# avik-pal/RegNeuralDE.jl

Hardware: AMD Instinct MI355X
Metric: training-step samples/sec + mean NFE, MNIST Neural ODE bs=512 (higher is better)
Workload: dtype f32; 1 GPU; MNIST NODE regularized (error_est), Tsit5 reltol=abstol=1.4e-8, batch 512 per GPU, 1xMI355X per rank; step = loss fwd + reverse pass through the solver + InvDecay/Momentum update; the weights train during the timed steps (mean_nfe drifts with --steps: value_fixed_weights of --full is the stationary companion); global_batch=512, parallelism=single

## Files before the change

### include/rnde.h

```cpp
#ifndef RNDE_H
#define RNDE_H
#include <stddef.h>
#include <stdint.h>

#ifdef __cplusplus
extern "C" {
#endif

#define RNDE_MAX_LAYERS 8

typedef enum {
    RNDE_OK = 0,
    RNDE_ERR_BAD_ARG = 1,
    RNDE_ERR_MAX_ATTEMPTS = 2,
    RNDE_ERR_DT_UNDERFLOW = 3,
    RNDE_ERR_NONFINITE = 4,
    RNDE_ERR_HIP = 5,
    RNDE_ERR_NO_TAPE = 6,
    RNDE_ERR_NO_DEVICE = 7
} rnde_status;

typedef enum { RNDE_ACT_IDENTITY = 0, RNDE_ACT_TANH = 1, RNDE_ACT_RELU = 2, RNDE_ACT_SIGMOID = 3, RNDE_ACT_SOFTPLUS = 4, RNDE_ACT_ELU = 5 } rnde_act;
typedef enum { RNDE_PRE_NONE = 0, RNDE_PRE_TANH = 1, RNDE_PRE_CUBE = 2 } rnde_pre_act;
typedef enum { RNDE_SOLVER_TSIT5 = 0, RNDE_SOLVER_DP5 = 1, RNDE_SOLVER_DOP853 = 2 } rnde_solver;
// ... 17 lines not shown
    int32_t max_attempts;
    int32_t device;
    int32_t col_tile;
    int32_t persist;
    int32_t wgrad_side_pct;
    int32_t stage_generic;
} rnde_node_config;

typedef struct rnde_node rnde_node;
typedef struct rnde_comm rnde_comm;

const char* rnde_version(void);
const char* rnde_last_error(const rnde_node* h);
int32_t     rnde_param_count(const rnde_node_config* cfg);

rnde_status rnde_node_create(const rnde_node_config* cfg, rnde_node** out);
void        rnde_node_destroy(rnde_node* h);

rnde_status rnde_node_forward(rnde_node* h, const float* x_dev, const float* p_dev, int32_t B,
                              float t0, float t1, float* u_out_dev, int64_t* nfe_out,
                              float* saveval_host, int32_t* n_saveval_out, int32_t keep_tape,
                              void* stream);

rnde_status rnde_node_forward_saveat(rnde_node* h, const float* x_dev, const float* p_dev, int32_t B,
                                     float t0, float t1, const float* saveat_host, int32_t n_saveat,
                                     float* u_saved_dev, int64_t* nfe_out, float* saveval_host,
                                     int32_t* n_saveval_out, int32_t keep_tape, void* stream);

rnde_status rnde_node_forward_everystep(rnde_node* h, const float* x_dev, const float* p_dev, int32_t B, float t0, float t1,
                                        int32_t save_start, float* sol_out_dev, int32_t capacity, float* t_host_out, int32_t* n_out,
                                        int64_t* nfe_out, float* saveval_host, int32_t* n_saveval_out, int32_t keep_tape, void* stream);

rnde_status rnde_node_forward_replay(rnde_node* h, const float* x_dev, const float* p_dev, int32_t B,
                                     float t0, float t1, const float* steps_host, int32_t n_steps,
                                     float* u_out_dev, int64_t* nfe_out, float* saveval_host,
                                     int32_t* n_saveval_out, int32_t keep_tape, void* stream);

rnde_status rnde_node_backward(rnde_node* h, const float* u_bar_dev, const float* saveval_bar_host,
                               float* x_bar_dev, float* p_bar_dev, float* tspan_bar_host,
                               void* stream);

rnde_status rnde_node_backward_async(rnde_node* h, const float* u_bar_dev, const float* saveval_bar_host,
                                     float* x_bar_dev, float* p_bar_dev, float* tspan_bar_dev, void* stream);

rnde_status rnde_node_release_tape(rnde_node* h);

rnde_status rnde_node_forward_host(rnde_node* h, const float* x, const float* p, int32_t B, float t0,
                                   float t1, float* u_out, int64_t* nfe_out, float* saveval,
                                   int32_t* n_saveval_out, int32_t keep_tape);
rnde_status rnde_node_backward_host(rnde_node* h, const float* u_bar, const float* saveval_bar,
                                    float* x_bar, float* p_bar, float* tspan_bar);

rnde_status rnde_node_steps(rnde_node* h, float* steps_host, int32_t capacity, int32_t* n_attempts_out);

rnde_status rnde_debug_feval(rnde_node* h, const float* u_dev, const float* p_dev, int32_t B, float t,
                             float* out_dev, void* stream);
rnde_status rnde_debug_attempt(rnde_node* h, const float* uprev_dev, const float* k1_dev,
                               const float* p_dev, int32_t B, float t, float dt, float* k_out_dev,
                               float* unew_out_dev, float* eest_out, void* stream);
rnde_status rnde_bench_attempt(rnde_node* h, const float* x_dev, const float* p_dev, int32_t B,
                               int32_t iters, float* mean_us_out, void* stream);
rnde_status rnde_bench_attempt_taped(rnde_node* h, const float* x_dev, const float* p_dev, int32_t B,
                                     int32_t iters, float* mean_us_out, void* stream);
rnde_status rnde_bench_attempt_cold_tape(rnde_node* h, const float* x_dev, const float* p_dev, int32_t B, int32_t iters,
                                         int32_t records, float* mean_us_out, void* stream);
rnde_status rnde_node_set_timing(rnde_node* h, int32_t on);
rnde_status rnde_node_timing(rnde_node* h, float* fwd_attempts_ms, float* rev_sweep_ms, float* rev_rest_ms);
int32_t     rnde_node_last_attempts(const rnde_node* h);
int32_t     rnde_node_fallback_count(const rnde_node* h);
int32_t     rnde_node_launches_per_attempt(const rnde_node* h);
int32_t     rnde_node_one_launch_solves(const rnde_node* h);
#define RNDE_MATRIX_F32 0
#define RNDE_MATRIX_BF16X3 1
rnde_status rnde_node_set_matrix_mode(rnde_node* h, int32_t mode);
int32_t     rnde_node_matrix_mode(const rnde_node* h);

typedef struct rnde_tapes rnde_tapes;
rnde_status rnde_tapes_create(const rnde_node_config* cfg, int32_t max_tapes, rnde_tapes** out);
void        rnde_tapes_destroy(rnde_tapes* t);
const char* rnde_tapes_last_error(const rnde_tapes* t);
int32_t     rnde_tapes_in_use(const rnde_tapes* t);
rnde_node*  rnde_tapes_node(rnde_tapes* t, int32_t tape_id);
rnde_status rnde_tapes_forward(rnde_tapes* t, const float* x_dev, const float* p_dev, int32_t B, float t0, float t1, float* u_out_dev,
                               int64_t* nfe_out, float* saveval_host, int32_t* n_saveval_out, int32_t keep_tape, void* stream,
                               int32_t* tape_id_out);
rnde_status rnde_tapes_backward(rnde_tapes* t, int32_t tape_id, const float* u_bar_dev, const float* saveval_bar_host, float* x_bar_dev,
                                float* p_bar_dev, float* tspan_bar_host, void* stream);
rnde_status rnde_tapes_release(rnde_tapes* t, int32_t tape_id);

rnde_status rnde_classifier_head(rnde_node* h, const float* u_dev, const float* p3_dev, const float* y_dev,
                                 int32_t B, int32_t n_classes, float* logits_out_dev, float* u_bar_dev,
                                 float* p3_bar_dev, float* ce_out_dev, void* stream);

rnde_status rnde_node_classifier_grad(rnde_node* h, const float* x_dev, const float* p2_dev, const float* p3_dev,
                                      const float* y_dev, int32_t B, int32_t n_classes, float t0, float t1, float lambda,
                                      float* p2_bar_dev, float* p3_bar_dev, float* x_bar_dev, float* ce_out_dev,
                                      float* reg_out_host, int64_t* nfe_out, rnde_comm* comm, void* stream);

rnde_status rnde_momentum_step(float* p_dev, const float* g_dev, float* v_dev, int64_t len, int64_t n, float gamma,
                               float eta, float rho, void* stream);

rnde_status rnde_momentum_step_scaled(float* p_dev, const float* g_dev, float* v_dev, int64_t len, int64_t n, float gamma,
                                      float eta, float rho, float gscale, void* stream);
rnde_status rnde_adam_step(float* p_dev, const float* g_dev, float* m_dev, float* v_dev, int64_t len, int64_t t, float eta, float beta1,
                           float beta2, float eps, float gscale, void* stream);
rnde_status rnde_adabelief_step(float* p_dev, const float* g_dev, float* m_dev, float* s_dev, int64_t len, float eta, float beta1, float beta2,
                                float eps, float gscale, void* stream);

#define RNDE_COMM_ID_BYTES 128
rnde_status rnde_comm_unique_id(uint8_t id_out[RNDE_COMM_ID_BYTES]);
rnde_status rnde_comm_create(const uint8_t id[RNDE_COMM_ID_BYTES], int32_t rank, int32_t world, int32_t device, rnde_comm** out);
void        rnde_comm_destroy(rnde_comm* c);
int32_t     rnde_comm_world(const rnde_comm* c);
const char* rnde_comm_last_error(const rnde_comm* c);
const char* rnde_comm_library(void);
rnde_status rnde_comm_allreduce(rnde_comm* c, float* buf_dev, int64_t n, int32_t mean, void* stream);
rnde_status rnde_comm_create_local_group(int32_t world, int32_t device, rnde_comm** out);
rnde_status rnde_comm_health(rnde_comm* c);
#define RNDE_COMM_WINDOW_BYTES 64
typedef struct rnde_comm_window rnde_comm_window;
rnde_status rnde_comm_window_create(int32_t device, rnde_comm_window** win_out, uint8_t handle_out[RNDE_COMM_WINDOW_BYTES]);
void        rnde_comm_window_destroy(rnde_comm_window* w);
rnde_status rnde_comm_create_peers(rnde_comm_window* win, const uint8_t* handles, int32_t rank, int32_t world, rnde_comm** out);
const char* rnde_comm_path(const rnde_comm* c);

rnde_status rnde_node_set_coupling(rnde_node* h, rnde_comm* c, int32_t global_batch);

typedef enum { RNDE_SDE_SOSRI = 0, RNDE_SDE_SRIW1 = 1, RNDE_SDE_SOSRI2 = 2 } rnde_sde_solver;

typedef struct {
    int32_t drift_layers;
    int32_t drift_dims[RNDE_MAX_LAYERS + 1];
    int32_t drift_act[RNDE_MAX_LAYERS];
    int32_t diff_layers;
    int32_t diff_dims[RNDE_MAX_LAYERS + 1];
    int32_t diff_act[RNDE_MAX_LAYERS];
    int32_t max_batch;
    int32_t solver;
    float   reltol, abstol;
    int32_t regularize;
    int32_t cb_save_start;
    int32_t max_attempts;
    int32_t device;
    float   beta1, beta2, gamma, qmin, qmax, qoldinit, delta;
    int32_t generic;
    float   stability_size;
} rnde_nsde_config;

typedef struct rnde_nsde rnde_nsde;

int32_t     rnde_nsde_param_count(const rnde_nsde_config* cfg, int32_t* len_drift_out);
rnde_status rnde_nsde_create(const rnde_nsde_config* cfg, rnde_nsde** out);
void        rnde_nsde_destroy(rnde_nsde* h);
const char* rnde_nsde_last_error(const rnde_nsde* h);

rnde_status rnde_nsde_forward(rnde_nsde* h, const float* x_dev, const float* p_dev, int32_t B, float t0, float t1,
// ... 95 lines not shown
```

### regneuralde.jl_amd/_lib.py

```python
import ctypes as C
import os

from . import build as _build

MAX_LAYERS = 8
OK, BAD_ARG, MAX_ATTEMPTS, DT_UNDERFLOW, NONFINITE, HIP_ERR, NO_TAPE, NO_DEVICE = range(8)
REG = {"none": 0, False: 0, None: 0, "error_est": 1, True: 1, "stiff_est": 2, "error_stiff_est": 3}


class NodeConfig(C.Structure):
    _fields_ = [("n_layers", C.c_int32), ("dims", C.c_int32 * (MAX_LAYERS + 1)), ("act", C.c_int32 * MAX_LAYERS),
                ("time_dep", C.c_int32), ("pre_act", C.c_int32), ("max_batch", C.c_int32), ("solver", C.c_int32),
                ("reltol", C.c_float), ("abstol", C.c_float), ("regularize", C.c_int32),
                ("cb_save_start", C.c_int32), ("track_ctrl", C.c_int32), ("track_initdt", C.c_int32),
                ("max_attempts", C.c_int32), ("device", C.c_int32), ("col_tile", C.c_int32),
                ("persist", C.c_int32), ("wgrad_side_pct", C.c_int32), ("stage_generic", C.c_int32)]


class NsdeConfig(C.Structure):
    _fields_ = [("drift_layers", C.c_int32), ("drift_dims", C.c_int32 * (MAX_LAYERS + 1)), ("drift_act", C.c_int32 * MAX_LAYERS),
                ("diff_layers", C.c_int32), ("diff_dims", C.c_int32 * (MAX_LAYERS + 1)), ("diff_act", C.c_int32 * MAX_LAYERS),
                ("max_batch", C.c_int32), ("solver", C.c_int32), ("reltol", C.c_float), ("abstol", C.c_float),
                ("regularize", C.c_int32), ("cb_save_start", C.c_int32), ("max_attempts", C.c_int32), ("device", C.c_int32),
                ("beta1", C.c_float), ("beta2", C.c_float), ("gamma", C.c_float), ("qmin", C.c_float), ("qmax", C.c_float),
# ... 2 lines not shown

class FfjordConfig(C.Structure):
    _fields_ = [("in_dims", C.c_int32), ("hidden", C.c_int32), ("dynamics", C.c_int32), ("time_dep", C.c_int32), ("regularize", C.c_int32),
                ("kinetic_reg", C.c_int32), ("max_batch", C.c_int32), ("solver", C.c_int32), ("reltol", C.c_float), ("abstol", C.c_float),
                ("cb_save_start", C.c_int32), ("max_attempts", C.c_int32), ("device", C.c_int32)]


class LatentConfig(C.Structure):
    _fields_ = [("max_batch", C.c_int32), ("max_T", C.c_int32), ("device", C.c_int32)]


ODE_SOLVER = {"Tsit5": 0, "AutoTsit5": 0, "DP5": 1, "DOP853": 2}
SDE_SOLVER = {"SOSRI": 0, "SRIW1": 1, "SOSRI2": 2, "AutoSOSRI2": 2}


class RndeError(RuntimeError):
    def __init__(self, status, msg):
        super().__init__(f"rnde status {status}: {msg}")
        self.status = status


_lib = None


def lib():
    global _lib
    if _lib is not None:
        return _lib
    path = _build.LIB
    if not os.path.exists(path):
        raise ImportError(f"{path} is missing: build it with `python -c 'import __graft_entry__ as g; g.build()'` "
                          "(hipcc --offload-arch=gfx950). There is no CPU fallback for the integration path.")
    L = C.CDLL(path)
    vp, f, i32, i64p, fp, i32p = C.c_void_p, C.c_float, C.c_int32, C.POINTER(C.c_int64), C.POINTER(C.c_float), C.POINTER(C.c_int32)
    L.rnde_version.restype = C.c_char_p
    L.rnde_last_error.restype = C.c_char_p
    L.rnde_last_error.argtypes = [vp]
    L.rnde_param_count.restype = i32
    L.rnde_param_count.argtypes = [C.POINTER(NodeConfig)]
    L.rnde_node_create.argtypes = [C.POINTER(NodeConfig), C.POINTER(vp)]
    L.rnde_node_destroy.argtypes = [vp]
    L.rnde_node_destroy.restype = None
    L.rnde_node_forward.argtypes = [vp, vp, vp, i32, f, f, vp, i64p, fp, i32p, i32, vp]
    L.rnde_node_forward_saveat.argtypes = [vp, vp, vp, i32, f, f, fp, i32, vp, i64p, fp, i32p, i32, vp]
    L.rnde_node_forward_everystep.argtypes = [vp, vp, vp, i32, f, f, i32, vp, i32, fp, i32p, i64p, fp, i32p, i32, vp]
    L.rnde_node_forward_replay.argtypes = [vp, vp, vp, i32, f, f, fp, i32, vp, i64p, fp, i32p, i32, vp]
    L.rnde_node_backward.argtypes = [vp, vp, fp, vp, vp, fp, vp]
    L.rnde_node_backward_async.restype = C.c_int32
    L.rnde_node_backward_async.argtypes = [vp, vp, fp, vp, vp, vp, vp]
    L.rnde_node_release_tape.argtypes = [vp]
    L.rnde_node_forward_host.argtypes = [vp, fp, fp, i32, f, f, fp, i64p, fp, i32p, i32]
    L.rnde_node_backward_host.argtypes = [vp, fp, fp, fp, fp, fp]
    L.rnde_node_steps.argtypes = [vp, fp, i32, i32p]
    L.rnde_debug_feval.argtypes = [vp, vp, vp, i32, f, vp, vp]
    L.rnde_debug_attempt.argtypes = [vp, vp, vp, vp, i32, f, f, vp, vp, fp, vp]
    L.rnde_bench_attempt.argtypes = [vp, vp, vp, i32, i32, fp, vp]
    L.rnde_bench_attempt_taped.argtypes = [vp, vp, vp, i32, i32, fp, vp]
    L.rnde_bench_attempt_cold_tape.argtypes = [vp, vp, vp, i32, i32, i32, fp, vp]
    L.rnde_node_set_timing.argtypes = [vp, i32]
    L.rnde_node_timing.argtypes = [vp, fp, fp, fp]
    L.rnde_node_fallback_count.restype = C.c_int32
    L.rnde_node_fallback_count.argtypes = [vp]
    L.rnde_node_last_attempts.restype = C.c_int32
    L.rnde_node_last_attempts.argtypes = [vp]
    L.rnde_node_launches_per_attempt.restype = C.c_int32
    L.rnde_node_launches_per_attempt.argtypes = [vp]
    L.rnde_node_one_launch_solves.restype = C.c_int32
    L.rnde_node_one_launch_solves.argtypes = [vp]
    L.rnde_node_set_matrix_mode.restype = C.c_int32
    L.rnde_node_set_matrix_mode.argtypes = [vp, i32]
    L.rnde_node_matrix_mode.restype = C.c_int32
    L.rnde_node_matrix_mode.argtypes = [vp]
    L.rnde_classifier_head.argtypes = [vp, vp, vp, vp, i32, i32, vp, vp, vp, vp, vp]
    L.rnde_node_classifier_grad.argtypes = [vp, vp, vp, vp, vp, i32, i32, f, f, f, vp, vp, vp, vp, fp, C.POINTER(C.c_int64), vp, vp]
    L.rnde_momentum_step.argtypes = [vp, vp, vp, C.c_int64, C.c_int64, f, f, f, vp]
    u64 = C.c_uint64
    L.rnde_momentum_step_scaled.argtypes = [vp, vp, vp, C.c_int64, C.c_int64, f, f, f, f, vp]
    L.rnde_adam_step.argtypes = [vp, vp, vp, vp, C.c_int64, C.c_int64, C.c_float, C.c_float, C.c_float, C.c_float, C.c_float, vp]
    L.rnde_adabelief_step.argtypes = [vp, vp, vp, vp, C.c_int64, f, f, f, f, f, vp]
    L.rnde_moment_loss.argtypes = [vp, vp, vp, i32, i32, i32, vp, vp, vp]
    L.rnde_comm_unique_id.argtypes = [C.c_char_p]
    L.rnde_comm_create.argtypes = [C.c_char_p, i32, i32, i32, C.POINTER(vp)]
    L.rnde_comm_destroy.argtypes = [vp]
    L.rnde_comm_destroy.restype = None
    L.rnde_comm_world.argtypes = [vp]
    L.rnde_comm_world.restype = i32
    L.rnde_comm_last_error.argtypes = [vp]
    L.rnde_comm_last_error.restype = C.c_char_p
    L.rnde_comm_library.argtypes = []
    L.rnde_comm_library.restype = C.c_char_p
    L.rnde_comm_allreduce.argtypes = [vp, vp, C.c_int64, i32, vp]
    L.rnde_comm_create_local_group.argtypes = [i32, i32, C.POINTER(vp)]
    L.rnde_node_set_coupling.argtypes = [vp, vp, i32]
    L.rnde_comm_health.argtypes = [vp]
    L.rnde_comm_window_create.argtypes = [i32, C.POINTER(vp), C.c_char_p]
    L.rnde_comm_window_destroy.argtypes = [vp]
    L.rnde_comm_window_destroy.restype = None
    L.rnde_comm_create_peers.argtypes = [vp, C.c_char_p, i32, i32, C.POINTER(vp)]
    L.rnde_comm_path.argtypes = [vp]
    L.rnde_comm_path.restype = C.c_char_p
    L.rnde_tapes_create.argtypes = [C.POINTER(NodeConfig), i32, C.POINTER(vp)]
    L.rnde_tapes_destroy.argtypes = [vp]
    L.rnde_tapes_destroy.restype = None
    L.rnde_tapes_last_error.argtypes = [vp]
    L.rnde_tapes_last_error.restype = C.c_char_p
    L.rnde_tapes_in_use.argtypes = [vp]
    L.rnde_tapes_node.argtypes = [vp, i32]
    L.rnde_tapes_node.restype = vp
    L.rnde_tapes_forward.argtypes = [vp, vp, vp, i32, C.c_float, C.c_float, vp, C.POINTER(C.c_int64), fp, C.POINTER(i32), i32, vp, C.POINTER(i32)]
    L.rnde_tapes_backward.argtypes = [vp, i32, vp, fp, vp, vp, fp, vp]
    L.rnde_tapes_release.argtypes = [vp, i32]
    L.rnde_nsde_param_count.restype = i32
    L.rnde_nsde_param_count.argtypes = [C.POINTER(NsdeConfig), i32p]
    L.rnde_nsde_create.argtypes = [C.POINTER(NsdeConfig), C.POINTER(vp)]
    L.rnde_nsde_destroy.argtypes = [vp]
    L.rnde_nsde_destroy.restype = None
    L.rnde_nsde_last_error.restype = C.c_char_p
    L.rnde_nsde_last_error.argtypes = [vp]
    L.rnde_nsde_forward.argtypes = [vp, vp, vp, i32, f, f, vp, i32, u64, vp, i64p, i64p, fp, i32p, i32, vp]
    L.rnde_nsde_forward_saveat.argtypes = [vp, vp, vp, i32, f, f, vp, i32, u64, fp, i32, vp, i64p, i64p, fp, i32p, i32, vp]
    L.rnde_nsde_forward_everystep.argtypes = [vp, vp, vp, i32, f, f, vp, i32, u64, i32, vp, i32, fp, i32p, i64p, i64p, fp, i32p, i32, vp]
    L.rnde_nsde_forward_replay.argtypes = [vp, vp, vp, i32, f, f, vp, i32, fp, i32, vp, i64p, i64p, fp, i32p, i32, vp]
    L.rnde_nsde_backward.argtypes = [vp, vp, fp, vp, vp, vp]
    L.rnde_nsde_backward_async.argtypes = [vp, vp, fp, vp, vp, vp]
    L.rnde_nsde_classifier_head.argtypes = [vp, vp, vp, vp, i32, i32, vp, vp, vp, vp, vp]
    L.rnde_nsde_classifier_grad.argtypes = [vp, vp, vp, vp, vp, i32, i32, f, f, vp, i32, C.c_uint64, f, vp, vp, vp, vp, fp, C.POINTER(C.c_int64), C.POINTER(C.c_int64), vp]
    L.rnde_nsde_steps.argtypes = [vp, fp, i32, i32p, i32p]
    L.rnde_nsde_debug_attempt.argtypes = [vp, vp, vp, i32, f, vp, vp, vp, vp, fp, vp]
    L.rnde_nsde_set_pre_act.argtypes = [vp, i32, i32]
    L.rnde_nsde_moment_grad.argtypes = [vp, vp, vp, i32, f, f, vp, i32, u64, fp, i32, vp, vp, f, vp, vp, vp, fp, i64p, i64p, vp]
    L.rnde_nsde_timing.argtypes = [vp, fp, fp, i32p, i32p]
    L.rnde_normal_fill.argtypes = [vp, C.c_int64, u64, u64, vp]
    L.rnde_latent_create.argtypes = [C.POINTER(LatentConfig), C.POINTER(vp)]
    L.rnde_latent_destroy.argtypes = [vp]
    L.rnde_latent_destroy.restype = None
    L.rnde_latent_last_error.argtypes = [vp]
    L.rnde_latent_last_error.restype = C.c_char_p
    L.rnde_latent_param_counts.argtypes = [i32p, i32p, i32p]
    L.rnde_latent_param_counts.restype = None
    L.rnde_latent_encode.argtypes = [vp, vp, vp, vp, vp, i32, i32, vp, vp, vp, vp]
    L.rnde_latent_decode_loss.argtypes = [vp, vp, vp, vp, i32, i32, vp, vp, vp, vp]
    L.rnde_latent_encode_backward.argtypes = [vp, vp, f, vp, vp, vp, vp, vp, vp]
    L.rnde_adamax_step.argtypes = [vp, vp, vp, vp, C.c_int64, C.c_int64, f, f, f, f, f, f, vp]
    L.rnde_ffjord_param_count.restype = i32
    L.rnde_ffjord_param_count.argtypes = [C.POINTER(FfjordConfig)]
    L.rnde_ffjord_create.argtypes = [C.POINTER(FfjordConfig), C.POINTER(vp)]
    L.rnde_ffjord_destroy.argtypes = [vp]
    L.rnde_ffjord_destroy.restype = None
    L.rnde_ffjord_last_error.argtypes = [vp]
    L.rnde_ffjord_last_error.restype = C.c_char_p
    L.rnde_ffjord_forward.argtypes = [vp, vp, vp, vp, i32, f, f, u64, vp, vp, i64p, fp, i32p, i32, vp]
    L.rnde_ffjord_forward_replay.argtypes = [vp, vp, vp, vp, i32, f, f, u64, fp, i32, vp, vp, i64p, fp, i32p, i32, vp]
    L.rnde_ffjord_steps.argtypes = [vp, fp, i32, i32p]
    L.rnde_ffjord_backward.argtypes = [vp, vp, fp, vp, vp, vp]
    L.rnde_ffjord_sample.argtypes = [vp, vp, vp, i32, f, f, u64, vp, vp]
    L.rnde_ffjord_debug_feval.argtypes = [vp, vp, vp, vp, i32, f, i32, vp, vp]
    L.rnde_ffjord_timing.argtypes = [vp, fp, fp, i32p, i32p]
    L.rnde_ffjord_create_tiled.argtypes = [C.POINTER(FfjordConfig), C.POINTER(vp)]
    L.rnde_ffjord_engine.restype = i32
    L.rnde_ffjord_engine.argtypes = [vp]
    _lib = L
    return L


EXPORTS = ["rnde_version", "rnde_last_error", "rnde_param_count", "rnde_node_create", "rnde_node_destroy",
           "rnde_node_forward", "rnde_node_forward_saveat", "rnde_node_forward_everystep", "rnde_node_forward_replay", "rnde_node_backward", "rnde_node_backward_async", "rnde_node_release_tape", "rnde_node_forward_host",
           "rnde_node_backward_host", "rnde_node_steps", "rnde_debug_feval", "rnde_debug_attempt",
           "rnde_bench_attempt", "rnde_bench_attempt_taped", "rnde_bench_attempt_cold_tape", "rnde_node_set_timing", "rnde_node_timing", "rnde_node_last_attempts", "rnde_node_fallback_count",
           "rnde_node_launches_per_attempt", "rnde_node_one_launch_solves", "rnde_node_set_matrix_mode", "rnde_node_matrix_mode", "rnde_classifier_head", "rnde_node_classifier_grad", "rnde_momentum_step", "rnde_momentum_step_scaled", "rnde_adam_step",
           "rnde_comm_unique_id", "rnde_comm_create", "rnde_comm_destroy", "rnde_comm_world", "rnde_comm_last_error", "rnde_comm_library", "rnde_comm_allreduce", "rnde_comm_create_local_group", "rnde_comm_health", "rnde_comm_window_create", "rnde_comm_window_destroy", "rnde_comm_create_peers", "rnde_comm_path", "rnde_node_set_coupling", "rnde_tapes_create", "rnde_tapes_destroy", "rnde_tapes_last_error", "rnde_tapes_in_use", "rnde_tapes_node", "rnde_tapes_forward", "rnde_tapes_backward", "rnde_tapes_release",
           "rnde_nsde_param_count", "rnde_nsde_create", "rnde_nsde_destroy", "rnde_nsde_last_error", "rnde_nsde_forward",
           "rnde_nsde_forward_saveat", "rnde_nsde_forward_everystep", "rnde_nsde_forward_replay", "rnde_nsde_backward", "rnde_nsde_backward_async", "rnde_nsde_classifier_head", "rnde_nsde_classifier_grad", "rnde_nsde_steps", "rnde_nsde_debug_attempt", "rnde_nsde_set_pre_act", "rnde_nsde_moment_grad", "rnde_moment_loss", "rnde_adabelief_step", "rnde_nsde_timing", "rnde_normal_fill", "rnde_latent_create", "rnde_latent_destroy", "rnde_latent_last_error", "rnde_latent_param_counts", "rnde_latent_encode",
           "rnde_latent_decode_loss", "rnde_latent_encode_backward", "rnde_adamax_step",
           "rnde_ffjord_param_count", "rnde_ffjord_create", "rnde_ffjord_destroy", "rnde_ffjord_last_error", "rnde_ffjord_forward",
           "rnde_ffjord_forward_replay", "rnde_ffjord_steps", "rnde_ffjord_backward", "rnde_ffjord_sample", "rnde_ffjord_debug_feval",
           "rnde_ffjord_timing", "rnde_ffjord_create_tiled", "rnde_ffjord_engine"]


def check(h, status):
    if status != OK:
        msg = lib().rnde_last_error(h).decode() if h else lib().rnde_last_error(None).decode()
        raise RndeError(status, msg)


def check_latent(h, status):
    if status != OK:
        raise RndeError(status, lib().rnde_latent_last_error(h if h else None).decode())


def check_ffjord(h, status):
    if status != OK:
        raise RndeError(status, lib().rnde_ffjord_last_error(h if h else None).decode())


def check_nsde(h, status):
    if status != OK:
        raise RndeError(status, lib().rnde_nsde_last_error(h if h else None).decode())
```

### regneuralde.jl_amd/classifier.py

```python
import math
import os

import torch

from .layers import Dense
from .node import TrackedNeuralODE


class ClassifierNODE:

    def __init__(self, node: TrackedNeuralODE, post: Dense, device="cuda"):
        self.node = node
        self.post_shape = (post.n_in, post.n_out)
        self.p1 = torch.zeros(0, device=device)
        self.p2 = node.p.to(device).clone().requires_grad_(True)
        self.p3 = torch.cat([post.W.reshape(-1), post.b]).to(device).clone().requires_grad_(True)

    def trainable(self):
        return (self.p1, self.p2, self.p3)

    def __call__(self, x, p1=None, p2=None, p3=None, **node_kwargs):
        p2 = self.p2 if p2 is None else p2
        p3 = self.p3 if p3 is None else p3
        x = x.reshape(x.shape[0], -1)
# ... 55 lines not shown
    n = nsv.value
    reg = 0.0
    svb = None
    if regularize and n > 0 and node.regularize:
        if agg_max:
            vals = list(sv[:n])
            k = max(range(n), key=lambda i: vals[i])
            reg = lam * vals[k]
            svb = (C.c_float * n)(*[lam if i == k else 0.0 for i in range(n)])
        else:
            reg = lam * sum(sv[:n]) / n
            svb = (C.c_float * n)(*([lam / n] * n))
    xbar = torch.empty_like(x2)
    n2 = p2bar.numel()
    if not sync:
        _lib.check(h.ptr, L.rnde_node_backward_async(h.ptr, ubar.data_ptr(), svb, xbar.data_ptr(), p2bar.data_ptr(), None, stream))
        if reducer is not None:
            reducer.allreduce_range_(0, n2 + p3bar.numel())
        model.p2.grad, model.p3.grad = p2bar, p3bar
        node.last_nfe = int(nfe.value)
        model._keep = (ubar, xbar, u)
        return ce + reg, ce, reg, int(nfe.value)
    _lib.check(h.ptr, L.rnde_node_backward(h.ptr, ubar.data_ptr(), svb, xbar.data_ptr(), p2bar.data_ptr(), None, stream))
    if reducer is not None:
        reducer.allreduce_range_(0, n2 + p3bar.numel())
    model.p2.grad, model.p3.grad = p2bar, p3bar
    node.last_nfe = int(nfe.value)
    ce_f = float(ce.item())
    return ce_f + reg, ce_f, reg, int(nfe.value)


def logitcrossentropy(pred, y_onehot):
    return -(y_onehot * torch.log_softmax(pred, dim=1)).sum(dim=1).mean()


def loss_function(x, y, model, p1=None, p2=None, p3=None, lam=1.0e2, regularize=True, agg=torch.mean, func="error_est",
                  tspan=None):
    pred, nfe, sv = model(x, p1, p2, p3, func=func, tspan=tspan)
    ce = logitcrossentropy(pred, y)
    reg = lam * agg(sv.saveval) if regularize else torch.zeros((), device=pred.device)
    return ce + reg, ce.detach(), reg.detach(), nfe


class FluxOptimiser:

    def __init__(self, params, gamma=1.0e-5, eta=0.1, rho=0.9):
        self.params = [p for p in params if p.numel() > 0]
        self.gamma, self.eta, self.rho = gamma, eta, rho
        self.n = [1 for _ in self.params]
        self.v = [torch.zeros_like(p) for p in self.params]

    @torch.no_grad()
    def step(self, grads=None, grad_scale=1.0):
        for i, p in enumerate(self.params):
            g = p.grad if grads is None else grads[i]
            if g is None:
                continue
            if p.is_cuda:
                import ctypes as C
                from . import _lib
                g = g.contiguous()
                st = _lib.lib().rnde_momentum_step_scaled(p.data_ptr(), g.data_ptr(), self.v[i].data_ptr(), p.numel(), self.n[i],
                                                          self.gamma, self.eta, self.rho, float(grad_scale),
                                                          C.c_void_p(torch.cuda.current_stream(p.device).cuda_stream))
                _lib.check(None, st)
                self.n[i] += 1
                p.grad = None
                continue
            g = g * (grad_scale / (1.0 + self.gamma * self.n[i]))
            self.n[i] += 1
            self.v[i].mul_(self.rho).sub_(g, alpha=self.eta)
            p.add_(self.v[i])
            p.grad = None


class FluxADAM:

    def __init__(self, params, eta=0.001, beta=(0.9, 0.999), eps=1.0e-8, gamma=0.0, weight_decay=0.0):
        self.params = [p for p in params if p.numel() > 0]
        self.eta, self.beta, self.eps, self.gamma, self.weight_decay = eta, beta, eps, gamma, weight_decay
        self.n = [1 for _ in self.params]
        self.t = 0
        self.m = [torch.zeros_like(p) for p in self.params]
        self.v = [torch.zeros_like(p) for p in self.params]

    @torch.no_grad()
    def step(self, grad_scale=1.0):
        import ctypes as C
        from . import _lib
        self.t += 1
        for i, p in enumerate(self.params):
            g = p.grad
            if g is None:
                continue
            if not p.is_cuda:
                raise RuntimeError("FluxADAM runs on the device only")
            g = g.contiguous()
            gs = float(grad_scale) / (1.0 + self.gamma * self.n[i])
            if self.weight_decay:
                g = g.mul(float(grad_scale)).add_(p.data, alpha=float(self.weight_decay)).contiguous()
                gs = 1.0 / (1.0 + self.gamma * self.n[i])
            st = _lib.lib().rnde_adam_step(p.data_ptr(), g.data_ptr(), self.m[i].data_ptr(), self.v[i].data_ptr(), p.numel(), self.t, self.eta,
                                           self.beta[0], self.beta[1], self.eps, gs,
                                           C.c_void_p(torch.cuda.current_stream(p.device).cuda_stream))
            _lib.check(None, st)
            self.n[i] += 1
# ... 55 lines not shown
```

### regneuralde.jl_amd/csrc/rnde.hip

```cpp
#include "rnde_node.h"

static thread_local std::string g_create_err;
extern "C" const char* rnde_version(void) { return "rnde 0.1.0 (gfx950)"; }
extern "C" const char* rnde_last_error(const rnde_node* h) { return h ? h->err.c_str() : g_create_err.c_str(); }

extern "C" int32_t rnde_param_count(const rnde_node_config* c) {
    int n = 0;
    for (int l = 0; l < c->n_layers; ++l) n += (c->dims[l] + (c->time_dep ? 1 : 0)) * c->dims[l + 1] + c->dims[l + 1];
    return n;
}

StepParams make_params(rnde_node* h, const float* x, int B, float t0, float t1, int tape) {
    StepParams P{};
    P.x = x;
    P.f0 = h->f0; P.h0 = h->h0; P.u1 = h->u1; P.f1 = h->f1; P.h1 = h->h1;
    P.arena = h->arena; P.rec_stride = h->rec_stride;
    P.ctl = h->ctl; P.ctl_final = h->ctl_final; P.meta = h->meta; P.initrec = h->initrec;
    P.errpart = h->errpart; P.initpart = h->initpart; P.dbg_out = nullptr;
    P.D = h->D; P.H = h->H; P.B = B; P.Bn = h->couple ? h->couple_batch : B;
    P.Bpad = ((B + 15) / 16) * 16;
    P.nwg = h->engine == 2 ? h->sR * (P.Bpad / 16) : (h->engine == 3 ? (h->mw ? P.Bpad / 16 : (P.Bpad / 16 + kCW - 1) / kCW) : P.Bpad / h->BT);
    P.reltol = h->cfg.reltol; P.abstol = h->cfg.abstol; P.t0 = t0; P.t1 = t1;
    P.tape = tape; P.max_attempts = h->cfg.max_attempts;
    P.forced = 0; P.forced_t = 0; P.forced_dt = 0;
// ... 300 lines not shown
    if (hipGetDeviceCount(&ndev) != hipSuccess || ndev <= c->device) { g_create_err = "no HIP device"; return RNDE_ERR_NO_DEVICE; }
    if ((c->solver != RNDE_SOLVER_TSIT5 && c->solver != RNDE_SOLVER_DP5 && c->solver != RNDE_SOLVER_DOP853) || c->n_layers < 1 || c->n_layers > RNDE_MAX_LAYERS || c->dims[0] != c->dims[c->n_layers]) {
        g_create_err = "unsupported configuration: Tsit5 (or DP5) over a Dense chain with dims[0] == dims[n_layers]"; return RNDE_ERR_BAD_ARG;
    }
    if (c->pre_act != RNDE_PRE_NONE && c->pre_act != RNDE_PRE_TANH && c->pre_act != RNDE_PRE_CUBE) {
        g_create_err = "pre_act: RNDE_PRE_NONE, RNDE_PRE_TANH or RNDE_PRE_CUBE"; return RNDE_ERR_BAD_ARG;
    }
    if (!rnde_check_acts(c->n_layers, c->act, "act", g_create_err)) return RNDE_ERR_BAD_ARG;
    const bool mnist_form = c->n_layers == 2 && c->time_dep && !c->pre_act && c->act[0] == RNDE_ACT_TANH;
    if (mnist_form && c->col_tile != 64 && c->col_tile != 65 && c->act[1] != RNDE_ACT_IDENTITY && c->act[1] != RNDE_ACT_TANH) {
        g_create_err = std::string("act[1] = ") + rnde_act_name(c->act[1]) + ": the stage engine (two time-dependent layers, act[0] = tanh, no pre_act, col_tile 0 / 16) "
                       "serves identity or tanh in its second layer; a chain of width <= 64 runs any served activation on the chain engine (col_tile 64 / 65)";
        return RNDE_ERR_BAD_ARG;
    }
    if ((c->solver == RNDE_SOLVER_DP5 || c->solver == RNDE_SOLVER_DOP853) && ((mnist_form && c->col_tile != 65) || c->col_tile == 64 || c->regularize >= RNDE_REG_STIFF)) {
        g_create_err = "DP5 / DOP853 run on the tableau-as-data kernels of the chain engine (col_tile 0 for Dense chains of width <= 64, or 65), callbacks none / EEst*dt";
        return RNDE_ERR_BAD_ARG;
    }
    if (c->col_tile == 64 || c->col_tile == 65 || !mnist_form) return chain_create(c, out);
    if (c->regularize < RNDE_REG_NONE || c->regularize > RNDE_REG_STIFF_DT) { g_create_err = "regularize: unknown value"; return RNDE_ERR_BAD_ARG; }
    rnde_node* h = new rnde_node();
    h->cfg = *c;
    h->D = c->dims[0]; h->H = c->dims[1]; h->P = rnde_param_count(c); h->act2 = c->act[1];
    h->BT = 8;
    if (c->col_tile != 0 && c->col_tile != 16) {
        g_create_err = "col_tile must be 0 (auto) or 16 (stage engine) for the two-layer TDChain form; 64 / 65 select the chain engine.  (The round-1 column-owner "
                       "engine, col_tile 4 / 8, was retired in round 4: 126 us per attempted step against 24; its sources are kept under tools/experiments/column_owner/.)";
        delete h; return RNDE_ERR_BAD_ARG;
    }
    if (h->H + 2 > 128 || h->D < 1 || h->H < 1 || (h->D + 15) / 16 > 64 || c->max_batch < 1 || c->max_attempts < 1) {
        g_create_err = "shape outside the kernel limits (H <= 126, D <= 1024)"; delete h; return RNDE_ERR_BAD_ARG;
    }
    h->Bpad_max = ((c->max_batch + 15) / 16) * 16;
    h->sMT = (h->D + 15) / 16; h->sHT = (h->H + 1 + 15) / 16; h->sK2b = (h->H + 2 + 15) / 16; h->sKHb = (h->H + 15) / 16;
    { int best = 1, bw = 1 << 30;
      for (int wt = std::min(8, h->sMT); wt >= std::max(1, std::min(4, h->sMT)); --wt) { int R = (h->sMT + wt - 1) / wt; int waste = R * wt - h->sMT; if (waste < bw) { bw = waste; best = wt; } }
      if (const char* e = getenv("RNDE_STAGE_WT")) { const int v = atoi(e); if (v >= 1 && v <= 8) best = std::min(v, h->sMT); }
      h->sWT = best; h->sR = (h->sMT + best - 1) / best; }
    h->engine = 2;
    h->nwg_max = std::max(h->Bpad_max / h->BT, h->sR * (h->Bpad_max / 16));
    h->stage_lds = sizeof(float) * ((size_t)16 * (16 * std::max(h->sK2b, h->sHT) + 4) + (size_t)16 * (16 * std::max(h->sWT, h->sKHb) + 4) + 64);
    if (hipSetDevice(c->device) != hipSuccess) { g_create_err = "hipSetDevice failed"; delete h; return RNDE_ERR_HIP; }
    const size_t A = (size_t)h->D * h->Bpad_max, HB = (size_t)h->H * h->Bpad_max;
    RecLayout L{(long long)A, (long long)HB};
    h->rec_stride = L.total();
    auto dm = [&](void** p, size_t bytes) { return hipMalloc(p, bytes) == hipSuccess; };
    bool ok = true;
    ok &= dm((void**)&h->f0, A * 4) && dm((void**)&h->u1, A * 4) && dm((void**)&h->f1, A * 4) && dm((void**)&h->xcopy, A * 4);
    ok &= dm((void**)&h->h0, HB * 4) && dm((void**)&h->h1, HB * 4);
    ok &= dm((void**)&h->pcopy, (size_t)h->P * 4);
    ok &= dm((void**)&h->spwB, (size_t)h->sMT * h->sK2b * 64 * 16) && dm((void**)&h->spwD, (size_t)h->sHT * h->sMT * 64 * 16);
    ok &= dm((void**)&h->spwBt, (size_t)h->sMT * h->sKHb * 64 * 16) && dm((void**)&h->spwDt, (size_t)h->sHT * h->sMT * 64 * 16);
    ok &= dm((void**)&h->slab2, (size_t)2 * (h->Bpad_max / 16) * h->sR * h->sHT * 64 * 16);
    const size_t tslab_bytes = (size_t)3 * (h->Bpad_max / 16) * h->sR * h->sHT * 64 * 16;
    h->tslab_bytes = tslab_bytes;
    ok &= dm((void**)&h->tslab, tslab_bytes);
    static_assert(sizeof(StepState) <= 512 && sizeof(InitRec) <= 504, "mailbox layout");
    h->mbox_meta_off = (1024 + (size_t)h->nwg_max * 4 + 255) / 256 * 256;
    const size_t mbox_bytes = h->mbox_meta_off + (size_t)(c->max_attempts + 1) * sizeof(StepMeta);
    ok &= dm((void**)&h->mbox, mbox_bytes) && hipHostMalloc((void**)&h->h_mbox, mbox_bytes) == hipSuccess;
    if (ok) {
        hipMemset(h->mbox, 0, mbox_bytes);
        h->ctl_final = (StepState*)h->mbox; h->initrec = (InitRec*)(h->mbox + 512);
        h->pabort = (unsigned*)(h->mbox + 1016); h->pxcc = (unsigned*)(h->mbox + 1024); h->meta = (StepMeta*)(h->mbox + h->mbox_meta_off);
        h->h_ctl = (StepState*)h->h_mbox; h->h_init = (InitRec*)(h->h_mbox + 512);
        h->h_pchk = (unsigned*)(h->h_mbox + 1016); h->h_meta = (StepMeta*)(h->h_mbox + h->mbox_meta_off);
    }
    ok &= dm((void**)&h->ctl, 2 * sizeof(StepState));
    ok &= dm((void**)&h->errpart, (size_t)(6 * h->nwg_max + 256 + 16) * 4) && dm((void**)&h->initpart, (size_t)(3 * h->nwg_max + 256) * 4);
    h->arena_recs = 2;
    ok &= dm((void**)&h->arena, (size_t)h->arena_recs * h->rec_stride * 4);
    ok &= hipHostMalloc((void**)&h->h_scal, 64 * sizeof(float)) == hipSuccess;
    if (!ok) { g_create_err = "device allocation failed"; rnde_node_destroy(h); return RNDE_ERR_HIP; }
    hipMemset(h->tslab, 0xFF, tslab_bytes); hipMemset(h->pabort, 0, 8); hipMemset(h->pxcc, 0, (size_t)h->nwg_max * 4);
    {
        const char* e = getenv("RNDE_PERSIST");
        const bool off = c->persist < 0 || (e && e[0] == '0');
        h->persist = (h->engine == 2 && h->sR <= 8 && !off) ? 1 : 0;
        if (const char* e2 = getenv("RNDE_PERSIST_SPINS")) h->persist_spins = atoi(e2);
        if (const char* e3 = getenv("RNDE_PERSIST2")) h->persist2 = atoi(e3);
        h->wgrad_side_pct = c->wgrad_side_pct < 0 ? 0 : (c->wgrad_side_pct == 0 ? 30 : std::min(100, c->wgrad_side_pct));
        if (const char* e3 = getenv("RNDE_WGRAD_SIDE")) h->wgrad_side_pct = atoi(e3);
        h->stage_generic = (c->stage_generic != 0 || getenv("RNDE_STAGE_GENERIC") != nullptr) ? 1 : 0;
        if (const char* e6 = getenv("RNDE_STAGE_SOLVE")) h->stage_solve = atoi(e6);
    }
    if (h->persist == 1 && h->stage_solve && c->max_attempts < 8192) {
        const size_t xb = (size_t)(c->max_attempts + 1) * 3 * 256 * 8;
        if (hipMalloc((void**)&h->sxch, xb) != hipSuccess) { g_create_err = "device allocation failed"; rnde_node_destroy(h); return RNDE_ERR_HIP; }
        hipMemset(h->sxch, 0, xb);
    }
    if (h->persist == 1) {
        h->x3 = 1;
        if (const char* e7 = getenv("RNDE_X3")) h->x3 = atoi(e7) != 0;
        if (h->sMT == 49 && h->sHT == 7 && h->sR == 7 && h->sWT == 7 && h->D == 784 && h->H == 100 && !h->stage_generic) {
            const size_t img = (size_t)49 * 4 * 3 * 64 * 16;
            if (hipMalloc(&h->x3B, img) != hipSuccess || hipMalloc(&h->x3D, img) != hipSuccess || hipMalloc(&h->x3Bt, img) != hipSuccess || hipMalloc(&h->x3Dt, img) != hipSuccess) { g_create_err = "device allocation failed"; rnde_node_destroy(h); return RNDE_ERR_HIP; }
        } else h->x3 = 0;
    }
    h->predicted = 12;
    *out = h;
    return RNDE_OK;
}

extern "C" void rnde_node_destroy(rnde_node* h) {
    if (!h) return;
    void* d[] = {h->f0, h->h0, h->u1, h->f1, h->h1, h->arena, h->xcopy, h->pcopy, h->spwB, h->spwD, h->spwBt, h->spwDt, h->slab2,
                 h->ctl, h->ctl_final, h->meta, h->initrec, h->errpart, h->initpart};
// ... 65 lines not shown
    HIPCHK(h, hipMalloc((void**)&h->arena, (size_t)recs * h->rec_stride * 4));
    h->arena_recs = recs;
    return RNDE_OK;
}

static StageParams make_stage_params(rnde_node* h, const StepParams& P, const float* p_dev) {
    StageParams Q{};
    Q.F = P; Q.p = p_dev; Q.pwB = h->spwB; Q.pwD = h->spwD; Q.slab = h->slab2;
    Q.MT = h->sMT; Q.WT = h->sWT; Q.R = h->sR; Q.C = P.Bpad / 16; Q.HT = h->sHT; Q.K2b = h->sK2b; Q.Bpad16 = P.Bpad;
    return Q;
}
template <int ACT2, int MODE>
static hipError_t launch_stage_t(rnde_node* h, const StageParams& Q, int n, int s, hipStream_t st) {
    hipLaunchKernelGGL((rnde_stage_kernel<ACT2, MODE>), dim3(Q.R * Q.C), dim3(64 * Q.WT), h->stage_lds, st, Q, n, s);
    return hipGetLastError();
}
template <int MODE>
static hipError_t launch_stage(rnde_node* h, const StageParams& Q, int n, int s, hipStream_t st) {
    return h->act2 ? launch_stage_t<1, MODE>(h, Q, n, s, st) : launch_stage_t<0, MODE>(h, Q, n, s, st);
}
hipError_t stage_pack(rnde_node* h, const float* p, f32x4* dst, int which, int MTrows, int Kb, hipStream_t st) {
    const long long total = (long long)MTrows * Kb * 64;
    const int grid = (int)std::min<long long>((total + 255) / 256, 1024);
    hipLaunchKernelGGL(rnde_stage_pack_kernel, dim3(grid), dim3(256), 0, st, p, dst, which, h->D, h->H, MTrows, Kb);
    return hipGetLastError();
}
static rnde_status x3_pack(rnde_node* h, const float* p_dev, bool with_rev, hipStream_t s) {
    h->x3_fwd = false;
    if (!(h->x3 && h->x3B && h->x3D && h->persist == 1 && !h->stage_generic)) return RNDE_OK;
    HIPCHK(h, rnde_launch_x3_pack(p_dev, h->x3B, h->x3D, with_rev ? h->x3Bt : nullptr, with_rev ? h->x3Dt : nullptr, h->D, h->H, h->sMT, h->sWT, h->sR, h->sHT, s));
    h->x3_fwd = true;
    h->x3_packed = with_rev;
    return RNDE_OK;
}
static rnde_status stage_pack_weights(rnde_node* h, const float* p_dev, hipStream_t s) {
    HIPCHK(h, stage_pack(h, p_dev, h->spwB, 0, h->sMT, h->sK2b, s));
    HIPCHK(h, stage_pack(h, p_dev, h->spwD, 1, h->sHT, h->sMT, s));
    return x3_pack(h, p_dev, false, s);
}
rnde_status stage_pack_all(rnde_node* h, const float* p_dev, hipStream_t s, const float* x_src, long long x_floats) {
    PackJobs J{};
    int n = 0;
    auto add = [&](void* dst, long long total, int kind, int which, int kdim, const float* src = nullptr) { J.j[n++] = PackJob{dst, src, total, kind, which, kdim, 0}; };
    add(h->spwB, (long long)h->sMT * h->sK2b * 64, 0, 0, h->sK2b);
    add(h->spwD, (long long)h->sHT * h->sMT * 64, 0, 1, h->sMT);
    add(h->spwBt, (long long)h->sMT * h->sKHb * 64, 0, 2, h->sKHb);
    add(h->spwDt, (long long)h->sHT * h->sMT * 64, 0, 3, h->sMT);
    auto add_copy = [&](float* dst, const float* src, long long floats) {
        const bool v4 = floats % 4 == 0 && ((uintptr_t)dst % 16 == 0) && ((uintptr_t)(src ? src : p_dev) % 16 == 0);
        add(dst, v4 ? floats / 4 : floats, v4 ? 3 : 2, 0, 0, src);
    };
    add_copy(h->pcopy, nullptr, (long long)h->P);
    if (x_src) add_copy(h->xcopy, x_src, x_floats);
    long long most = 0;
    for (int i = 0; i < n; ++i) most = std::max(most, J.j[i].total);
    const int grid = (int)std::min<long long>((most + 255) / 256, 256);
    hipLaunchKernelGGL(rnde_pack_all_kernel, dim3(grid, n), dim3(256), 0, s, p_dev, J, h->D, h->H);
    HIPCHK(h, hipGetLastError());
    h->rev_packed = true;
    return x3_pack(h, p_dev, true, s);
}
hipError_t slab_prepare(rnde_node* h, int Bpad, hipStream_t s) {
    if (h->tslab_Bpad == Bpad) return hipSuccess;
    h->tslab_Bpad = Bpad;
    return hipMemsetAsync(h->tslab, 0xFF, h->tslab_bytes, s);
}
static bool stage_two_tile(const rnde_node* h, const StageParams& Q) {
    const bool fix = Q.WT == 7 && Q.HT == 7 && Q.K2b == 7 && Q.MT == 49 && Q.R == 7 && h->D == 784 && h->H == 100 && !h->stage_generic;
    return h->persist == 1 && fix && Q.C % 2 == 0 && h->persist2 != 0 && (Q.C >= kPersist2MinTiles || h->persist2 >= 1);
}
static bool stage_epart_reduce(const rnde_node* h, const StageParams& Q) {
    return stage_two_tile(h, Q) && Q.F.nwg >= 896 && !getenv("RNDE_NO_EPART_REDUCE");
}
static hipError_t stage_attempt(rnde_node* h, const StageParams& Q, int n, hipStream_t s) {
    if (h->persist == 1) {
        PersistSync Y{h->tslab, h->pabort, h->pxcc, h->persist_spins};
        if (hipError_t e = slab_prepare(h, Q.Bpad16, s); e != hipSuccess) return e;
        const dim3 grid(8 * Q.R * ((Q.C + 7) / 8));
        const bool fix = Q.WT == 7 && Q.HT == 7 && Q.K2b == 7 && Q.MT == 49 && Q.R == 7 && h->D == 784 && h->H == 100 && !h->stage_generic;
        static const bool x3_over_mt = !(getenv("RNDE_X3_MT") && atoi(getenv("RNDE_X3_MT")) == 0);
        if (stage_two_tile(h, Q)) {
            const dim3 grid2(8 * Q.R * ((Q.C / 2 + 7) / 8));
            if (h->x3_fwd && x3_over_mt) {
                const size_t xlds2 = sizeof(float) * ((size_t)2 * 2 * kX3ImageFloats + 32 * 3);
                if (h->act2) hipLaunchKernelGGL((rnde_stage_attempt_mt_kernel<1, 2, 1>), grid2, dim3(64 * 7), xlds2, s, Q, n, Y, (const void*)h->x3B, (const void*)h->x3D);
                else hipLaunchKernelGGL((rnde_stage_attempt_mt_kernel<0, 2, 1>), grid2, dim3(64 * 7), xlds2, s, Q, n, Y, (const void*)h->x3B, (const void*)h->x3D);
                return hipGetLastError();
            }
            const size_t lds2 = sizeof(float) * (2 * 2 * 16 * (16 * 7 + 4) + 32 * 3);
            if (h->act2) hipLaunchKernelGGL((rnde_stage_attempt_mt_kernel<1, 2>), grid2, dim3(64 * 7), lds2, s, Q, n, Y, (const void*)nullptr, (const void*)nullptr);
            else hipLaunchKernelGGL((rnde_stage_attempt_mt_kernel<0, 2>), grid2, dim3(64 * 7), lds2, s, Q, n, Y, (const void*)nullptr, (const void*)nullptr);
            return hipGetLastError();
        }
        if (fix && h->x3_fwd) {
            const size_t xlds = sizeof(float) * ((size_t)2 * kX3ImageFloats + 64);
            if (h->act2) hipLaunchKernelGGL((rnde_stage_attempt_kernel<1, 1, 1>), grid, dim3(64 * 7), xlds, s, Q, n, Y, (const void*)h->x3B, (const void*)h->x3D);
            else hipLaunchKernelGGL((rnde_stage_attempt_kernel<0, 1, 1>), grid, dim3(64 * 7), xlds, s, Q, n, Y, (const void*)h->x3B, (const void*)h->x3D);
        } else if (fix) {
            if (h->act2) hipLaunchKernelGGL((rnde_stage_attempt_kernel<1, 1>), grid, dim3(64 * Q.WT), h->stage_lds, s, Q, n, Y, (const void*)nullptr, (const void*)nullptr);
            else hipLaunchKernelGGL((rnde_stage_attempt_kernel<0, 1>), grid, dim3(64 * Q.WT), h->stage_lds, s, Q, n, Y, (const void*)nullptr, (const void*)nullptr);
        } else if (h->act2) hipLaunchKernelGGL((rnde_stage_attempt_kernel<1, 0>), grid, dim3(64 * Q.WT), h->stage_lds, s, Q, n, Y, (const void*)nullptr, (const void*)nullptr);
        else hipLaunchKernelGGL((rnde_stage_attempt_kernel<0, 0>), grid, dim3(64 * Q.WT), h->stage_lds, s, Q, n, Y, (const void*)nullptr, (const void*)nullptr);
        return hipGetLastError();
    }
    hipError_t e = launch_stage<SM_START>(h, Q, n, 0, s);
    for (int st = 1; st <= 5 && e == hipSuccess; ++st) e = launch_stage<SM_STAGE>(h, Q, n, st, s);
    if (e == hipSuccess) e = launch_stage<SM_LAST>(h, Q, n, 6, s);
    return e;
}

bool bsweep_failed(rnde_node* h, hipStream_t s) {
    if (!h->pending_bsweep) return false;
    h->pending_bsweep = false;
    bool bad = h->h_mw_bchk[0] != 0;
    const int nt = h->bsweep_nt;
    for (int i = 1; i < nt && !h->bsweep_global && !bad; ++i) bad = h->h_mw_bchk[2 + i] != h->h_mw_bchk[2];
    if (!bad) return false;
    fprintf(stderr, "[rnde] chain engine: one-launch reverse sweep abandoned (%s); one launch per reversed attempt for the next %d solves\n",
// ... 95 lines not shown
        h->err = "coupled controller: equal shards only (B * world must equal the global batch given to rnde_node_set_coupling)";
        return RNDE_ERR_BAD_ARG;
    }
    HIPCHK(h, hipSetDevice(h->cfg.device));
    h->have_tape = false; h->rev_packed = false; h->x3_packed = false; h->x3_fwd = false;
    const float* x_caller = nullptr;
    if (keep_tape) {
        rnde_status st = ensure_arena(h, h->cfg.max_attempts);
        if (st != RNDE_OK) return st;
        if (B % h->BT) HIPCHK(h, hipMemsetAsync(h->xcopy, 0, (size_t)h->D * (((B + h->BT - 1) / h->BT) * h->BT) * 4, s));
        if (h->engine != 2) {
            HIPCHK(h, hipMemcpyAsync(h->xcopy, x_dev, (size_t)h->D * B * 4, hipMemcpyDeviceToDevice, s));
            HIPCHK(h, hipMemcpyAsync(h->pcopy, p_dev, (size_t)h->P * 4, hipMemcpyDeviceToDevice, s));
        } else x_caller = x_dev;
        x_dev = h->xcopy;
    }
    StepParams P = make_params(h, x_dev, B, t0, t1, keep_tape ? 1 : 0);
    P.sv_t = n_saveat > 0 ? h->sv_t_dev : nullptr; P.nsave = n_saveat; P.sv_out = sv_out_dev;
    if (h->n_replay > 0) {
        if ((size_t)h->n_replay > h->replay_cap) {
            if (h->replay_dev) hipFree(h->replay_dev);
            h->replay_dev = nullptr; h->replay_cap = 0;
            HIPCHK(h, hipMalloc((void**)&h->replay_dev, (size_t)h->n_replay * 8));
            h->replay_cap = h->n_replay;
        }
        HIPCHK(h, hipMemcpyAsync(h->replay_dev, h->replay_host, (size_t)h->n_replay * 8, hipMemcpyHostToDevice, s));
        P.replay = h->replay_dev; P.n_replay = h->n_replay;
    }
    h->B = B; h->Bpad = P.Bpad; h->nwg = P.nwg; h->t0 = t0; h->t1 = t1;
    rnde_status st = RNDE_OK;
    if (h->engine == 2 && keep_tape) st = stage_pack_all(h, p_dev, s, x_caller, (long long)h->D * B);
    else if (h->engine == 3) st = chain_pack(h, keep_tape ? h->pcopy : p_dev, s);
    if (st != RNDE_OK) return st;
    StageParams SQ{};
    ChainParams CQ{};
    MwParams MQ{};
    if (h->engine == 3) {
        CQ = make_chain_params(h, P);
        if (h->mw) {
            if (keep_tape) { st = ensure_mw_slab(h, 2 + (long long)(h->rk_S - 1) * std::max(4, h->predicted), P.Bpad, s); if (st != RNDE_OK) return st; }
            MQ = make_mw_params(h, P);
            HIPCHK(h, launch_mw<MW_INIT_A>(h, MQ, 0, s));
            if ((st = couple_sum(h, P.initpart, 2LL * P.nwg, s)) != RNDE_OK) return st;
            HIPCHK(h, launch_mw<MW_INIT_B>(h, MQ, 0, s));
            if ((st = couple_sum(h, P.initpart + 2LL * P.nwg, P.nwg, s)) != RNDE_OK) return st;
        } else {
            HIPCHK(h, launch_chain<CM_INIT_A>(h, CQ, 0, nullptr, s));
            HIPCHK(h, launch_chain<CM_INIT_B>(h, CQ, 0, nullptr, s));
        }
    } else if (h->engine == 2) {
        if (!keep_tape) { st = stage_pack_weights(h, p_dev, s); if (st != RNDE_OK) return st; }
        SQ = make_stage_params(h, P, keep_tape ? h->pcopy : p_dev);
        if (stage_epart_reduce(h, SQ)) SQ.F.esum = (const double*)(h->errpart + 6 * (size_t)h->nwg_max + 256);
        HIPCHK(h, launch_stage<SM_I1>(h, SQ, 0, 0, s));
        HIPCHK(h, launch_stage<SM_I2>(h, SQ, 0, 0, s));
        if ((st = couple_sum(h, P.initpart, 2LL * P.nwg, s)) != RNDE_OK) return st;
        HIPCHK(h, launch_stage<SM_I3>(h, SQ, 0, 0, s));
        HIPCHK(h, launch_stage<SM_I4>(h, SQ, 0, 0, s));
        if ((st = couple_sum(h, P.initpart + 2LL * P.nwg, P.nwg, s)) != RNDE_OK) return st;
    }
    int launched = 0;
    int chunk = h->couple ? 16 : std::max(4, h->predicted);
    const int cap = h->cfg.max_attempts;
    h->tev_fwd = false;
    if (h->timing) HIPCHK(h, hipEventRecord(h->tev[0], s));
    bool solved = false;
    if (h->engine == 3 && h->mw && h->mw_solve > 0 && !h->couple && P.Bpad / 16 <= kMwMeetMax) {
        const int n_limit = keep_tape ? std::min(cap, std::max(48, 2 * h->predicted)) : cap;
        if (keep_tape) { st = ensure_mw_slab(h, 2 + (long long)(h->rk_S - 1) * n_limit, P.Bpad, s); if (st != RNDE_OK) return st; MQ.slab = h->mw_slab; }
        MQ.n_limit = n_limit;
        if (++h->mw_epoch >= 500000u) { h->mw_epoch = 1; HIPCHK(h, hipMemsetAsync(h->mw_xch, 0, (size_t)(cap + 4) * 3 * kMwMeetMax * 8, s)); }
        const int nt = P.Bpad / 16;
        MQ.u_out = u_out_dev; MQ.xch = h->mw_xch; MQ.xcc = h->mw_xcc; MQ.abort_word = h->mw_abort; MQ.epoch = h->mw_epoch; MQ.xch_global = nt > 32 ? 1 : 0; MQ.xcd_slot = h->mw_slot;
        HIPCHK(h, launch_mw<MW_SOLVE>(h, MQ, 0, s));
        if (h->timing) { HIPCHK(h, hipEventRecord(h->tev[1], s)); h->tev_fwd = true; }
        HIPCHK(h, hipMemcpyAsync(h->h_ctl, h->ctl_final, sizeof(StepState), hipMemcpyDeviceToHost, s));
        HIPCHK(h, hipMemcpyAsync(h->h_meta, h->meta, (size_t)cap * sizeof(StepMeta), hipMemcpyDeviceToHost, s));
        HIPCHK(h, hipMemcpyAsync(h->h_init, h->initrec, sizeof(InitRec), hipMemcpyDeviceToHost, s));
        HIPCHK(h, hipMemcpyAsync(h->h_mw_chk, h->mw_abort, 4, hipMemcpyDeviceToHost, s));
        HIPCHK(h, hipMemcpyAsync(h->h_mw_chk + 2, h->mw_xcc, (size_t)nt * 4, hipMemcpyDeviceToHost, s));
        if (h->after_solve) {
            HIPCHK(h, hipEventRecord(h->ev_host, s));
            const rnde_status hs = h->after_solve(s);
            if (hs != RNDE_OK) return hs;
            HIPCHK(h, hipEventSynchronize(h->ev_host));
        } else HIPCHK(h, hipStreamSynchronize(s));
        if (bsweep_failed(h, s)) { h->err = "the one-launch reverse sweep of the previous asynchronous backward call was abandoned: the gradients of that step are invalid (one launch per reversed attempt now in use)"; return RNDE_ERR_HIP; }
        bool bad = h->h_mw_chk[0] != 0;
        for (int i = 1; i < nt && !MQ.xch_global && !bad; ++i) bad = h->h_mw_chk[2 + i] != h->h_mw_chk[2];
        if (bad) {
            fprintf(stderr, "[rnde] chain engine: one-launch solve abandoned (%s); one launch per attempted step for the next %d solves\n",
                    h->h_mw_chk[0] ? "a meeting timed out" : "workgroups pinned by block index landed on different XCDs", h->mw_retry_after);
            h->mw_solve = -1; h->mw_clean = 0; ++h->persist_fallbacks;
            hipMemsetAsync(h->mw_abort, 0, 8, s);
            return RNDE_INTERNAL_RETRY;
        }
        if (!h->h_ctl->done && h->h_ctl->n_att >= n_limit && n_limit < cap) { h->predicted = cap; return RNDE_INTERNAL_RETRY; }
        h->pending_bwd = false;
        ++h->one_launch_solves;
        solved = true;
    }
    if (h->engine == 2 && h->persist == 1 && h->stage_solve && h->sxch && SQ.C <= 32 && n_saveat == 0 && h->n_replay == 0 && !h->couple &&
        SQ.WT == 7 && SQ.HT == 7 && SQ.K2b == 7 && SQ.MT == 49 && SQ.R == 7 && h->D == 784 && h->H == 100 && !h->stage_generic) {
        PersistSync Y{h->tslab, h->pabort, h->pxcc, h->persist_spins};
        HIPCHK(h, slab_prepare(h, SQ.Bpad16, s));
        if (++h->s_epoch >= 500000u) { h->s_epoch = 1; HIPCHK(h, hipMemsetAsync(h->sxch, 0, (size_t)(cap + 1) * 3 * 256 * 8, s)); }
        const int x3 = h->x3_fwd ? 1 : 0;
        SolveSync Z{h->sxch, h->s_epoch, cap, h->x3B, h->x3D};
#ifdef RNDE_DIAG
        StageParams SD = SQ;
        if (getenv("RNDE_DIAG_SOLVE")) {
// ... 171 lines not shown
    }
    h->n_saveval = nsv;
    if (n_saveval_out) *n_saveval_out = nsv;
    switch (h->h_ctl->status) {
        case 0: break;
        case 2: h->err = "max_attempts reached"; return RNDE_ERR_MAX_ATTEMPTS;
        case 3: h->err = "dt underflow"; return RNDE_ERR_DT_UNDERFLOW;
        default: h->err = "non-finite error estimate or dt"; return RNDE_ERR_NONFINITE;
    }
    h->have_tape = keep_tape != 0;
    return RNDE_OK;
}

extern "C" rnde_status rnde_node_forward_everystep(rnde_node* h, const float* x_dev, const float* p_dev, int32_t B, float t0, float t1, int32_t save_start,
                                                   float* sol_out_dev, int32_t capacity, float* t_host_out, int32_t* n_out, int64_t* nfe_out,
                                                   float* saveval_host, int32_t* n_saveval_out, int32_t keep_tape, void* stream) {
    if (!h || !n_out || !sol_out_dev || capacity < 1) return RNDE_ERR_BAD_ARG;
    rnde_status st = forward_impl(h, x_dev, p_dev, B, t0, t1, nullptr, nullptr, 0, nullptr, nullptr, nullptr, nullptr, 0, stream);
    if (st != RNDE_OK) return st;
    std::vector<float> times;
    if (save_start) times.push_back(t0);
    for (int i = 0; i < h->n_att; ++i) {
        const StepMeta& m = h->h_meta[i];
        if (m.flags & F_ACCEPT) { float tn = m.t + m.dt; if (tn > t1) tn = t1; times.push_back(tn); }
    }
    *n_out = (int32_t)times.size();
    if ((int)times.size() > capacity) { h->err = "rnde_node_forward_everystep: more accepted steps than the output has room for"; return RNDE_ERR_BAD_ARG; }
    if (t_host_out) memcpy(t_host_out, times.data(), times.size() * sizeof(float));
    st = forward_impl(h, x_dev, p_dev, B, t0, t1, nullptr, times.data(), (int32_t)times.size(), sol_out_dev, nfe_out, saveval_host, n_saveval_out, keep_tape, stream);
    if (st != RNDE_OK) return st;
    size_t k = save_start ? 1 : 0;
    for (int i = 0; i < h->n_att; ++i) {
        const StepMeta& m = h->h_meta[i];
        if (!(m.flags & F_ACCEPT)) continue;
        float tn = m.t + m.dt; if (tn > t1) tn = t1;
        if (k >= times.size() || times[k] != tn) { h->err = "rnde_node_forward_everystep: the saving solve did not retrace the steps of the first one"; return RNDE_ERR_HIP; }
        ++k;
    }
    if (k != times.size()) { h->err = "rnde_node_forward_everystep: the saving solve took fewer accepted steps than the first one"; return RNDE_ERR_HIP; }
    return RNDE_OK;
}

extern "C" rnde_status rnde_node_steps(rnde_node* h, float* steps_host, int32_t capacity, int32_t* n_out) {
    if (!h) return RNDE_ERR_BAD_ARG;
    const int n = std::min(capacity, h->n_att);
    for (int i = 0; i < n; ++i) {
        steps_host[4 * i + 0] = h->h_meta[i].t; steps_host[4 * i + 1] = h->h_meta[i].dt;
        steps_host[4 * i + 2] = h->h_meta[i].eest; steps_host[4 * i + 3] = (h->h_meta[i].flags & F_ACCEPT) ? 1.f : 0.f;
    }
    if (n_out) *n_out = h->n_att;
    return RNDE_OK;
}

extern "C" rnde_status rnde_node_set_timing(rnde_node* h, int32_t on) {
    if (!h) return RNDE_ERR_BAD_ARG;
    if (on && !h->tev[0]) for (auto& e : h->tev) HIPCHK(h, hipEventCreate(&e));
    h->timing = on ? 1 : 0; h->tev_fwd = h->tev_bwd = false;
    return RNDE_OK;
}
extern "C" rnde_status rnde_node_timing(rnde_node* h, float* fwd_attempts_ms, float* rev_sweep_ms, float* rev_rest_ms) {
    if (!h || !h->timing) return RNDE_ERR_BAD_ARG;
    float a = -1.f, b = -1.f, c = -1.f;
    if (h->tev_fwd) { HIPCHK(h, hipEventSynchronize(h->tev[1])); HIPCHK(h, hipEventElapsedTime(&a, h->tev[0], h->tev[1])); }
    if (h->tev_bwd) {
        HIPCHK(h, hipEventSynchronize(h->tev[4]));
        HIPCHK(h, hipEventElapsedTime(&b, h->tev[2], h->tev[3])); HIPCHK(h, hipEventElapsedTime(&c, h->tev[3], h->tev[4]));
    }
    if (fwd_attempts_ms) *fwd_attempts_ms = a;
    if (rev_sweep_ms) *rev_sweep_ms = b;
    if (rev_rest_ms) *rev_rest_ms = c;
    return RNDE_OK;
}
extern "C" int32_t rnde_node_last_attempts(const rnde_node* h) { return h ? h->n_att : 0; }
extern "C" int32_t rnde_node_fallback_count(const rnde_node* h) { return h ? h->persist_fallbacks : 0; }

extern "C" int32_t rnde_node_one_launch_solves(const rnde_node* h) { return h ? h->one_launch_solves : 0; }
extern "C" rnde_status rnde_node_set_matrix_mode(rnde_node* h, int32_t mode) {
    if (!h) return RNDE_ERR_BAD_ARG;
    if (mode != RNDE_MATRIX_F32 && mode != RNDE_MATRIX_BF16X3) { h->err = "matrix mode: 0 (fp32-input MFMA) or 1 (bf16x3 on the matrix cores)"; return RNDE_ERR_BAD_ARG; }
    h->x3 = (mode == RNDE_MATRIX_BF16X3 && h->x3B && h->x3D) ? 1 : 0;
    return RNDE_OK;
}
extern "C" int32_t rnde_node_matrix_mode(const rnde_node* h) { return (h && h->x3 && h->x3B && h->x3D) ? RNDE_MATRIX_BF16X3 : RNDE_MATRIX_F32; }
extern "C" int32_t rnde_node_launches_per_attempt(const rnde_node* h) {
    if (!h) return 0;
    return (h->engine == 2 && h->persist != 1) ? 7 : 1;
}

extern "C" rnde_status rnde_node_release_tape(rnde_node* h) {
    if (!h) return RNDE_ERR_BAD_ARG;
    h->have_tape = false;
    return RNDE_OK;
}

extern "C" rnde_status rnde_node_forward_host(rnde_node* h, const float* x, const float* p, int32_t B, float t0, float t1,
                                              float* u_out, int64_t* nfe_out, float* saveval, int32_t* n_saveval_out,
                                              int32_t keep_tape) {
    if (!h) return RNDE_ERR_BAD_ARG;
    float *xd = nullptr, *pd = nullptr, *ud = nullptr;
    const size_t nb = (size_t)h->D * B * 4;
    HIPCHK(h, hipMalloc((void**)&xd, nb)); HIPCHK(h, hipMalloc((void**)&ud, nb)); HIPCHK(h, hipMalloc((void**)&pd, (size_t)h->P * 4));
    HIPCHK(h, hipMemcpy(xd, x, nb, hipMemcpyHostToDevice)); HIPCHK(h, hipMemcpy(pd, p, (size_t)h->P * 4, hipMemcpyHostToDevice));
    rnde_status st = rnde_node_forward(h, xd, pd, B, t0, t1, ud, nfe_out, saveval, n_saveval_out, keep_tape, nullptr);
    if (st == RNDE_OK || st == RNDE_ERR_MAX_ATTEMPTS) hipMemcpy(u_out, ud, nb, hipMemcpyDeviceToHost);
    hipFree(xd); hipFree(pd); hipFree(ud);
    return st;
// ... 180 lines not shown
```

### regneuralde.jl_amd/csrc/rnde_binit_stage.h

```cpp
#pragma once
#include "rnde_bstage.h"

namespace rnde {

template <int ACT2, int STEP>
__global__ __launch_bounds__(64 * kSMaxW) void rnde_binit_stage_kernel(const BStageParams Q) {
#pragma clang fp contract(off)
    const BwdParams& Bq = Q.B;
    const StepParams& P = Bq.F;
    extern __shared__ __attribute__((aligned(16))) float smem[];
    const int KZ = 16 * Q.KHb + 4, KG = 16 * Q.WT + 4;
    float* ZL = smem;
    float* GL = ZL + kSCB * KZ;
    float* RED = GL + kSCB * KG;
    const int tid = threadIdx.x, lane = tid & 63;
    const int w = __builtin_amdgcn_readfirstlane(tid >> 6);
    const int rb = blockIdx.x / Q.C, ct = blockIdx.x - rb * Q.C;
    const int wg = blockIdx.x;
    const int col = lane & 15, gcol = ct * kSCB + col;
    const bool colok = gcol < P.B;
    const bool vec = (P.D & 3) == 0;
    const bool writer = (blockIdx.x == 0 && tid == 0);
    const int T = rb * Q.WT + w;
    const int r0 = 16 * T + 4 * (lane >> 4);
    const bool tile_ok = T < Q.MT;
    const long long A = (long long)P.D * P.Bpad, HB = (long long)P.H * P.Bpad;
    const size_t co = (size_t)gcol * P.D;
    const double N = (double)P.D * (double)P.Bn;
    const InitRec ir = *P.initrec;
    const float dt0 = ir.dt0;
    constexpr bool kD = (STEP == 0 || STEP == 2);
    constexpr int kPhase = STEP < 2 ? 1 : 2;
    constexpr int par = STEP < 2 ? 0 : 1;

    float dot = 0.f, tau = 0.f;
    if constexpr (kD) {
        f32x4 wD[kSMaxW];
#pragma unroll
        for (int kb = 0; kb < kSMaxW; ++kb)
            if (kb < Q.WT && w < Q.HT && rb * Q.WT + kb < Q.MT) wD[kb] = Q.pwDt[((size_t)w * Q.MT + rb * Q.WT + kb) * 64 + lane];
        f32x4 xv = {0.f, 0.f, 0.f, 0.f}, f0v = xv, f1v = xv, ub1 = xv, Uv = xv, K1v = xv;
        if (tile_ok) {
            xv = ld4(P.x + co, r0, P.D, colok, P.xvec != 0);
            f0v = ld4(P.f0 + co, r0, P.D, true, vec);
            f1v = ld4(P.f1 + co, r0, P.D, true, vec);
            if constexpr (kPhase == 2) {
                ub1 = ld4(Bq.UB1 + co, r0, P.D, true, vec);
                Uv = ld4(Bq.U + co, r0, P.D, true, vec);
                K1v = ld4(Bq.K1 + co, r0, P.D, true, vec);
            }
        }
        f32x4 v = {0.f, 0.f, 0.f, 0.f};
        if constexpr (kPhase == 1) {
            double tb, dtpb, qoldb, t1b, t0b;
            finish_attempt_scalars(Bq, 0, lane, tb, dtpb, qoldb, t1b, t0b);
            const double dtb = Bq.track_initdt ? dtpb : 0.0;
            double dt0b = 0, d1b = 0, d2b = 0;
            if (ir.sel == 2) { t1b += dtb; t0b -= dtb; }
            else if (ir.sel == 0) dt0b += 100.0 * dtb;
            else if (!ir.dt1_const) {
                const double mm = ir.max_is_d2 ? (double)ir.d2 : (double)ir.d1;
                const double mb = dtb * (-0.2) * (double)ir.dt1 / mm;
                if (ir.max_is_d2) d2b += mb; else d1b += mb;
            } else if (dt0 * 1e-3f > 1e-6f) dt0b += 1e-3 * dtb;
            const double n2 = (double)ir.d2 * (double)dt0, n2b = d2b / (double)dt0;
            dt0b += -d2b * (double)ir.d2 / (double)dt0;
            const double coef_w = n2 > 0 ? n2b / (N * n2) : 0.0;
            if (writer) { IBState b; b.tb = tb; b.t1b = t1b; b.t0b = t0b; b.dt0b = dt0b; b.d1b = d1b; b.d2b = d2b; b.coef_w = coef_w; b.pad = 0; Bq.ibstate[0] = b; }
            const float cw = (float)coef_w;
            if (tile_ok) {
#pragma unroll
                for (int i = 0; i < 4; ++i) {
                    const float sk = P.abstol + fabsf(xv[i]) * P.reltol;
                    const float wv = (f1v[i] - f0v[i]) / sk;
                    const float f1b = (colok && r0 + i < P.D ? cw * wv : 0.f) / sk;
                    v[i] = ACT2 ? f1b * (1.f - f1v[i] * f1v[i]) : f1b;
                }
                st4(Bq.zi2 + A + co, r0, P.D, true, vec, v);
            }
        } else {
            const IBState ib = Bq.ibstate[0];
            double dot1 = 0, tau1 = 0;
            for (int i = lane; i < P.nwg; i += 64) { dot1 += (double)Bq.ipart[4 * i]; tau1 += (double)Bq.ipart[4 * i + 1]; }
            dot1 = wave_sum_d(dot1); tau1 = wave_sum_d(tau1);
            double dt0b = ib.dt0b + tau1 + dot1, t0b = ib.t0b + tau1, t1b = ib.t1b, d1b = ib.d1b, d0b = 0;
            if (ir.dt0_clamped) { t1b += dt0b; t0b -= dt0b; }
            else if (!ir.dt0_const) { d0b = dt0b / (100.0 * (double)ir.d1); d1b += -dt0b * (double)dt0 / (double)ir.d1; }
            const float cv = ir.d1 > 0.f ? (float)(d1b / (N * (double)ir.d1)) : 0.f;
            const float cz = ir.d0 > 0.f ? (float)(d0b / (N * (double)ir.d0)) : 0.f;
            const float cw = (float)ib.coef_w;
            if (writer) { IBState b = ib; b.t1b = t1b; b.t0b = t0b; Bq.ibstate[1] = b; }
            if (tile_ok) {
                f32x4 u0b = {0.f, 0.f, 0.f, 0.f};
#pragma unroll
                for (int i = 0; i < 4; ++i) {
                    const bool ok = colok && r0 + i < P.D;
                    const float sk = P.abstol + fabsf(xv[i]) * P.reltol;
                    const float wv = (f1v[i] - f0v[i]) / sk, vv = f0v[i] / sk, z = xv[i] / sk;
                    const float wb = ok ? cw * wv : 0.f, vb = ok ? cv * vv : 0.f, zb = ok ? cz * z : 0.f;
                    const float skb = -(wb * wv + vb * vv + zb * z) / sk;
                    const float f0b = K1v[i] + dt0 * ub1[i] + (vb - wb) / sk;
                    u0b[i] = Uv[i] + ub1[i] + zb / sk + skb * P.reltol * sgnf(xv[i]);
                    if (Bq.sv_ubar0 && ok) u0b[i] += Bq.sv_ubar0[((size_t)gcol * Bq.sv_T) * P.D + r0 + i];
                    v[i] = ACT2 ? f0b * (1.f - f0v[i] * f0v[i]) : f0b;
                }
                st4(Bq.zi2 + co, r0, P.D, true, vec, v);
                st_tile(Bq.xbar + co, r0, P.D, colok, false, u0b);
            }
        }
#pragma unroll
        for (int i = 0; i < 4; ++i) GL[col * KG + kperm(16 * w + 4 * (lane >> 4) + i)] = tile_ok ? v[i] : 0.f;
        __syncthreads();
        f32x4* sl = (f32x4*)Q.slab + ((((size_t)par * Q.C + ct) * Q.R + rb) * Q.HT) * 64;
        const float* gbp = GL + col * KG + 4 * (lane >> 4);
        f32x4 bg[kSMaxW];
#pragma unroll
        for (int kb = 0; kb < kSMaxW; ++kb) if (kb < Q.WT) bg[kb] = *(const f32x4*)(gbp + 16 * kb);
        if (w < Q.HT) {
            f32x4 acc0 = {0.f, 0.f, 0.f, 0.f}, acc1 = {0.f, 0.f, 0.f, 0.f};
#pragma unroll
            for (int kb = 0; kb < kSMaxW; ++kb) {
                if (kb < Q.WT && rb * Q.WT + kb < Q.MT) {
                    acc0 = mfma16(wD[kb][0], bg[kb][0], acc0);
                    acc1 = mfma16(wD[kb][1], bg[kb][1], acc1);
                    acc0 = mfma16(wD[kb][2], bg[kb][2], acc0);
                    acc1 = mfma16(wD[kb][3], bg[kb][3], acc1);
                }
            }
            sl[(size_t)w * 64 + lane] = acc0 + acc1;
        }
        for (int ht = w + Q.WT; ht < Q.HT; ht += Q.WT) {
            f32x4 acc0 = {0.f, 0.f, 0.f, 0.f}, acc1 = {0.f, 0.f, 0.f, 0.f};
#pragma unroll
            for (int kb = 0; kb < kSMaxW; ++kb) {
                if (kb < Q.WT && rb * Q.WT + kb < Q.MT) {
                    const f32x4 a = Q.pwDt[((size_t)ht * Q.MT + rb * Q.WT + kb) * 64 + lane];
                    acc0 = mfma16(a[0], bg[kb][0], acc0);
                    acc1 = mfma16(a[1], bg[kb][1], acc1);
                    acc0 = mfma16(a[2], bg[kb][2], acc0);
                    acc1 = mfma16(a[3], bg[kb][3], acc1);
                }
            }
            sl[(size_t)ht * 64 + lane] = acc0 + acc1;
        }
        return;
    } else {
        f32x4 wB[kSMaxHT];
#pragma unroll
        for (int kb = 0; kb < kSMaxHT; ++kb)
            if (kb < Q.KHb && tile_ok) wB[kb] = Q.pwBt[((size_t)T * Q.KHb + kb) * 64 + lane];
        const float* hsrc = kPhase == 1 ? P.h1 : P.h0;
        float* z1dst = kPhase == 1 ? Bq.zi1 + HB : Bq.zi1;
        const float* W1t = Q.p + (size_t)P.H * P.D;
        const f32x4* sl = (const f32x4*)Q.slab + (((size_t)par * Q.C + ct) * Q.R) * Q.HT * 64;
        f32x4 f0v = {0.f, 0.f, 0.f, 0.f};
        if (kPhase == 1 && tile_ok) f0v = ld4(P.f0 + co, r0, P.D, true, vec);
        for (int ht = w; ht < Q.HT; ht += Q.WT) {
            f32x4 z = {0.f, 0.f, 0.f, 0.f};
            for (int r = 0; r < Q.R; ++r) z += sl[((size_t)r * Q.HT + ht) * 64 + lane];
            const int h0 = 16 * ht + 4 * (lane >> 4);
#pragma unroll
            for (int i = 0; i < 4; ++i) {
                const int hr = h0 + i;
                float zv = 0.f;
                if (hr < P.H) {
                    const float hv = hsrc[(size_t)gcol * P.H + hr];
                    zv = z[i] * (1.f - hv * hv);
                    if (rb == 0) { z1dst[(size_t)gcol * P.H + hr] = zv; tau += W1t[hr] * zv; }
                } else if (hr == P.H) {
                    if (rb == 0) tau += z[i];
                }
                if (hr < 16 * Q.KHb) ZL[col * KZ + kperm(hr)] = zv;
            }
        }
        if (Q.KHb > Q.HT) {
            for (int i = tid; i < kSCB * 16 * Q.KHb; i += blockDim.x) {
                const int c = i / (16 * Q.KHb), k = i - c * 16 * Q.KHb;
                if (k >= 16 * Q.HT) ZL[c * KZ + kperm(k)] = 0.f;
            }
        }
        __syncthreads();
        f32x4 gb = {0.f, 0.f, 0.f, 0.f};
        if (tile_ok) {
            f32x4 acc0 = {0.f, 0.f, 0.f, 0.f}, acc1 = {0.f, 0.f, 0.f, 0.f};
            const float* zb = ZL + col * KZ + 4 * (lane >> 4);
            f32x4 bf[kSMaxHT];
#pragma unroll
            for (int kb = 0; kb < kSMaxHT; ++kb) if (kb < Q.KHb) bf[kb] = *(const f32x4*)(zb + 16 * kb);
#pragma unroll
            for (int kb = 0; kb < kSMaxHT; ++kb) {
                if (kb < Q.KHb) {
                    acc0 = mfma16(wB[kb][0], bf[kb][0], acc0);
                    acc1 = mfma16(wB[kb][1], bf[kb][1], acc1);
                    acc0 = mfma16(wB[kb][2], bf[kb][2], acc0);
                    acc1 = mfma16(wB[kb][3], bf[kb][3], acc1);
                }
            }
            gb = acc0 + acc1;
#pragma unroll
            for (int i = 0; i < 4; ++i) if (r0 + i >= P.D) gb[i] = 0.f;
            if constexpr (kPhase == 1) {
                st4(Bq.UB1 + co, r0, P.D, true, vec, gb);
#pragma unroll
                for (int i = 0; i < 4; ++i) dot += gb[i] * f0v[i];
            } else {
                const f32x4 u0b = ld_tile(Bq.xbar + co, r0, P.D, colok, false);
                st_tile(Bq.xbar + co, r0, P.D, colok, false, u0b + gb);
            }
        }
        if (!colok) tau = 0.f;
        dot = wave_sum_f(dot); tau = wave_sum_f(tau);
        __syncthreads();
        if (lane == 0) { RED[w] = dot; RED[8 + w] = tau; }
        __syncthreads();
        if (tid == 0) {
            float sa = 0.f, ta = 0.f;
            for (int i = 0; i < Q.WT; ++i) { sa += RED[i]; ta += RED[8 + i]; }
            if constexpr (kPhase == 1) { float* o = Bq.ipart + (size_t)wg * 4; o[0] = sa; o[1] = ta; o[2] = 0.f; o[3] = 0.f; }
            else { float* o = Bq.ipart + ((size_t)P.nwg + wg) * 4; o[0] = ta; o[1] = 0.f; o[2] = 0.f; o[3] = 0.f; }
        }
    }
}

}
```

### regneuralde.jl_amd/csrc/rnde_head.h

```cpp
#pragma once
#include "rnde_device.h"

namespace rnde {

constexpr int kHeadMaxC = 16;

constexpr int kHeadRowsPerThread = 4;
template <int CC>
__global__ __launch_bounds__(256) void rnde_head_col_kernel(const float* __restrict__ u, const float* __restrict__ p3,
                                                            const float* __restrict__ y, int D, int C, int B,
                                                            float* __restrict__ logits_out, float* __restrict__ ubar,
                                                            float* __restrict__ delta, float* __restrict__ ce_col) {
    constexpr int NC = CC ? CC : kHeadMaxC;
    if (CC) C = CC;
    __shared__ float red[4][kHeadMaxC];
    const int tid = threadIdx.x, lane = tid & 63, w = tid >> 6;
    const int c = blockIdx.x;
    const float* W = p3;
    const float* b = p3 + (size_t)C * D;
    const float* uc = u + (size_t)c * D;
    float wv[kHeadRowsPerThread][NC], uv[kHeadRowsPerThread];
#pragma unroll
    for (int k = 0; k < kHeadRowsPerThread; ++k) {
        const int d = tid + 256 * k;
// ... 48 lines not shown
                                                              int D, int C, int B, float* __restrict__ partial) {
    const int d = blockIdx.x * 256 + threadIdx.x;
    const int ch = blockIdx.y;
    const int per = (B + kHeadChunks - 1) / kHeadChunks;
    const int c0 = ch * per, c1 = min(B, c0 + per);
    if (d >= D) return;
    float acc[kHeadMaxC];
#pragma unroll
    for (int i = 0; i < kHeadMaxC; ++i) acc[i] = 0.f;
    for (int cb = c0; cb < c1; cb += 8) {
        float uv[8];
#pragma unroll
        for (int j = 0; j < 8; ++j) uv[j] = cb + j < c1 ? u[(size_t)(cb + j) * D + d] : 0.f;
#pragma unroll
        for (int j = 0; j < 8; ++j) {
            const int c = cb + j < c1 ? cb + j : c0;
#pragma unroll
            for (int i = 0; i < kHeadMaxC; ++i) if (i < C) acc[i] = fmaf(delta[(size_t)c * C + i], uv[j], acc[i]);
        }
    }
    float* o = partial + (size_t)ch * C * D;
    for (int i = 0; i < C; ++i) o[(size_t)d * C + i] = acc[i];
}
static __global__ __launch_bounds__(256) void rnde_head_reduce_kernel(const float* __restrict__ partial, const float* __restrict__ delta,
                                                               const float* __restrict__ ce_col, int D, int C, int B,
                                                               float* __restrict__ p3bar, float* __restrict__ ce_out) {
    const int i = blockIdx.x * 256 + threadIdx.x;
    if (i < C * D) {
        float v[kHeadChunks];
#pragma unroll
        for (int ch = 0; ch < kHeadChunks; ++ch) v[ch] = partial[(size_t)ch * C * D + i];
        float s = 0.f;
#pragma unroll
        for (int ch = 0; ch < kHeadChunks; ++ch) s += v[ch];
        p3bar[i] = s;
    }
    if (blockIdx.x == gridDim.x - 1) {
        const int lane = threadIdx.x & 63, w = threadIdx.x >> 6;
        for (int k = w; k < C; k += 4) {
            float s = 0.f;
            for (int c = lane; c < B; c += 64) s += delta[(size_t)c * C + k];
            s = wave_sum_f(s);
            if (lane == 0) p3bar[(size_t)C * D + k] = s;
        }
        if (w == 3) {
            float s = 0.f;
            for (int c = lane; c < B; c += 64) s += ce_col[c];
            s = wave_sum_f(s);
            if (lane == 0) *ce_out = s / (float)B;
        }
    }
}

static __global__ __launch_bounds__(256) void rnde_momentum_kernel(float* __restrict__ p, const float* __restrict__ g, float* __restrict__ v,
                                                            long long len, float inv_decay, float eta, float rho) {
    const long long i = (long long)blockIdx.x * 256 + threadIdx.x;
    if (i >= len) return;
    const float gs = g[i] * inv_decay;
    const float vn = rho * v[i] - eta * gs;
    v[i] = vn;
    p[i] = p[i] + vn;
}

static __global__ __launch_bounds__(256) void rnde_adam_kernel(float* __restrict__ p, const float* __restrict__ g, float* __restrict__ m, float* __restrict__ v,
                                                        long long len, float gscale, float eta, float b1, float b2, float bc1, float bc2, float eps) {
    const long long i = (long long)blockIdx.x * 256 + threadIdx.x;
    if (i >= len) return;
    const float gs = g[i] * gscale;
    const float mn = b1 * m[i] + (1.f - b1) * gs;
    const float vn = b2 * v[i] + (1.f - b2) * gs * gs;
    m[i] = mn; v[i] = vn;
    p[i] = p[i] - mn / bc1 / (sqrtf(vn / bc2) + eps) * eta;
}

}
```

### regneuralde.jl_amd/csrc/rnde_node.h

```cpp
#pragma once
#include "../../include/rnde.h"
#include "rnde_fwd.h"
#include "rnde_bwd.h"
#include "rnde_stage.h"
#include "rnde_bstage.h"
#include "rnde_stage_persist2.h"
#include "rnde_bstage_persist.h"
#include "rnde_solve_sync.h"
#include "rnde_binit_stage.h"
#include "rnde_head.h"
#include "rnde_chain.h"
#include "rk_tables.h"
#include "rnde_bchain.h"
#include "rnde_chainmw.h"
#include "rnde_bchainmw.h"

#include <chrono>
#include <algorithm>
#include <atomic>
#include <cmath>
#include <cstdlib>
#include <cstdio>
#include <cstring>
#include <functional>
#include <string>
#include <vector>

static hipError_t rnde_malloc(void** p, size_t bytes) {
    const hipError_t e = (hipMalloc)(p, bytes);
    const bool poison = getenv("RNDE_POISON") != nullptr;
    if (e == hipSuccess && poison && bytes) (void)hipMemset(*p, 0xFF, bytes);
    return e;
}
#define hipMalloc(p, n) rnde_malloc((void**)(p), (n))

extern "C" hipError_t rnde_launch_stage_solve(const void* stage_params, const void* persist_sync, const void* solve_sync, int act2, int x3, hipStream_t s);
extern "C" hipError_t rnde_launch_x3_pack(const float* p, void* x3B, void* x3D, void* x3Bt, void* x3Dt, int D, int H, int MT, int WT, int R, int HT, hipStream_t s);
using namespace rnde;

struct rnde_node {
    rnde_node_config cfg{};
    int D = 0, H = 0, P = 0, BT = 8, act2 = 1;
    int Bpad_max = 0, nwg_max = 0;
    int engine = 1;
    ChainGeo cg{}; float* cfrags = nullptr; int NKD = 0, chain_alt = 0;
    int chain_ga = 0;
    size_t chain_lds_f = 0, chain_lds_b = 0;
    rnde_comm* couple = nullptr; int couple_batch = 0, couple_world = 1;
    int rk_tab = 0; RkTab rk{};
    int mw_slot = 0;
    int mw_clean = 0, mw_retry_after = 8;
    int mw_solve = 1; unsigned long long* mw_xch = nullptr; unsigned* mw_xcc = nullptr; unsigned* mw_abort = nullptr; unsigned* h_mw_chk = nullptr; unsigned mw_epoch = 0;
    int mw_bsweep = 1; int* mw_bargs = nullptr; int* h_mw_bargs = nullptr; unsigned* h_mw_bchk = nullptr; bool pending_bsweep = false; int bsweep_nt = 0; bool bsweep_global = false;
    int rk_S = 7, rk_order = 5;
    int mw_lat = 0;
    int mw = 0; MwGeo mg{}; float* mw_tab = nullptr; float* mw_slab = nullptr; long long mw_slab_evals = 0; size_t mw_lds_f = 0, mw_lds_b = 0;
    float* cslab = nullptr; size_t cslab_floats = 0; float* ev_t = nullptr; float* h_ev_t = nullptr;
    int sMT = 0, sWT = 0, sR = 0, sHT = 0, sK2b = 0, sKHb = 0;
    f32x4 *spwB = nullptr, *spwD = nullptr, *spwBt = nullptr, *spwDt = nullptr;
    float* slab2 = nullptr;
    size_t stage_lds = 0;
    float* head_ws = nullptr; size_t head_ws_floats = 0;
    std::function<rnde_status(hipStream_t)> after_solve; hipEvent_t ev_host = nullptr; bool rev_packed = false;
    float* cg_ws = nullptr; size_t cg_ws_floats = 0; std::vector<float> cg_sv;
    float* sv_t_dev = nullptr; size_t sv_cap = 0; std::vector<float> saveat;
    float* replay_dev = nullptr; size_t replay_cap = 0; const float* replay_host = nullptr; int n_replay = 0;
    int wgrad_side_pct = 30, stage_generic = 0;
    int persist_clean = 0, persist_retry_after = 8, persist_fallbacks = 0;
    int persist2 = -1;
    int persist = 0, persist_spins = kPersistMaxSpins; int tslab_Bpad = -1; size_t tslab_bytes = 0; float* tslab = nullptr; unsigned *pabort = nullptr, *pxcc = nullptr; unsigned* h_pchk = nullptr;
    int stage_solve = 1; unsigned long long* sxch = nullptr; unsigned s_epoch = 0; int one_launch_solves = 0;
    int x3 = 0; void *x3B = nullptr, *x3D = nullptr, *x3Bt = nullptr, *x3Dt = nullptr; bool x3_packed = false, x3_fwd = false;
    hipStream_t wstream = nullptr;
    std::vector<hipEvent_t> wevents;
    float *f0 = nullptr, *h0 = nullptr, *u1 = nullptr, *f1 = nullptr, *h1 = nullptr, *arena = nullptr;
    float* xcopy = nullptr;
    long long arena_recs = 0, rec_stride = 0;
    float* pcopy = nullptr;
    StepState *ctl = nullptr, *ctl_final = nullptr;
    unsigned char *mbox = nullptr, *h_mbox = nullptr; size_t mbox_meta_off = 0;
    StepMeta* meta = nullptr;
    InitRec* initrec = nullptr;
    float *errpart = nullptr, *initpart = nullptr;
    BwdBuffers bw{};
    StepState* h_ctl = nullptr;
    StepMeta* h_meta = nullptr;
    InitRec* h_init = nullptr;
    float* h_scal = nullptr;
    int B = 0, Bpad = 0, nwg = 0, n_att = 0, predicted = 0;
    float t0 = 0, t1 = 0;
    bool have_tape = false;
    bool pending_bwd = false;
    float* diag_buf = nullptr;
    std::vector<int> sv_index;
    int n_saveval = 0;
    int timing = 0; hipEvent_t tev[5] = {nullptr, nullptr, nullptr, nullptr, nullptr}; bool tev_fwd = false, tev_bwd = false;
    std::string err;
};

#define HIPCHK(h, call)                                                                              \
    do {                                                                                             \
        hipError_t e__ = (call);                                                                     \
        if (e__ != hipSuccess) {                                                                     \
            (h)->err = std::string(#call) + ": " + hipGetErrorString(e__);                           \
            return RNDE_ERR_HIP;                                                                     \
        }                                                                                            \
    } while (0)

static const rnde_status RNDE_INTERNAL_RETRY = static_cast<rnde_status>(100);
StepParams make_params(rnde_node* h, const float* x, int B, float t0, float t1, int tape);
MwParams make_mw_params(rnde_node* h, const StepParams& P);
ChainParams make_chain_params(rnde_node* h, const StepParams& P);
rnde_status couple_sum(rnde_node* h, float* partials, long long count, hipStream_t s);
hipError_t stage_pack(rnde_node* h, const float* p, f32x4* dst, int which, int MTrows, int Kb, hipStream_t st);
rnde_status stage_pack_all(rnde_node* h, const float* p_dev, hipStream_t s, const float* x_src = nullptr, long long x_floats = 0);
hipError_t slab_prepare(rnde_node* h, int Bpad, hipStream_t s);
void persist_check_enqueue(rnde_node* h, int grid, hipStream_t s);
bool persist_check_result(rnde_node* h, int C, int R, hipStream_t s);
bool bsweep_failed(rnde_node* h, hipStream_t s);
rnde_status forward_impl(rnde_node* h, const float* x_dev, const float* p_dev, int32_t B, float t0, float t1,
                         float* u_out_dev, const float* saveat_host, int32_t n_saveat, float* sv_out_dev,
                         int64_t* nfe_out, float* saveval_host, int32_t* n_saveval_out, int32_t keep_tape, void* stream);
```

### regneuralde.jl_amd/csrc/rnde_reverse.hip

```cpp
#include "rnde_node.h"
#include "rnde_wgradx.h"

static rnde_status chain_bwd_run(rnde_node* h, const float* u_bar_dev, const float* saveval_bar_host, float* x_bar_dev,
                                 float* p_bar_dev, float* tspan_bar_host, hipStream_t s, bool sync = true, float* tspan_bar_dev = nullptr);
static rnde_status bwd_run(rnde_node* h, const float* u_bar_dev, const float* saveval_bar_host, float* x_bar_dev,
                           float* p_bar_dev, float* tspan_bar_host, hipStream_t s, bool sync = true, float* tspan_bar_dev = nullptr);


extern "C" rnde_status rnde_node_backward_async(rnde_node* h, const float* u_bar_dev, const float* saveval_bar_host, float* x_bar_dev,
                                                float* p_bar_dev, float* tspan_bar_dev, void* stream) {
    if (!h) return RNDE_ERR_BAD_ARG;
    if (!h->have_tape) { h->err = "no recorded forward"; return RNDE_ERR_NO_TAPE; }
    if (h->engine == 3) return chain_bwd_run(h, u_bar_dev, saveval_bar_host, x_bar_dev, p_bar_dev, nullptr, (hipStream_t)stream, false, tspan_bar_dev);
    return bwd_run(h, u_bar_dev, saveval_bar_host, x_bar_dev, p_bar_dev, nullptr, (hipStream_t)stream, false, tspan_bar_dev);
}

extern "C" rnde_status rnde_node_backward(rnde_node* h, const float* u_bar_dev, const float* saveval_bar_host,
                                          float* x_bar_dev, float* p_bar_dev, float* tspan_bar_host, void* stream) {
    if (!h) return RNDE_ERR_BAD_ARG;
    if (!h->have_tape) { h->err = "no recorded forward"; return RNDE_ERR_NO_TAPE; }
    if (h->engine == 3) return chain_bwd_run(h, u_bar_dev, saveval_bar_host, x_bar_dev, p_bar_dev, tspan_bar_host, (hipStream_t)stream);
    return bwd_run(h, u_bar_dev, saveval_bar_host, x_bar_dev, p_bar_dev, tspan_bar_host, (hipStream_t)stream);
}
extern "C" rnde_status rnde_node_backward_host(rnde_node* h, const float* u_bar, const float* saveval_bar, float* x_bar,
// ... 271 lines not shown
            eig_coefs(n, c1, c2);
            const double qo = pow((double)h->h_meta[n].qold_in, (double)kBeta2);
            if (h->persist == 1) {
                PersistSync Y{h->tslab, h->pabort, h->pxcc, h->persist_spins};
                HIPCHK(h, slab_prepare(h, Q.F.Bpad, s));
                const dim3 pgrid(8 * BQ.R * ((BQ.C + 7) / 8));
                const bool fix = BQ.WT == 7 && BQ.HT == 7 && BQ.KHb == 7 && BQ.MT == 49 && BQ.R == 7 && h->D == 784 && h->H == 100 && !h->stage_generic;
                if (fix) {
                    const size_t flds = h->stage_lds + (size_t)(RNDE_BSTAGE_HDMA ? 1 : 0) * 6 * 7 * 2 * 1024;
                    static DeviceOnce attr;
                    if (attr.need()) {
                        HIPCHK(h, hipFuncSetAttribute((const void*)rnde_bstage_attempt_kernel<1, 1>, hipFuncAttributeMaxDynamicSharedMemorySize, 160 * 1024));
                        HIPCHK(h, hipFuncSetAttribute((const void*)rnde_bstage_attempt_kernel<0, 1>, hipFuncAttributeMaxDynamicSharedMemorySize, 160 * 1024));
                        attr.done();
                    }
                    const bool x3 = h->x3_packed && h->x3Bt && h->x3Dt && !getenv("RNDE_X3_REV_OFF");
                    if (x3) {
                        const size_t xlds = sizeof(float) * ((size_t)2 * kX3ImageFloats + 64) + (size_t)(RNDE_BSTAGE_HDMA ? 1 : 0) * 6 * 7 * 2 * 1024;
                        static DeviceOnce attr3;
                        if (attr3.need()) {
#define RNDE_X3_ATTR(A, E) HIPCHK(h, hipFuncSetAttribute((const void*)rnde_bstage_attempt_kernel<A, 1, 1, E>, hipFuncAttributeMaxDynamicSharedMemorySize, 160 * 1024));
                            RNDE_X3_ATTR(1, 0) RNDE_X3_ATTR(1, 1) RNDE_X3_ATTR(1, 2) RNDE_X3_ATTR(1, 3) RNDE_X3_ATTR(0, 0) RNDE_X3_ATTR(0, 1) RNDE_X3_ATTR(0, 2) RNDE_X3_ATTR(0, 3)
#undef RNDE_X3_ATTR
                            attr3.done();
                        }
                        const int ex = (h->saveat.empty() ? 0 : 1) | (h->cfg.regularize >= RNDE_REG_STIFF ? 2 : 0);
#define RNDE_X3_LAUNCH(A, E) hipLaunchKernelGGL((rnde_bstage_attempt_kernel<A, 1, 1, E>), pgrid, blk, xlds, s, BQ, n, h->h_meta[n], c1, c2, sv_lo[n], sv_hi[n], Y, qo, b.h_svb[n])
                        if (h->act2) { if (ex == 0) RNDE_X3_LAUNCH(1, 0); else if (ex == 1) RNDE_X3_LAUNCH(1, 1); else if (ex == 2) RNDE_X3_LAUNCH(1, 2); else RNDE_X3_LAUNCH(1, 3); }
                        else { if (ex == 0) RNDE_X3_LAUNCH(0, 0); else if (ex == 1) RNDE_X3_LAUNCH(0, 1); else if (ex == 2) RNDE_X3_LAUNCH(0, 2); else RNDE_X3_LAUNCH(0, 3); }
#undef RNDE_X3_LAUNCH
                    } else if (h->act2) hipLaunchKernelGGL((rnde_bstage_attempt_kernel<1, 1>), pgrid, blk, flds, s, BQ, n, h->h_meta[n], c1, c2, sv_lo[n], sv_hi[n], Y, qo, b.h_svb[n]);
                    else hipLaunchKernelGGL((rnde_bstage_attempt_kernel<0, 1>), pgrid, blk, flds, s, BQ, n, h->h_meta[n], c1, c2, sv_lo[n], sv_hi[n], Y, qo, b.h_svb[n]);
                } else if (h->act2) hipLaunchKernelGGL((rnde_bstage_attempt_kernel<1, 0>), pgrid, blk, h->stage_lds, s, BQ, n, h->h_meta[n], c1, c2, sv_lo[n], sv_hi[n], Y, qo, b.h_svb[n]);
                else hipLaunchKernelGGL((rnde_bstage_attempt_kernel<0, 0>), pgrid, blk, h->stage_lds, s, BQ, n, h->h_meta[n], c1, c2, sv_lo[n], sv_hi[n], Y, qo, b.h_svb[n]);
                if ((st = couple_sum(h, b.bpart + (size_t)(n & 1) * Q.bpart_n * 4, 4LL * Q.bpart_n, s)) != RNDE_OK) return st;
                if (pre_reduce && n > 0) hipLaunchKernelGGL(rnde_bpart_reduce_kernel, dim3(1), dim3(64), 0, s, Q, n, bsum);
                if (n >= n_att - side_att && (hi_att - n >= group || n == n_att - side_att)) {
                    st = wgrad_group(2 + 6 * n, 2 + 6 * hi_att, true);
                    if (st != RNDE_OK) return st;
                    hi_att = n;
                }
                continue;
            }
            if (h->act2) hipLaunchKernelGGL((rnde_bstage_kernel<1, BM_START>), grid, blk, h->stage_lds, s, BQ, n, 0, h->h_meta[n], c1, c2, sv_lo[n], sv_hi[n], qo);
            else hipLaunchKernelGGL((rnde_bstage_kernel<0, BM_START>), grid, blk, h->stage_lds, s, BQ, n, 0, h->h_meta[n], c1, c2, sv_lo[n], sv_hi[n], qo);
            for (int j = 6; j >= 1; --j) {
                if (h->act2) hipLaunchKernelGGL((rnde_bstage_kernel<1, BM_STAGE>), grid, blk, h->stage_lds, s, BQ, n, j, h->h_meta[n], c1, c2, sv_lo[n], sv_hi[n], qo);
                else hipLaunchKernelGGL((rnde_bstage_kernel<0, BM_STAGE>), grid, blk, h->stage_lds, s, BQ, n, j, h->h_meta[n], c1, c2, sv_lo[n], sv_hi[n], qo);
            }
            if ((st = couple_sum(h, b.bpart + (size_t)(n & 1) * Q.bpart_n * 4, 4LL * Q.bpart_n, s)) != RNDE_OK) return st;
        }
        HIPCHK(h, hipGetLastError());
        {
            if (h->act2) {
                hipLaunchKernelGGL((rnde_binit_stage_kernel<1, 0>), grid, blk, h->stage_lds, s, BQ);
                hipLaunchKernelGGL((rnde_binit_stage_kernel<1, 1>), grid, blk, h->stage_lds, s, BQ);
            } else {
                hipLaunchKernelGGL((rnde_binit_stage_kernel<0, 0>), grid, blk, h->stage_lds, s, BQ);
                hipLaunchKernelGGL((rnde_binit_stage_kernel<0, 1>), grid, blk, h->stage_lds, s, BQ);
            }
            if ((st = couple_sum(h, Q.ipart, 4LL * Q.F.nwg, s)) != RNDE_OK) return st;
            if (h->act2) {
                hipLaunchKernelGGL((rnde_binit_stage_kernel<1, 2>), grid, blk, h->stage_lds, s, BQ);
                hipLaunchKernelGGL((rnde_binit_stage_kernel<1, 3>), grid, blk, h->stage_lds, s, BQ);
            } else {
                hipLaunchKernelGGL((rnde_binit_stage_kernel<0, 2>), grid, blk, h->stage_lds, s, BQ);
                hipLaunchKernelGGL((rnde_binit_stage_kernel<0, 3>), grid, blk, h->stage_lds, s, BQ);
            }
            if ((st = couple_sum(h, Q.ipart + 4LL * Q.F.nwg, 4LL * Q.F.nwg, s)) != RNDE_OK) return st;
            hipLaunchKernelGGL(rnde_bfin_kernel, dim3(1), dim3(64), 0, s, Q);
            HIPCHK(h, hipGetLastError());
        }
    }
    if (h->timing) HIPCHK(h, hipEventRecord(h->tev[3], s));
    st = wgrad_group(0, 2 + 6 * hi_att, false);
    if (st != RNDE_OK) return st;
    if (used_side) {
        hipEvent_t ev = h->wevents[64];
        HIPCHK(h, hipEventRecord(ev, h->wstream));
        HIPCHK(h, hipStreamWaitEvent(s, ev, 0));
    }
    if (cur1 > 16 && cur2 > 16) {
        const long long len1 = (long long)h->H * (h->D + 2), len2 = (long long)h->D * (h->H + 2);
        const size_t seg_r = std::max((size_t)len1, (size_t)len2);
        float* r1 = b.slab_r; float* r2 = b.slab_r + 16 * seg_r;
        const int pg1 = (cur1 + 15) / 16, g1 = (cur1 + pg1 - 1) / pg1, pg2 = (cur2 + 15) / 16, g2 = (cur2 + pg2 - 1) / pg2;
        const int grid = (int)std::min<long long>((std::max(len1, len2) + 255) / 256, 2048);
        ReducePair A{{{slab1, r1, len1, cur1, pg1}, {slab2w, r2, len2, cur2, pg2}}};
        hipLaunchKernelGGL(rnde_wgrad_reduce_pair, dim3(grid, std::max(g1, g2), 2), dim3(256), 0, s, A);
        ReducePair Bp{{{r1, p_bar_dev, len1, g1, g1}, {r2, p_bar_dev + (size_t)h->H * (h->D + 2), len2, g2, g2}}};
        hipLaunchKernelGGL(rnde_wgrad_reduce_pair, dim3(grid, 1, 2), dim3(256), 0, s, Bp);
        HIPCHK(h, hipGetLastError());
    } else {
        st = launch_wgrad_reduce(h, slab1, cur1, h->H, h->D, p_bar_dev, s);
        if (st != RNDE_OK) return st;
        st = launch_wgrad_reduce(h, slab2w, cur2, h->D, h->H, p_bar_dev + (size_t)h->H * (h->D + 2), s);
        if (st != RNDE_OK) return st;
    }
    if (h->timing) { HIPCHK(h, hipEventRecord(h->tev[4], s)); h->tev_bwd = true; }
#ifdef RNDE_DIAG
    if (h->engine == 2 && h->persist == 1 && getenv("RNDE_DIAG_BWD")) {
        unsigned long long hst[64] = {0};
        hipStreamSynchronize(s);
        hipMemcpy(hst, h->diag_buf, sizeof(hst), hipMemcpyDeviceToHost);
        fprintf(stderr, "persistent reverse attempt (workgroup 0 thread 0, cycles): START %lld (entry->weights issued %lld, ->w1t %lld, ->array loads issued %lld, finish_attempt_scalars %lld, scalar chain %lld, vector part %lld), its phase D + put %lld\n", (long long)(hst[1]-hst[0]), (long long)(hst[43]-hst[0]), (long long)(hst[44]-hst[43]), (long long)(hst[40]-hst[44]), (long long)(hst[41]-hst[40]), (long long)(hst[42]-hst[41]), (long long)(hst[1]-hst[42]), (long long)(hst[2]-hst[1]));
        for (int st = 0; st < 6; ++st) { const unsigned long long* q = hst + 3 + 5 * st; const unsigned long long prev = st == 0 ? hst[2] : hst[7 + 5 * (st - 1)];
            fprintf(stderr, "  stage j=%d: poll %lld A %lld B %lld C %lld D+put %lld\n", 6 - st, (long long)(q[0]-prev), (long long)(q[1]-q[0]), (long long)(q[2]-q[1]), (long long)(q[3]-q[2]), st < 5 ? (long long)(q[4]-q[3]) : 0LL); }
        fprintf(stderr, "  total %lld cycles to the end of stage 1, END (reduction of the 21 partial sums) %lld; in START's vector part the wait for the record's k arrays %lld\n",
                (long long)(hst[34]-hst[0]), (long long)(hst[35]-hst[34]), (long long)(hst[45]-hst[42]));
    }
#endif
    if (!sync) {
        if (tspan_bar_dev) HIPCHK(h, hipMemcpyAsync(tspan_bar_dev, b.tspan_out, 8, hipMemcpyDeviceToDevice, s));
        h->have_tape = false;
        h->pending_bwd = (h->engine == 2 && h->persist == 1);
        return RNDE_OK;
    }
    HIPCHK(h, hipMemcpyAsync(h->h_scal, b.tspan_out, 8, hipMemcpyDeviceToHost, s));
    if (h->engine == 2) persist_check_enqueue(h, h->sR * (Q.F.Bpad / 16), s);
    HIPCHK(h, hipStreamSynchronize(s));
// ... 353 lines not shown
    }
    HIPCHK(h, e);
    const int n_units = n_evals * Q.ntiles;
    const int chunks = std::max(1, std::min(96, n_units / 8));
    const int per_chunk = (n_units + chunks - 1) / chunks;
    hipLaunchKernelGGL(rnde_chain_wgrad_kernel, dim3(G.n_layers, chunks), dim3(64 * kCW), 0, s, Q, (const float*)h->ev_t, n_units, per_chunk, b.slab, h->P);
    HIPCHK(h, hipGetLastError());
    {
        const long long len = h->P;
        const int grid = (int)std::min<long long>((len + 255) / 256, 2048);
        if (chunks <= 16) hipLaunchKernelGGL(rnde_wgrad_reduce, dim3(grid, 1), dim3(256), 0, s, (const float*)b.slab, chunks, chunks, len, p_bar_dev);
        else {
            const int per_group = (chunks + 15) / 16, groups = (chunks + per_group - 1) / per_group;
            hipLaunchKernelGGL(rnde_wgrad_reduce, dim3(grid, groups), dim3(256), 0, s, (const float*)b.slab, chunks, per_group, len, b.slab_r);
            hipLaunchKernelGGL(rnde_wgrad_reduce, dim3(grid, 1), dim3(256), 0, s, (const float*)b.slab_r, groups, groups, len, p_bar_dev);
        }
        HIPCHK(h, hipGetLastError());
    }
    h->have_tape = false;
    if (!sync) {
        if (tspan_bar_dev) HIPCHK(h, hipMemcpyAsync(tspan_bar_dev, b.tspan_out, 8, hipMemcpyDeviceToDevice, s));
        return RNDE_OK;
    }
    HIPCHK(h, hipMemcpyAsync(h->h_scal, b.tspan_out, 8, hipMemcpyDeviceToHost, s));
    HIPCHK(h, hipStreamSynchronize(s));
    if (tspan_bar_host) { tspan_bar_host[0] = h->h_scal[0]; tspan_bar_host[1] = h->h_scal[1]; }
    return RNDE_OK;
}

extern "C" rnde_status rnde_adam_step(float* p_dev, const float* g_dev, float* m_dev, float* v_dev, int64_t len, int64_t t, float eta, float beta1,
                                      float beta2, float eps, float gscale, void* stream) {
    if (!p_dev || !g_dev || !m_dev || !v_dev || len < 0 || t < 1) return RNDE_ERR_BAD_ARG;
    if (len == 0) return RNDE_OK;
    const float bc1 = (float)(1.0 - pow((double)beta1, (double)t)), bc2 = (float)(1.0 - pow((double)beta2, (double)t));
    hipLaunchKernelGGL(rnde::rnde_adam_kernel, dim3((unsigned)((len + 255) / 256)), dim3(256), 0, (hipStream_t)stream, p_dev, g_dev, m_dev, v_dev,
                       (long long)len, gscale, eta, beta1, beta2, bc1, bc2, eps);
    return hipGetLastError() == hipSuccess ? RNDE_OK : RNDE_ERR_HIP;
}
extern "C" rnde_status rnde_momentum_step_scaled(float* p_dev, const float* g_dev, float* v_dev, int64_t len, int64_t n, float gamma,
                                                 float eta, float rho, float gscale, void* stream);
extern "C" rnde_status rnde_momentum_step(float* p_dev, const float* g_dev, float* v_dev, int64_t len, int64_t n, float gamma,
                                          float eta, float rho, void* stream) {
    return rnde_momentum_step_scaled(p_dev, g_dev, v_dev, len, n, gamma, eta, rho, 1.0f, stream);
}
extern "C" rnde_status rnde_momentum_step_scaled(float* p_dev, const float* g_dev, float* v_dev, int64_t len, int64_t n, float gamma,
                                                 float eta, float rho, float gscale, void* stream) {
    if (!p_dev || !g_dev || !v_dev || len < 0 || n < 1) return RNDE_ERR_BAD_ARG;
    if (len == 0) return RNDE_OK;
    const float inv_decay = gscale / (1.0f + gamma * (float)n);
    hipLaunchKernelGGL(rnde::rnde_momentum_kernel, dim3((unsigned)((len + 255) / 256)), dim3(256), 0, (hipStream_t)stream, p_dev, g_dev,
                       v_dev, (long long)len, inv_decay, eta, rho);
    return hipGetLastError() == hipSuccess ? RNDE_OK : RNDE_ERR_HIP;
}
```

### regneuralde.jl_amd/csrc/rnde_stage.h

```cpp
#pragma once
#include "rnde_fwd.h"

namespace rnde {

constexpr int kSCB = 16;
constexpr int kSMaxW = 8;
constexpr int kSMaxHT = 8;

struct StageParams {
    StepParams F;
    const float* p;
    const f32x4* pwB;
    const f32x4* pwD;
    float* slab;
    int MT, WT, R, C, HT, K2b;
    int Bpad16;
};

__device__ __forceinline__ int kperm(int k) { return (k & ~15) | ((k & 3) << 2) | ((k >> 2) & 3); }

__device__ __forceinline__ f32x4 mfma16(float a, float b, f32x4 c) {
    return __builtin_amdgcn_mfma_f32_16x16x4f32(a, b, c, 0, 0, 0);
}
__device__ __forceinline__ float add_square_unfused(float acc, float d) {
#pragma clang fp contract(off)
    const float m = d * d;
    return acc + m;
}
__device__ __forceinline__ f32x4 fma4(float s, f32x4 a, f32x4 c) { return __builtin_elementwise_fma((f32x4){s, s, s, s}, a, c); }

__device__ __forceinline__ f32x4 stage_pack_elem(const float* __restrict__ p, int which, int D, int H, int Kb, long long i) {
    const float* W1 = p;
    const float* b1 = W1 + (size_t)H * (D + 1);
    const float* W2 = b1 + H;
    const float* b2 = W2 + (size_t)D * (H + 1);
    const int l = (int)(i & 63);
    const int kb = (int)((i >> 6) % Kb);
    const int T = (int)((i >> 6) / Kb);
    const int m = 16 * T + (l & 15);
    f32x4 v;
#pragma unroll
    for (int q = 0; q < 4; ++q) {
        const int k = 16 * kb + 4 * q + (l >> 4);
        float w = 0.f;
        if (which == 0) { if (m < D) w = k <= H ? W2[(size_t)k * D + m] : (k == H + 1 ? b2[m] : 0.f); }
        else if (which == 1) { if (m < H && k < D) w = W1[(size_t)k * H + m]; }
        else if (which == 2) { if (m < D && k < H) w = W1[(size_t)m * H + k]; }
        else { if (m <= H && k < D) w = W2[(size_t)m * D + k]; }
        v[q] = w;
    }
    return v;
}
static __global__ void rnde_stage_pack_kernel(const float* __restrict__ p, f32x4* __restrict__ dst, int which, int D, int H,
                                       int MTrows, int Kb) {
    const long long total = (long long)MTrows * Kb * 64;
    for (long long i = blockIdx.x * (long long)blockDim.x + threadIdx.x; i < total; i += (long long)gridDim.x * blockDim.x)
        dst[i] = stage_pack_elem(p, which, D, H, Kb, i);
}

struct PackJob { void* dst; const float* src; long long total; int kind, which, kdim, pad; };
struct PackJobs { PackJob j[8]; };
static __global__ void rnde_pack_all_kernel(const float* __restrict__ p, const PackJobs J, int D, int H) {
    const PackJob job = J.j[blockIdx.y];
    for (long long i = blockIdx.x * (long long)blockDim.x + threadIdx.x; i < job.total; i += (long long)gridDim.x * blockDim.x) {
        if (job.kind == 0) ((f32x4*)job.dst)[i] = stage_pack_elem(p, job.which, D, H, job.kdim, i);
        else if (job.kind == 2) ((float*)job.dst)[i] = (job.src ? job.src : p)[i];
        else ((f32x4*)job.dst)[i] = ((const f32x4*)(job.src ? job.src : p))[i];
    }
}

__device__ __forceinline__ void dense_points(const StepParams& P, const RecLayout& L, const float* Rp, float tp, float dtp_, float tnew,
                                             int lo, int hi, size_t co, int gcol, int r0, bool colok, bool vec) {
    const f32x4 up = ld_tile(Rp + L.upc() + co, r0, P.D, true, vec);
    f32x4 k[7];
    k[0] = ld_tile(Rp + L.k1c() + co, r0, P.D, true, vec);
#pragma unroll
    for (int j = 1; j < 7; ++j) k[j] = ld_tile(Rp + L.k(j + 1) + co, r0, P.D, true, vec);
    const f32x4 un = ld_tile(Rp + L.unew() + co, r0, P.D, true, vec);
    for (int idx = lo; idx < hi; ++idx) {
        const float ts = P.sv_t[idx];
        f32x4 o = un;
        if (ts != tnew) {
            float b[7];
            dense_weights((ts - tp) / dtp_, b);
            f32x4 acc = b[0] * k[0];
#pragma unroll
            for (int j = 1; j < 7; ++j) acc += b[j] * k[j];
            o = up + dtp_ * acc;
        }
        st_tile(P.sv_out + ((size_t)gcol * P.nsave + idx) * P.D, r0, P.D, colok, vec && ((P.D & 3) == 0), o);
    }
}

enum { SM_START = 0, SM_STAGE = 1, SM_LAST = 2, SM_I1 = 3, SM_I2 = 4, SM_I3 = 5, SM_I4 = 6, SM_FEVAL1 = 7, SM_FEVAL2 = 8 };

__device__ __forceinline__ f32x4 ld4(const float* colbase, int r0, int D, bool ok, bool vec) { return ld_tile(colbase, r0, D, ok, vec); }
__device__ __forceinline__ void st4(float* colbase, int r0, int D, bool ok, bool vec, f32x4 v) { st_tile(colbase, r0, D, ok, vec, v); }

template <int ACT2, int MODE>
__global__ __launch_bounds__(64 * kSMaxW) void rnde_stage_kernel(const StageParams Q, const int n, const int s) {
    const StepParams& P = Q.F;
    extern __shared__ __attribute__((aligned(16))) float smem[];
    const int KH = 16 * Q.K2b + 4, KG = 16 * Q.WT + 4;
    float* HL = smem;
    float* GL = HL + kSCB * KH;
    float* RED = GL + kSCB * KG;
    const int tid = threadIdx.x, lane = tid & 63;
    const int w = __builtin_amdgcn_readfirstlane(tid >> 6);
    const int rb = blockIdx.x / Q.C, ct = blockIdx.x - rb * Q.C;
    const int col = lane & 15, gcol = ct * kSCB + col;
    const bool colok = gcol < P.B;
    const bool vec = (P.D & 3) == 0;
    const bool writer = (blockIdx.x == 0 && tid == 0);
    const int T = rb * Q.WT + w;
    const int r0 = 16 * T + 4 * (lane >> 4);
    const bool tile_ok = T < Q.MT;
    const RecLayout L{(long long)P.D * P.Bpad, (long long)P.H * P.Bpad};
    constexpr bool kHasA = (MODE == SM_STAGE || MODE == SM_LAST || MODE == SM_I2 || MODE == SM_I4 || MODE == SM_FEVAL2);
    constexpr bool kHasD = (MODE == SM_START || MODE == SM_STAGE || MODE == SM_I1 || MODE == SM_I3 || MODE == SM_FEVAL1);

#ifdef RNDE_DIAG
#define SSTAMP(i) do { if (MODE == SM_STAGE && s == 3 && P.dbg_out && blockIdx.x == 0 && lane == 0) ((unsigned long long*)P.dbg_out)[(w * 8 + (i))] = clock64(); } while (0)
#else
#define SSTAMP(i) do { } while (0)
#endif
    SSTAMP(0);
    StepState S0;
    if constexpr (MODE == SM_STAGE || MODE == SM_LAST) S0 = P.ctl[n & 1];
    f32x4 c_up = {0.f, 0.f, 0.f, 0.f}, c_un = {0.f, 0.f, 0.f, 0.f}, c_k[6];
    bool c_early = false;
    if constexpr (MODE == SM_STAGE || MODE == SM_LAST) {
        if (P.tape && tile_ok) {
            const float* Rn = P.arena + (long long)n * P.rec_stride;
            const size_t co = (size_t)gcol * P.D;
            c_up = ld4(Rn + L.upc() + co, r0, P.D, true, vec);
            c_k[0] = ld4(Rn + L.k1c() + co, r0, P.D, true, vec);
#pragma unroll
            for (int j = 1; j < 6; ++j) if (j < s) c_k[j] = ld4(Rn + L.k(j + 1) + co, r0, P.D, true, vec);
            if constexpr (MODE == SM_LAST) c_un = ld4(Rn + L.unew() + co, r0, P.D, true, vec);
            c_early = true;
        }
    }
    f32x4 wB[kSMaxHT];
    f32x4 wD[kSMaxW];
    if constexpr (kHasA) {
#pragma unroll
        for (int kb = 0; kb < kSMaxHT; ++kb)
            if (kb < Q.K2b && tile_ok) wB[kb] = Q.pwB[((size_t)T * Q.K2b + kb) * 64 + lane];
    }
    if constexpr (kHasD) {
#pragma unroll
        for (int kb = 0; kb < kSMaxW; ++kb)
            if (kb < Q.WT && w < Q.HT && rb * Q.WT + kb < Q.MT) wD[kb] = Q.pwD[((size_t)w * Q.MT + rb * Q.WT + kb) * 64 + lane];
    }

    f32x4 zs = {0.f, 0.f, 0.f, 0.f};
    f32x4 zr[kSMaxW];
    float w1t_own[4] = {0.f, 0.f, 0.f, 0.f}, b1_own[4] = {0.f, 0.f, 0.f, 0.f};
    if constexpr (kHasA) {
#pragma unroll
        for (int i = 0; i < 4; ++i) {
            const int hr = 16 * w + 4 * (lane >> 4) + i;
            if (hr < P.H) { w1t_own[i] = Q.p[(size_t)P.H * P.D + hr]; b1_own[i] = Q.p[(size_t)P.H * (P.D + 1) + hr]; }
        }
        const int par0 = (MODE == SM_STAGE || MODE == SM_LAST) ? (s & 1) : 0;
        const f32x4* sl0 = (const f32x4*)Q.slab + (((size_t)par0 * Q.C + ct) * Q.R) * Q.HT * 64;
        if (w < Q.HT) {
#pragma unroll
            for (int r = 0; r < kSMaxW; ++r) if (r < Q.R) zr[r] = sl0[((size_t)r * Q.HT + w) * 64 + lane];
        }
    }

    float t = P.t0, dt = 0.f;
    int live = -1, rec = 0;
    if constexpr (MODE == SM_START) {
        const StepState S = advance_state(P, n, lane, writer, &P.ctl[n & 1]);
        if (P.nsave > 0) {
            const int lo = (n == 0) ? 0 : P.ctl[(n - 1) & 1].next_save, hi = S.next_save;
            if (hi > lo && tile_ok) {
                if (n == 0) {
                    st_tile(P.sv_out + (size_t)gcol * P.nsave * P.D, r0, P.D, colok, vec,
                            ld_tile(P.x + (size_t)gcol * P.D, r0, P.D, colok, P.xvec != 0));
                } else {
                    const StepState pv = P.ctl[(n - 1) & 1];
                    const float dtp_ = (P.t1 - pv.t < pv.dtp) ? (P.t1 - pv.t) : pv.dtp;
                    const float* Rp = P.arena + (long long)S.live * P.rec_stride;
                    dense_points(P, L, Rp, pv.t, dtp_, S.t, lo, hi, (size_t)gcol * P.D, gcol, r0, colok, vec);
                }
            }
        }
        if (S.done) return;
        t = S.t; dt = (!P.forced && (P.t1 - S.t < S.dtp)) ? (P.t1 - S.t) : S.dtp; live = S.live;
    } else if constexpr (MODE == SM_STAGE || MODE == SM_LAST) {
        const StepState S = S0;
        if (S.done) return;
        t = S.t; dt = (!P.forced && (P.t1 - S.t < S.dtp)) ? (P.t1 - S.t) : S.dtp; live = S.live;
    }
    if constexpr (MODE == SM_START || MODE == SM_STAGE || MODE == SM_LAST) rec = P.tape ? n + P.rec_shift : (live == 0 ? 1 : 0);
    float* R = P.arena + (long long)rec * P.rec_stride;
    const float* upsrc = P.x; const float* k1p = P.f0; bool upok = colok, upvec = P.xvec != 0;
    if (live >= 0) { const float* Rl = P.arena + (long long)live * P.rec_stride; upsrc = Rl + L.unew(); k1p = Rl + L.k(7); upok = true; upvec = vec; }

    if constexpr (kHasA) {
        if (w < Q.HT) {
            const int par0 = (MODE == SM_STAGE || MODE == SM_LAST) ? (s & 1) : 0;
            const f32x4* sl0 = (const f32x4*)Q.slab + (((size_t)par0 * Q.C + ct) * Q.R) * Q.HT * 64;
#pragma unroll
            for (int r = 0; r < kSMaxW; ++r) if (r < Q.R) zs += zr[r];
            for (int r = kSMaxW; r < Q.R; ++r) zs += sl0[((size_t)r * Q.HT + w) * 64 + lane];
        }
    }
    if constexpr (MODE == SM_START || MODE == SM_STAGE || MODE == SM_LAST) {
        if (tile_ok && !c_early) {
            c_up = ld4(upsrc + (size_t)gcol * P.D, r0, P.D, upok, upvec);
            c_k[0] = ld4(k1p + (size_t)gcol * P.D, r0, P.D, true, vec);
            if constexpr (MODE != SM_START) {
#pragma unroll
                for (int j = 1; j < 6; ++j) if (j < s) c_k[j] = ld4(R + L.k(j + 1) + (size_t)gcol * P.D, r0, P.D, true, vec);
            }
            if constexpr (MODE == SM_LAST) c_un = ld4(R + L.unew() + (size_t)gcol * P.D, r0, P.D, true, vec);
        }
    }

    float dt0 = 0.f;
    if constexpr (MODE == SM_I3) {
        const double N = (double)P.D * (double)P.Bn;
        const double s0 = sum_partials(P.initpart, P.nwg, lane), s1 = sum_partials(P.initpart + P.nwg, P.nwg, lane);
        const float d0 = (float)sqrt(s0 / N), d1 = (float)sqrt(s1 / N), dtmax = P.t1 - P.t0;
        int c0 = 0, cl = 0;
        if (d0 < 1e-5f || d1 < 1e-5f) { dt0 = 1e-6f; c0 = 1; } else dt0 = (d0 / d1) / 100.f;
        if (dtmax < dt0) { dt0 = dtmax; cl = 1; }
        if (writer) { P.initrec->d0 = d0; P.initrec->d1 = d1; P.initrec->dt0 = dt0; P.initrec->dt0_const = c0; P.initrec->dt0_clamped = cl; }
    }
    if constexpr (MODE == SM_I4) dt0 = P.initrec->dt0;

    float ts = t;
    float* hdst = nullptr; float* kdst = nullptr;
    if constexpr (MODE == SM_STAGE || MODE == SM_LAST) { ts = fmaf(kTsC[s], dt, t); hdst = R + L.h(s + 1); kdst = R + L.k(s + 1); }
    if constexpr (MODE == SM_I2) { ts = P.t0; hdst = P.h0; kdst = P.f0; }
    if constexpr (MODE == SM_I4) { ts = P.t0 + dt0; hdst = P.h1; kdst = P.f1; }
    if constexpr (MODE == SM_FEVAL2) { ts = P.forced_t; }

    f32x4 kv = {0.f, 0.f, 0.f, 0.f};
    SSTAMP(1);
    if constexpr (kHasA) {

        const float* W1t = Q.p + (size_t)P.H * P.D;
        const float* b1 = Q.p + (size_t)P.H * (P.D + 1);
        const int par = (MODE == SM_STAGE || MODE == SM_LAST) ? (s & 1) : 0;
        const f32x4* sl = (const f32x4*)Q.slab + (((size_t)par * Q.C + ct) * Q.R) * Q.HT * 64;
        for (int ht = w; ht < Q.HT; ht += Q.WT) {
            f32x4 z = zs;
            if (ht != w) {
                z = (f32x4){0.f, 0.f, 0.f, 0.f};
                for (int r = 0; r < Q.R; ++r) z += sl[((size_t)r * Q.HT + ht) * 64 + lane];
            }
            const int h0 = 16 * ht + 4 * (lane >> 4);
            float pre[4];
#pragma unroll
            for (int i = 0; i < 4; ++i) {
                const int hr = h0 + i;
                pre[i] = (hr < P.H) ? fmaf((ht == w) ? w1t_own[i] : W1t[hr], ts, z[i]) + ((ht == w) ? b1_own[i] : b1[hr]) : 0.f;
            }
            const f32x2 t01 = tanh_fast2((f32x2){pre[0], pre[1]}), t23 = tanh_fast2((f32x2){pre[2], pre[3]});
            const float th4[4] = {t01.x, t01.y, t23.x, t23.y};
#pragma unroll
            for (int i = 0; i < 4; ++i) {
                const int hr = h0 + i;
                float v = 0.f;
                if (hr < P.H) {
                    v = th4[i];
                    if (rb == 0 && hdst) hdst[(size_t)gcol * P.H + hr] = v;
                } else if (hr == P.H) v = ts;
                else if (hr == P.H + 1) v = 1.f;
                if (hr < 16 * Q.K2b) HL[col * KH + kperm(hr)] = v;
            }
        }
        if (Q.K2b > Q.HT) {
            for (int i = tid; i < kSCB * 16 * Q.K2b; i += blockDim.x) {
                const int c = i / (16 * Q.K2b), k = i - c * 16 * Q.K2b;
                if (k >= 16 * Q.HT) HL[c * KH + kperm(k)] = (k == P.H) ? ts : (k == P.H + 1 ? 1.f : 0.f);
            }
        }
        SSTAMP(2);
        __syncthreads();
        SSTAMP(3);
        if (tile_ok) {
            f32x4 acc0 = {0.f, 0.f, 0.f, 0.f}, acc1 = {0.f, 0.f, 0.f, 0.f};
            const float* hb = HL + col * KH + 4 * (lane >> 4);
            f32x4 bf[kSMaxHT];
#pragma unroll
            for (int kb = 0; kb < kSMaxHT; ++kb) if (kb < Q.K2b) bf[kb] = *(const f32x4*)(hb + 16 * kb);
#pragma unroll
            for (int kb = 0; kb < kSMaxHT; ++kb) {
                if (kb < Q.K2b) {
                    acc0 = mfma16(wB[kb][0], bf[kb][0], acc0);
                    acc1 = mfma16(wB[kb][1], bf[kb][1], acc1);
                    acc0 = mfma16(wB[kb][2], bf[kb][2], acc0);
                    acc1 = mfma16(wB[kb][3], bf[kb][3], acc1);
                }
            }
            kv = acc0 + acc1;
            if (ACT2) {
                const f32x2 a01 = tanh_fast2((f32x2){kv[0], kv[1]}), a23 = tanh_fast2((f32x2){kv[2], kv[3]});
                kv = (f32x4){a01.x, a01.y, a23.x, a23.y};
            }
#pragma unroll
            for (int i = 0; i < 4; ++i) kv[i] = (r0 + i < P.D) ? kv[i] : 0.f;
        }
    }

    SSTAMP(4);
    f32x4 v = {0.f, 0.f, 0.f, 0.f};
    float part0 = 0.f, part1 = 0.f, part2 = 0.f;
    if (tile_ok) {
        if constexpr (MODE == SM_START) {
            v = fma4(dt, kFwdShift[0][0] * c_k[0], c_up);
            if (P.tape) st4(R + L.g(2) + (size_t)gcol * P.D, r0, P.D, true, vec, v);
            if (P.tape || P.nsave > 0) {
                st4(R + L.upc() + (size_t)gcol * P.D, r0, P.D, true, vec, c_up);
                st4(R + L.k1c() + (size_t)gcol * P.D, r0, P.D, true, vec, c_k[0]);
            }
        } else if constexpr (MODE == SM_STAGE) {
            st4(kdst + (size_t)gcol * P.D, r0, P.D, true, vec, kv);
            f32x4 acc = tsA_rt(s + 1, 0) * c_k[0];
#pragma unroll
            for (int j = 1; j < 6; ++j) if (j < s) acc = fma4(tsA_rt(s + 1, j), c_k[j], acc);
            acc = fma4(tsA_rt(s + 1, s), kv, acc);
            v = fma4(dt, acc, c_up);
            if (s == 5) st4(R + L.unew() + (size_t)gcol * P.D, r0, P.D, true, vec, v);
            else if (P.tape) st4(R + L.g(s + 2) + (size_t)gcol * P.D, r0, P.D, true, vec, v);
        } else if constexpr (MODE == SM_LAST) {
            st4(kdst + (size_t)gcol * P.D, r0, P.D, true, vec, kv);
            const f32x4 up = c_up, un = c_un;
            f32x4 acc = kTsBt[0] * c_k[0];
#pragma unroll
            for (int j = 1; j < 6; ++j) acc = fma4(kTsBt[j], c_k[j], acc);
            acc = fma4(kTsBt[6], kv, acc);
// ... 16 lines not shown
                            const float d1 = kv[i] - c_k[5][i], d2 = un[i] - g6[i];
                            part1 = add_square_unfused(part1, d1); part2 = add_square_unfused(part2, d2);
                        }
                    }
                }
            }
        } else if constexpr (MODE == SM_I1 || MODE == SM_FEVAL1) {
            v = ld4(P.x + (size_t)gcol * P.D, r0, P.D, colok, P.xvec != 0);
        } else if constexpr (MODE == SM_I2) {
            st4(kdst + (size_t)gcol * P.D, r0, P.D, true, vec, kv);
            const f32x4 xv = ld4(P.x + (size_t)gcol * P.D, r0, P.D, colok, P.xvec != 0);
            if (colok) {
#pragma unroll
                for (int i = 0; i < 4; ++i) {
                    if (r0 + i < P.D) {
                        const float sk = P.abstol + fabsf(xv[i]) * P.reltol;
                        const float a = xv[i] / sk, b = kv[i] / sk;
                        part0 += a * a; part1 += b * b;
                    }
                }
            }
        } else if constexpr (MODE == SM_I3) {
            const f32x4 xv = ld4(P.x + (size_t)gcol * P.D, r0, P.D, colok, P.xvec != 0);
            const f32x4 f0 = ld4(P.f0 + (size_t)gcol * P.D, r0, P.D, true, vec);
            v = xv + dt0 * f0;
            st4(P.u1 + (size_t)gcol * P.D, r0, P.D, true, vec, v);
        } else if constexpr (MODE == SM_I4) {
            st4(kdst + (size_t)gcol * P.D, r0, P.D, true, vec, kv);
            const f32x4 xv = ld4(P.x + (size_t)gcol * P.D, r0, P.D, colok, P.xvec != 0);
            const f32x4 f0 = ld4(P.f0 + (size_t)gcol * P.D, r0, P.D, true, vec);
            if (colok) {
#pragma unroll
                for (int i = 0; i < 4; ++i) {
                    if (r0 + i < P.D) {
                        const float sk = P.abstol + fabsf(xv[i]) * P.reltol;
                        const float a = (kv[i] - f0[i]) / sk;
                        part0 += a * a;
                    }
                }
            }
        } else if constexpr (MODE == SM_FEVAL2) {
            st4(P.dbg_out + (size_t)gcol * P.D, r0, P.D, colok, false, kv);
        }
    }

    if constexpr (kHasD) {
#pragma unroll
        for (int i = 0; i < 4; ++i) GL[col * KG + kperm(16 * w + 4 * (lane >> 4) + i)] = (tile_ok && r0 + i < P.D) ? v[i] : 0.f;
        SSTAMP(5);
        __syncthreads();
        SSTAMP(6);
        const int par = (MODE == SM_START) ? 1 : (MODE == SM_STAGE ? ((s + 1) & 1) : 0);
        f32x4* sl = (f32x4*)Q.slab + ((((size_t)par * Q.C + ct) * Q.R + rb) * Q.HT) * 64;
        const float* gbp = GL + col * KG + 4 * (lane >> 4);
        f32x4 bg[kSMaxW];
#pragma unroll
        for (int kb = 0; kb < kSMaxW; ++kb) if (kb < Q.WT) bg[kb] = *(const f32x4*)(gbp + 16 * kb);
        if (w < Q.HT) {
            f32x4 acc0 = {0.f, 0.f, 0.f, 0.f}, acc1 = {0.f, 0.f, 0.f, 0.f};
#pragma unroll
            for (int kb = 0; kb < kSMaxW; ++kb) {
                if (kb < Q.WT && rb * Q.WT + kb < Q.MT) {
                    acc0 = mfma16(wD[kb][0], bg[kb][0], acc0);
                    acc1 = mfma16(wD[kb][1], bg[kb][1], acc1);
                    acc0 = mfma16(wD[kb][2], bg[kb][2], acc0);
                    acc1 = mfma16(wD[kb][3], bg[kb][3], acc1);
                }
            }
            sl[(size_t)w * 64 + lane] = acc0 + acc1;
        }
        for (int ht = w + Q.WT; ht < Q.HT; ht += Q.WT) {
            f32x4 acc0 = {0.f, 0.f, 0.f, 0.f}, acc1 = {0.f, 0.f, 0.f, 0.f};
#pragma unroll
            for (int kb = 0; kb < kSMaxW; ++kb) {
                if (kb < Q.WT && rb * Q.WT + kb < Q.MT) {
                    const f32x4 a = Q.pwD[((size_t)ht * Q.MT + rb * Q.WT + kb) * 64 + lane];
                    acc0 = mfma16(a[0], bg[kb][0], acc0);
                    acc1 = mfma16(a[1], bg[kb][1], acc1);
                    acc0 = mfma16(a[2], bg[kb][2], acc0);
                    acc1 = mfma16(a[3], bg[kb][3], acc1);
                }
            }
            sl[(size_t)ht * 64 + lane] = acc0 + acc1;
        }
        SSTAMP(7);
    }

    if constexpr (MODE == SM_LAST || MODE == SM_I2 || MODE == SM_I4) {
        part0 = wave_sum_f(part0); part1 = wave_sum_f(part1); part2 = wave_sum_f(part2);
        if (lane == 0) { RED[w] = part0; RED[8 + w] = part1; RED[16 + w] = part2; }
        __syncthreads();
        if (tid == 0) {
            float sa = 0.f, sb = 0.f, sc = 0.f;
            for (int i = 0; i < Q.WT; ++i) { sa += RED[i]; sb += RED[8 + i]; sc += RED[16 + i]; }
            if constexpr (MODE == SM_LAST) {
                float* ep = P.errpart + (size_t)(n & 1) * 3 * P.nwg;
                ep[blockIdx.x] = sa; ep[P.nwg + blockIdx.x] = sb; ep[2 * P.nwg + blockIdx.x] = sc;
            }
            else if constexpr (MODE == SM_I2) { P.initpart[blockIdx.x] = sa; P.initpart[P.nwg + blockIdx.x] = sb; }
            else P.initpart[2 * P.nwg + blockIdx.x] = sa;
        }
    }
}

static __global__ __launch_bounds__(256) void rnde_stage_finish_kernel(const StageParams Q, const int n, float* __restrict__ u_out) {
    const StepParams& P = Q.F;
    const int tid = threadIdx.x, lane = tid & 63;
    const bool writer = (blockIdx.x == 0 && tid == 0);
    const StepState S = n < 0 ? *P.ctl_final : advance_state(P, n, lane, writer, P.ctl_final);
    const RecLayout L{(long long)P.D * P.Bpad, (long long)P.H * P.Bpad};
    if (P.nsave > 0 && n > 0) {
        const StepState pv = P.ctl[(n - 1) & 1];
        const int lo = pv.next_save, hi = S.next_save;
        if (hi > lo && !pv.done) {
            const float dtp_ = (P.t1 - pv.t < pv.dtp) ? (P.t1 - pv.t) : pv.dtp;
            const float* Rp = P.arena + (long long)S.live * P.rec_stride;
            const bool vec = (P.D & 3) == 0;
            const int ntile = (P.D + 3) / 4;
            for (long long i = blockIdx.x * 256LL + tid; i < (long long)ntile * P.B; i += (long long)gridDim.x * 256) {
                const int gcol = (int)(i / ntile), r0 = 4 * (int)(i % ntile);
                dense_points(P, L, Rp, pv.t, dtp_, S.t, lo, hi, (size_t)gcol * P.D, gcol, r0, true, vec);
            }
        }
    }
    if (!u_out) return;
    const float* src = S.live < 0 ? P.x : P.arena + (long long)S.live * P.rec_stride + L.unew();
    const long long total = (long long)P.D * P.B;
    if (((total & 3) == 0) && (((reinterpret_cast<size_t>(u_out) | reinterpret_cast<size_t>(src)) & 15) == 0)) {
        for (long long i = blockIdx.x * 256LL + tid; i < total / 4; i += (long long)gridDim.x * 256) ((f32x4*)u_out)[i] = ((const f32x4*)src)[i];
    } else {
        for (long long i = blockIdx.x * 256LL + tid; i < total; i += (long long)gridDim.x * 256) u_out[i] = src[i];
    }
}

}
```

### regneuralde.jl_amd/csrc/rnde_stage_persist.h

```cpp
#pragma once
#include "rnde_stage.h"
#include "rnde_x3.h"

#include <type_traits>

namespace rnde {

struct PersistSync {
    float* tslab;
    unsigned* abort_flag;
    unsigned* xcc;
    int max_spins;
};

constexpr int kPersistMaxSpins = 2000000;
typedef unsigned u32x4 __attribute__((ext_vector_type(4)));

constexpr unsigned kSlabEmpty = 0xFFFFFFFFu;
__device__ __forceinline__ int slab_buf(unsigned ex) { return (int)(ex % 3u); }
__device__ __forceinline__ void slab_put(float* tslab, size_t tile_index, int lane, const f32x4& v) {
    u32x4 b = __builtin_bit_cast(u32x4, v);
#pragma unroll
    for (int i = 0; i < 4; ++i) b[i] = b[i] < 0xFFFFFFFEu ? b[i] : 0xFFFFFFFEu;
    ((u32x4*)tslab + tile_index * 64)[lane] = b;
}
__device__ __forceinline__ void slab_clear(float* tslab, size_t tile_index, int lane) {
    const float e = __builtin_bit_cast(float, kSlabEmpty);
    ((f32x4*)tslab + tile_index * 64)[lane] = (f32x4){e, e, e, e};
}
__device__ __forceinline__ void slab_clears_done() { __builtin_amdgcn_s_waitcnt(0x0F70); }
__device__ __forceinline__ bool slab_poll_sum(const PersistSync& Y, int buf, int C, int R, int HT, int ct, int ht, int lane, f32x4& zs) {
    const float* base = Y.tslab + ((((size_t)buf * C + ct) * R) * HT) * 256;
    __amdgpu_buffer_rsrc_t rs = __builtin_amdgcn_make_buffer_rsrc((void*)base, 0, 0x7fffffff, 0x00020000);
    int spins = 0;
    while (true) {
        __asm__ volatile("" ::: "memory");
        u32x4 e[kSMaxW];
#pragma unroll
        for (int r = 0; r < kSMaxW; ++r)
            if (r < R) e[r] = __builtin_amdgcn_raw_buffer_load_b128(rs, ((r * HT + ht) * 64 + lane) * 16, 0, 16);
        float s0 = 0.f, s1 = 0.f, s2 = 0.f, s3 = 0.f;
#pragma unroll
        for (int r = 0; r < kSMaxW; ++r) {
            if (r < R) {
                const f32x4 f = __builtin_bit_cast(f32x4, e[r]);
                s0 += f[0]; s1 += f[1]; s2 += f[2]; s3 += f[3];
            }
        }
        zs = (f32x4){s0, s1, s2, s3};
        const bool clean = !(__builtin_isunordered(s0, s1) || __builtin_isunordered(s2, s3));
        if (__all(clean)) return true;
        unsigned m = 0u;
#pragma unroll
        for (int r = 0; r < kSMaxW; ++r)
            if (r < R) { const unsigned a = e[r][0] > e[r][1] ? e[r][0] : e[r][1], b = e[r][2] > e[r][3] ? e[r][2] : e[r][3]; const unsigned c = a > b ? a : b; m = m > c ? m : c; }
        const bool ok = m != kSlabEmpty;
        if (__all(ok)) return true;
        if (++spins > Y.max_spins || ((spins & 63) == 0 && __hip_atomic_load(Y.abort_flag, __ATOMIC_RELAXED, __HIP_MEMORY_SCOPE_AGENT))) {
            __hip_atomic_store(Y.abort_flag, 1u, __ATOMIC_RELAXED, __HIP_MEMORY_SCOPE_AGENT);
            zs = (f32x4){0.f, 0.f, 0.f, 0.f};
            return false;
        }
    }
}

#ifdef RNDE_DIAG
#define PSTAMP(i) do { if (P.dbg_out && wg == 0 && tid == 0) ((unsigned long long*)P.dbg_out)[i] = clock64(); } while (0)
#define WSTAMP(st, k) do { if (P.dbg_out && wg == 0 && lane == 0) ((unsigned long long*)P.dbg_out)[64 + (((st) - 1) * 8 + w) * 8 + (k)] = clock64(); } while (0)
#else
#define PSTAMP(i) do { } while (0)
#define WSTAMP(st, k) do { } while (0)
#endif

template <int ACT2, int FIX, int X3 = 0>
__global__ __launch_bounds__(64 * kSMaxW) void rnde_stage_attempt_kernel(const StageParams Q, const int n, const PersistSync Y, const void* x3B = nullptr, const void* x3D = nullptr) {
    static_assert(!X3 || FIX, "the X3 form exists for the headline geometry only");
    const StepParams& P = Q.F;
    const int gWT = FIX ? 7 : Q.WT, gHT = FIX ? 7 : Q.HT, gK2b = FIX ? 7 : Q.K2b, gMT = FIX ? 49 : Q.MT, gR = FIX ? 7 : Q.R;
    const int gD = FIX ? 784 : P.D, gH = FIX ? 100 : P.H;
    extern __shared__ __attribute__((aligned(16))) float smem[];
    const int KH = 16 * gK2b + 4, KG = 16 * gWT + 4;
    float* HL = smem;
    float* GL = HL + (X3 ? kX3ImageFloats : kSCB * KH);
    float* RED = GL + (X3 ? kX3ImageFloats : kSCB * KG);
    unsigned short* HX = (unsigned short*)HL;
    unsigned short* GX = (unsigned short*)GL;
    const int tid = threadIdx.x, lane = tid & 63;
    const int w = __builtin_amdgcn_readfirstlane(tid >> 6);
    if (FIX) __builtin_assume(w >= 0 && w < 7);
    const int rb = (blockIdx.x >> 3) % gR, ct = 8 * ((blockIdx.x >> 3) / gR) + (blockIdx.x & 7);
    if (ct >= Q.C) return;
    const int wg = rb * Q.C + ct;
    const int col = lane & 15, gcol = ct * kSCB + col;
    const bool colok = gcol < P.B;
    const bool vec = (gD & 3) == 0;
    const bool writer = (wg == 0 && tid == 0);
    const int T = rb * gWT + w;
    const int r0 = 16 * T + 4 * (lane >> 4);
    const bool tile_ok = FIX ? true : T < gMT;
    const RecLayout L{(long long)gD * P.Bpad, (long long)gH * P.Bpad};
    if (tid == 0) Y.xcc[wg] = __builtin_amdgcn_s_getreg((3 << 11) | (0 << 6) | 20) & 15;

    PSTAMP(0);
    float pre_part[4] = {0.f, 0.f, 0.f, 0.f};
    f32x4 prev_raw[3] = {{0.f, 0.f, 0.f, 0.f}, {0.f, 0.f, 0.f, 0.f}, {0.f, 0.f, 0.f, 0.f}};
    if (n > 0) {
        const f32x4* cp = (const f32x4*)&P.ctl[(n - 1) & 1];
        prev_raw[0] = cp[0]; prev_raw[1] = cp[1]; prev_raw[2] = cp[2];
        partials_request(P.errpart + (size_t)((n - 1) & 1) * 3 * P.nwg, lane, pre_part);
    }
    const bool spec = P.tape && n > 0 && !P.forced && tile_ok;
    f32x4 sp_up = {0.f, 0.f, 0.f, 0.f}, sp_k = {0.f, 0.f, 0.f, 0.f};
    if (spec) {
        const float* Rs = P.arena + (long long)(n - 1) * P.rec_stride;
        sp_up = ld4(Rs + L.unew() + (size_t)gcol * gD, r0, gD, true, vec);
        sp_k = ld4(Rs + L.k(7) + (size_t)gcol * gD, r0, gD, true, vec);
    }
// ... 349 lines not shown
```

### regneuralde.jl_amd/csrc/rnde_x3.h

```cpp
#pragma once
#include <hip/hip_runtime.h>

namespace rnde {

typedef unsigned x3u4 __attribute__((ext_vector_type(4)));
typedef unsigned x3u2 __attribute__((ext_vector_type(2)));
typedef __bf16 x3bf8 __attribute__((ext_vector_type(8)));
typedef float x3f4 __attribute__((ext_vector_type(4)));

constexpr int kX3K = 136;
constexpr int kX3PlaneShorts = 16 * kX3K;
constexpr int kX3ImageFloats = 3 * kX3PlaneShorts / 2;

__device__ __forceinline__ unsigned x3_cvt2(float a, float b) {
    unsigned r;
    asm("v_cvt_pk_bf16_f32 %0, %1, %2" : "=v"(r) : "v"(a), "v"(b));
    return r;
}
#ifndef RNDE_X3_DOT2
#define RNDE_X3_DOT2 0
#endif
typedef __bf16 x3bf2 __attribute__((ext_vector_type(2)));
typedef float x3f2 __attribute__((ext_vector_type(2)));
__device__ __forceinline__ void x3_split2(float x0, float x1, unsigned& hi, unsigned& mid, unsigned& lo) {
// ... 5 lines not shown
    const x3bf2 bl = __builtin_bit_cast(x3bf2, kl), bh = __builtin_bit_cast(x3bf2, kh);
    const x3bf2 h = __builtin_convertvector((x3f2){x0, x1}, x3bf2);
    const float r0 = __builtin_amdgcn_fdot2_f32_bf16(h, bl, x0, false), r1 = __builtin_amdgcn_fdot2_f32_bf16(h, bh, x1, false);
    const x3bf2 m = __builtin_convertvector((x3f2){r0, r1}, x3bf2);
    const float s0 = __builtin_amdgcn_fdot2_f32_bf16(m, bl, r0, false), s1 = __builtin_amdgcn_fdot2_f32_bf16(m, bh, r1, false);
    hi = __builtin_bit_cast(unsigned, h);
    mid = __builtin_bit_cast(unsigned, m);
    lo = __builtin_bit_cast(unsigned, __builtin_convertvector((x3f2){s0, s1}, x3bf2));
#else
    hi = x3_cvt2(x0, x1);
    const float r0 = x0 - __uint_as_float(hi << 16), r1 = x1 - __uint_as_float(hi & 0xFFFF0000u);
    mid = x3_cvt2(r0, r1);
    const float s0 = r0 - __uint_as_float(mid << 16), s1 = r1 - __uint_as_float(mid & 0xFFFF0000u);
    lo = x3_cvt2(s0, s1);
#endif
}
__device__ __forceinline__ void x3_store4(unsigned short* img, int col, int k0, const x3f4& v) {
    unsigned h01, m01, l01, h23, m23, l23;
    x3_split2(v[0], v[1], h01, m01, l01);
    x3_split2(v[2], v[3], h23, m23, l23);
    unsigned short* p = img + col * kX3K + k0;
    *(x3u2*)p = (x3u2){h01, h23};
    *(x3u2*)(p + kX3PlaneShorts) = (x3u2){m01, m23};
    *(x3u2*)(p + 2 * kX3PlaneShorts) = (x3u2){l01, l23};
}
__device__ __forceinline__ x3u4 x3_frag(const unsigned short* img, int pl, int s, int lane) {
    return *(const x3u4*)(img + pl * kX3PlaneShorts + (lane & 15) * kX3K + 32 * s + 8 * (lane >> 4));
}
__device__ __forceinline__ x3f4 x3_mfma(const x3u4& a, const x3u4& b, const x3f4& c) {
    return __builtin_amdgcn_mfma_f32_16x16x32_bf16(__builtin_bit_cast(x3bf8, a), __builtin_bit_cast(x3bf8, b), c, 0, 0, 0);
}
template <int NS>
__device__ __forceinline__ x3f4 x3_tile(const x3u4 (&wa)[NS][3], const unsigned short* img, int lane) {
    x3f4 aL = {0.f, 0.f, 0.f, 0.f}, aN = {0.f, 0.f, 0.f, 0.f}, aM = {0.f, 0.f, 0.f, 0.f}, aH = {0.f, 0.f, 0.f, 0.f};
    x3u4 bh = x3_frag(img, 0, 0, lane), bm = x3_frag(img, 1, 0, lane), bl = x3_frag(img, 2, 0, lane);
#pragma unroll
    for (int s = 0; s < NS; ++s) {
        x3u4 nh = bh, nm = bm, nl = bl;
        if (s + 1 < NS) { nh = x3_frag(img, 0, s + 1, lane); nm = x3_frag(img, 1, s + 1, lane); nl = x3_frag(img, 2, s + 1, lane); }
        __builtin_amdgcn_sched_barrier(0);
        aL = x3_mfma(wa[s][2], bh, aL);
        aM = x3_mfma(wa[s][1], bh, aM);
        aH = x3_mfma(wa[s][0], bh, aH);
        aN = x3_mfma(wa[s][1], bm, aN);
        aL = x3_mfma(wa[s][0], bl, aL);
        aM = x3_mfma(wa[s][0], bm, aM);
        __builtin_amdgcn_sched_barrier(0);
        bh = nh; bm = nm; bl = nl;
    }
    return ((aL + aN) + aM) + aH;
}

struct X3PackDst { x3u4* d[4]; };
static __global__ void rnde_x3_pack_kernel(const float* __restrict__ p, const X3PackDst dst, int D, int H, int MT, int WT, int R, int HT) {
    const float* W1 = p;
    const float* b1 = W1 + (size_t)H * (D + 1);
    const float* W2 = b1 + H;
    const float* b2 = W2 + (size_t)D * (H + 1);
    const long long nB = (long long)MT * 4 * 64, nD = (long long)HT * R * 4 * 64, per = nB + nD;
    const int nimg = dst.d[2] ? 2 : 1;
    for (long long i = blockIdx.x * (long long)blockDim.x + threadIdx.x; i < nimg * per; i += (long long)gridDim.x * blockDim.x) {
        const int rev = (int)(i / per);
        const long long ii = i - rev * per;
        const bool isD = ii >= nB;
        const long long q = isD ? ii - nB : ii;
        const int l = (int)(q & 63), s = (int)((q >> 6) & 3), tile = (int)(q >> 8);
        float wv[8];
#pragma unroll
        for (int j = 0; j < 8; ++j) {
            const int k = 32 * s + 8 * (l >> 4) + j;
            float w = 0.f;
            if (!isD) {
                const int m = 16 * tile + (l & 15);
                if (m < D) {
                    if (!rev) w = k <= H ? W2[(size_t)k * D + m] : (k == H + 1 ? b2[m] : 0.f);
                    else if (k < H) w = W1[(size_t)m * H + k];
                }
            } else {
                const int wt = tile / R, rb = tile % R;
                const int m = 16 * wt + (l & 15), row = 16 * WT * rb + k;
                if (k < 16 * WT && row < D) {
                    if (!rev) { if (m < H) w = W1[(size_t)row * H + m]; }
                    else if (m <= H) w = W2[(size_t)m * D + row];
                }
            }
            wv[j] = w;
        }
        unsigned hi[4], mid[4], lo[4];
#pragma unroll
        for (int j = 0; j < 4; ++j) x3_split2(wv[2 * j], wv[2 * j + 1], hi[j], mid[j], lo[j]);
        x3u4* o = dst.d[2 * rev + (isD ? 1 : 0)] + ((size_t)(tile * 4 + s) * 3) * 64 + l;
        o[0] = (x3u4){hi[0], hi[1], hi[2], hi[3]};
        o[64] = (x3u4){mid[0], mid[1], mid[2], mid[3]};
        o[128] = (x3u4){lo[0], lo[1], lo[2], lo[3]};
    }
}

}
```

Before: 306,900 samples/s.

## Fuse init-step stage pairs into persistent kernels, fold x3 packing and grouped momentum

Replaces the four separate initial-dt stage launches with two pair kernels. Each pair kernel hands partial sums between stages through a polled slab in global memory, which needs two extra slab regions. The x3 weight packing is folded into the existing pack-all launch. The per-parameter momentum updates are batched into a single grouped launch. All of this is meant to cut kernel launch count and per-step host overhead, at the cost of spin-wait synchronisation, more slab memory and extra poll/clear work.

```diff
diff --git a/include/rnde.h b/include/rnde.h
--- a/include/rnde.h
+++ b/include/rnde.h
@@ -93,6 +93,7 @@
                                     float* x_bar, float* p_bar, float* tspan_bar);
 
 rnde_status rnde_node_steps(rnde_node* h, float* steps_host, int32_t capacity, int32_t* n_attempts_out);
+rnde_status rnde_node_init_step(rnde_node* h, float* dt0_out, float* dt_out);
 
 rnde_status rnde_debug_feval(rnde_node* h, const float* u_dev, const float* p_dev, int32_t B, float t,
                              float* out_dev, void* stream);
@@ -138,11 +139,14 @@
                                       float* p2_bar_dev, float* p3_bar_dev, float* x_bar_dev, float* ce_out_dev,
                                       float* reg_out_host, int64_t* nfe_out, rnde_comm* comm, void* stream);
 
+
 rnde_status rnde_momentum_step(float* p_dev, const float* g_dev, float* v_dev, int64_t len, int64_t n, float gamma,
                                float eta, float rho, void* stream);
 
 rnde_status rnde_momentum_step_scaled(float* p_dev, const float* g_dev, float* v_dev, int64_t len, int64_t n, float gamma,
                                       float eta, float rho, float gscale, void* stream);
+rnde_status rnde_momentum_step_groups(int32_t n_groups, float* const* p_dev, const float* const* g_dev, float* const* v_dev,
+                                      const int64_t* len, const int64_t* n, float gamma, float eta, float rho, float gscale, void* stream);
 rnde_status rnde_adam_step(float* p_dev, const float* g_dev, float* m_dev, float* v_dev, int64_t len, int64_t t, float eta, float beta1,
                            float beta2, float eps, float gscale, void* stream);
 rnde_status rnde_adabelief_step(float* p_dev, const float* g_dev, float* m_dev, float* s_dev, int64_t len, float eta, float beta1, float beta2,
diff --git a/regneuralde.jl_amd/_lib.py b/regneuralde.jl_amd/_lib.py
--- a/regneuralde.jl_amd/_lib.py
+++ b/regneuralde.jl_amd/_lib.py
@@ -78,6 +78,8 @@
     L.rnde_node_forward_host.argtypes = [vp, fp, fp, i32, f, f, fp, i64p, fp, i32p, i32]
     L.rnde_node_backward_host.argtypes = [vp, fp, fp, fp, fp, fp]
     L.rnde_node_steps.argtypes = [vp, fp, i32, i32p]
+    if hasattr(L, "rnde_node_init_step"):
+        L.rnde_node_init_step.argtypes = [vp, fp, fp]
     L.rnde_debug_feval.argtypes = [vp, vp, vp, i32, f, vp, vp]
     L.rnde_debug_attempt.argtypes = [vp, vp, vp, vp, i32, f, f, vp, vp, fp, vp]
     L.rnde_bench_attempt.argtypes = [vp, vp, vp, i32, i32, fp, vp]
@@ -102,6 +104,8 @@
     L.rnde_momentum_step.argtypes = [vp, vp, vp, C.c_int64, C.c_int64, f, f, f, vp]
     u64 = C.c_uint64
     L.rnde_momentum_step_scaled.argtypes = [vp, vp, vp, C.c_int64, C.c_int64, f, f, f, f, vp]
+    if hasattr(L, "rnde_momentum_step_groups"):
+        L.rnde_momentum_step_groups.argtypes = [i32, C.POINTER(vp), C.POINTER(vp), C.POINTER(vp), i64p, i64p, f, f, f, f, vp]
     L.rnde_adam_step.argtypes = [vp, vp, vp, vp, C.c_int64, C.c_int64, C.c_float, C.c_float, C.c_float, C.c_float, C.c_float, vp]
     L.rnde_adabelief_step.argtypes = [vp, vp, vp, vp, C.c_int64, f, f, f, f, f, vp]
     L.rnde_moment_loss.argtypes = [vp, vp, vp, i32, i32, i32, vp, vp, vp]
@@ -191,9 +195,9 @@
 
 EXPORTS = ["rnde_version", "rnde_last_error", "rnde_param_count", "rnde_node_create", "rnde_node_destroy",
            "rnde_node_forward", "rnde_node_forward_saveat", "rnde_node_forward_everystep", "rnde_node_forward_replay", "rnde_node_backward", "rnde_node_backward_async", "rnde_node_release_tape", "rnde_node_forward_host",
-           "rnde_node_backward_host", "rnde_node_steps", "rnde_debug_feval", "rnde_debug_attempt",
+           "rnde_node_backward_host", "rnde_node_steps", "rnde_node_init_step", "rnde_debug_feval", "rnde_debug_attempt",
            "rnde_bench_attempt", "rnde_bench_attempt_taped", "rnde_bench_attempt_cold_tape", "rnde_node_set_timing", "rnde_node_timing", "rnde_node_last_attempts", "rnde_node_fallback_count",
-           "rnde_node_launches_per_attempt", "rnde_node_one_launch_solves", "rnde_node_set_matrix_mode", "rnde_node_matrix_mode", "rnde_classifier_head", "rnde_node_classifier_grad", "rnde_momentum_step", "rnde_momentum_step_scaled", "rnde_adam_step",
+           "rnde_node_launches_per_attempt", "rnde_node_one_launch_solves", "rnde_node_set_matrix_mode", "rnde_node_matrix_mode", "rnde_classifier_head", "rnde_node_classifier_grad", "rnde_momentum_step", "rnde_momentum_step_scaled", "rnde_momentum_step_groups", "rnde_adam_step",
            "rnde_comm_unique_id", "rnde_comm_create", "rnde_comm_destroy", "rnde_comm_world", "rnde_comm_last_error", "rnde_comm_library", "rnde_comm_allreduce", "rnde_comm_create_local_group", "rnde_comm_health", "rnde_comm_window_create", "rnde_comm_window_destroy", "rnde_comm_create_peers", "rnde_comm_path", "rnde_node_set_coupling", "rnde_tapes_create", "rnde_tapes_destroy", "rnde_tapes_last_error", "rnde_tapes_in_use", "rnde_tapes_node", "rnde_tapes_forward", "rnde_tapes_backward", "rnde_tapes_release",
            "rnde_nsde_param_count", "rnde_nsde_create", "rnde_nsde_destroy", "rnde_nsde_last_error", "rnde_nsde_forward",
            "rnde_nsde_forward_saveat", "rnde_nsde_forward_everystep", "rnde_nsde_forward_replay", "rnde_nsde_backward", "rnde_nsde_backward_async", "rnde_nsde_classifier_head", "rnde_nsde_classifier_grad", "rnde_nsde_steps", "rnde_nsde_debug_attempt", "rnde_nsde_set_pre_act", "rnde_nsde_moment_grad", "rnde_moment_loss", "rnde_adabelief_step", "rnde_nsde_timing", "rnde_normal_fill", "rnde_latent_create", "rnde_latent_destroy", "rnde_latent_last_error", "rnde_latent_param_counts", "rnde_latent_encode",
diff --git a/regneuralde.jl_amd/classifier.py b/regneuralde.jl_amd/classifier.py
--- a/regneuralde.jl_amd/classifier.py
+++ b/regneuralde.jl_amd/classifier.py
@@ -131,6 +131,24 @@
 
     @torch.no_grad()
     def step(self, grads=None, grad_scale=1.0):
+        gl = [p.grad if grads is None else grads[i] for i, p in enumerate(self.params)]
+        if (len(self.params) > 1 and all(g is not None for g in gl) and all(p.is_cuda and p.device == self.params[0].device for p in self.params)
+                and len(self.params) <= 8 and os.environ.get("RNDE_OPT_FUSE_OFF", "0") in ("", "0")):
+            import ctypes as C
+            from . import _lib
+            L = _lib.lib()
+            if hasattr(L, "rnde_momentum_step_groups"):
+                k = len(self.params)
+                gl = [g.contiguous() for g in gl]
+                st = L.rnde_momentum_step_groups(k, (C.c_void_p * k)(*[p.data_ptr() for p in self.params]), (C.c_void_p * k)(*[g.data_ptr() for g in gl]),
+                                                 (C.c_void_p * k)(*[v.data_ptr() for v in self.v]), (C.c_int64 * k)(*[p.numel() for p in self.params]),
+                                                 (C.c_int64 * k)(*self.n), self.gamma, self.eta, self.rho, float(grad_scale),
+                                                 C.c_void_p(torch.cuda.current_stream(self.params[0].device).cuda_stream))
+                _lib.check(None, st)
+                for i, p in enumerate(self.params):
+                    self.n[i] += 1
+                    p.grad = None
+                return
         for i, p in enumerate(self.params):
             g = p.grad if grads is None else grads[i]
             if g is None:
diff --git a/regneuralde.jl_amd/csrc/rnde.hip b/regneuralde.jl_amd/csrc/rnde.hip
--- a/regneuralde.jl_amd/csrc/rnde.hip
+++ b/regneuralde.jl_amd/csrc/rnde.hip
@@ -376,7 +376,7 @@
     ok &= dm((void**)&h->spwB, (size_t)h->sMT * h->sK2b * 64 * 16) && dm((void**)&h->spwD, (size_t)h->sHT * h->sMT * 64 * 16);
     ok &= dm((void**)&h->spwBt, (size_t)h->sMT * h->sKHb * 64 * 16) && dm((void**)&h->spwDt, (size_t)h->sHT * h->sMT * 64 * 16);
     ok &= dm((void**)&h->slab2, (size_t)2 * (h->Bpad_max / 16) * h->sR * h->sHT * 64 * 16);
-    const size_t tslab_bytes = (size_t)3 * (h->Bpad_max / 16) * h->sR * h->sHT * 64 * 16;
+    const size_t tslab_bytes = (size_t)5 * (h->Bpad_max / 16) * h->sR * h->sHT * 64 * 16;
     h->tslab_bytes = tslab_bytes;
     ok &= dm((void**)&h->tslab, tslab_bytes);
     static_assert(sizeof(StepState) <= 512 && sizeof(InitRec) <= 504, "mailbox layout");
@@ -548,18 +548,41 @@
     };
     add_copy(h->pcopy, nullptr, (long long)h->P);
     if (x_src) add_copy(h->xcopy, x_src, x_floats);
+    const bool x3_here = h->x3 && h->x3B && h->x3D && h->x3Bt && h->x3Dt && h->persist == 1 && !h->stage_generic && !getenv("RNDE_PACK_FUSE_OFF");
+    if (x3_here) {
+        J.x3 = X3PackDst{{(x3u4*)h->x3B, (x3u4*)h->x3D, (x3u4*)h->x3Bt, (x3u4*)h->x3Dt}};
+        J.MT = h->sMT; J.WT = h->sWT; J.R = h->sR; J.HT = h->sHT;
+        add(nullptr, 2LL * (h->sMT + h->sHT * h->sR) * 4 * 64, 4, 0, 0);
+    }
     long long most = 0;
     for (int i = 0; i < n; ++i) most = std::max(most, J.j[i].total);
     const int grid = (int)std::min<long long>((most + 255) / 256, 256);
     hipLaunchKernelGGL(rnde_pack_all_kernel, dim3(grid, n), dim3(256), 0, s, p_dev, J, h->D, h->H);
     HIPCHK(h, hipGetLastError());
     h->rev_packed = true;
+    if (x3_here) { h->x3_fwd = true; h->x3_packed = true; return RNDE_OK; }
     return x3_pack(h, p_dev, true, s);
 }
 hipError_t slab_prepare(rnde_node* h, int Bpad, hipStream_t s) {
     if (h->tslab_Bpad == Bpad) return hipSuccess;
     h->tslab_Bpad = Bpad;
     return hipMemsetAsync(h->tslab, 0xFF, h->tslab_bytes, s);
+}
+float* init_region(const rnde_node* h, int k) { return h->tslab + (size_t)(3 + k) * (h->Bpad_max / 16) * h->sR * h->sHT * 256; }
+hipError_t init_pairs_begin(rnde_node* h, int Bpad, hipStream_t s) {
+    if (hipError_t e = slab_prepare(h, Bpad, s); e != hipSuccess) return e;
+    if (h->init_pairs_open) { if (hipError_t e = hipMemsetAsync(init_region(h, 0), 0xFF, h->tslab_bytes / 5 * 2, s); e != hipSuccess) return e; }
+    h->init_pairs_open = true;
+    return hipSuccess;
+}
+bool init_pairs_on(const rnde_node* h, const char* off_switch) { return h->engine == 2 && h->persist == 1 && !h->stage_generic && !getenv(off_switch); }
+template <int PAIR>
+static hipError_t launch_init_pair(rnde_node* h, const StageParams& Q, hipStream_t st) {
+    PersistSync Y{init_region(h, PAIR), h->pabort, h->pxcc, h->persist_spins};
+    const dim3 grid(8 * Q.R * ((Q.C + 7) / 8)), blk(64 * Q.WT);
+    if (h->act2) hipLaunchKernelGGL((rnde_stage_init_pair_kernel<1, PAIR>), grid, blk, h->stage_lds, st, Q, Y, init_region(h, 1 - PAIR));
+    else hipLaunchKernelGGL((rnde_stage_init_pair_kernel<0, PAIR>), grid, blk, h->stage_lds, st, Q, Y, init_region(h, 1 - PAIR));
+    return hipGetLastError();
 }
 static bool stage_two_tile(const rnde_node* h, const StageParams& Q) {
     const bool fix = Q.WT == 7 && Q.HT == 7 && Q.K2b == 7 && Q.MT == 49 && Q.R == 7 && h->D == 784 && h->H == 100 && !h->stage_generic;
@@ -761,11 +784,19 @@
         if (!keep_tape) { st = stage_pack_weights(h, p_dev, s); if (st != RNDE_OK) return st; }
         SQ = make_stage_params(h, P, keep_tape ? h->pcopy : p_dev);
         if (stage_epart_reduce(h, SQ)) SQ.F.esum = (const double*)(h->errpart + 6 * (size_t)h->nwg_max + 256);
-        HIPCHK(h, launch_stage<SM_I1>(h, SQ, 0, 0, s));
-        HIPCHK(h, launch_stage<SM_I2>(h, SQ, 0, 0, s));
-        if ((st = couple_sum(h, P.initpart, 2LL * P.nwg, s)) != RNDE_OK) return st;
-        HIPCHK(h, launch_stage<SM_I3>(h, SQ, 0, 0, s));
-        HIPCHK(h, launch_stage<SM_I4>(h, SQ, 0, 0, s));
+        if (init_pairs_on(h, "RNDE_INIT_FUSE_OFF")) {
+            HIPCHK(h, init_pairs_begin(h, SQ.Bpad16, s));
+            HIPCHK(h, launch_init_pair<0>(h, SQ, s));
+            if ((st = couple_sum(h, P.initpart, 2LL * P.nwg, s)) != RNDE_OK) return st;
+            HIPCHK(h, launch_init_pair<1>(h, SQ, s));
+            h->init_pairs_open = false;
+        } else {
+            HIPCHK(h, launch_stage<SM_I1>(h, SQ, 0, 0, s));
+            HIPCHK(h, launch_stage<SM_I2>(h, SQ, 0, 0, s));
+            if ((st = couple_sum(h, P.initpart, 2LL * P.nwg, s)) != RNDE_OK) return st;
+            HIPCHK(h, launch_stage<SM_I3>(h, SQ, 0, 0, s));
+            HIPCHK(h, launch_stage<SM_I4>(h, SQ, 0, 0, s));
+        }
         if ((st = couple_sum(h, P.initpart + 2LL * P.nwg, P.nwg, s)) != RNDE_OK) return st;
     }
     int launched = 0;
@@ -1043,6 +1074,13 @@
     return RNDE_OK;
 }
 
+extern "C" rnde_status rnde_node_init_step(rnde_node* h, float* dt0_out, float* dt_out) {
+    if (!h || !h->h_init) return RNDE_ERR_BAD_ARG;
+    if (dt0_out) *dt0_out = h->h_init->dt0;
+    if (dt_out) *dt_out = h->h_init->dt;
+    return RNDE_OK;
+}
+
 extern "C" rnde_status rnde_node_set_timing(rnde_node* h, int32_t on) {
     if (!h) return RNDE_ERR_BAD_ARG;
     if (on && !h->tev[0]) for (auto& e : h->tev) HIPCHK(h, hipEventCreate(&e));
diff --git a/regneuralde.jl_amd/csrc/rnde_binit_stage.h b/regneuralde.jl_amd/csrc/rnde_binit_stage.h
--- a/regneuralde.jl_amd/csrc/rnde_binit_stage.h
+++ b/regneuralde.jl_amd/csrc/rnde_binit_stage.h
@@ -3,24 +3,21 @@
 
 namespace rnde {
 
-template <int ACT2, int STEP>
-__global__ __launch_bounds__(64 * kSMaxW) void rnde_binit_stage_kernel(const BStageParams Q) {
+template <int ACT2, int STEP, int HO>
+__device__ __forceinline__ bool binit_stage_body(const BStageParams& Q, float* smem, const int rb, const int ct, const int wg, const PersistSync* Y, float* clear_slab) {
 #pragma clang fp contract(off)
     const BwdParams& Bq = Q.B;
     const StepParams& P = Bq.F;
-    extern __shared__ __attribute__((aligned(16))) float smem[];
     const int KZ = 16 * Q.KHb + 4, KG = 16 * Q.WT + 4;
     float* ZL = smem;
     float* GL = ZL + kSCB * KZ;
     float* RED = GL + kSCB * KG;
     const int tid = threadIdx.x, lane = tid & 63;
     const int w = __builtin_amdgcn_readfirstlane(tid >> 6);
-    const int rb = blockIdx.x / Q.C, ct = blockIdx.x - rb * Q.C;
-    const int wg = blockIdx.x;
     const int col = lane & 15, gcol = ct * kSCB + col;
     const bool colok = gcol < P.B;
     const bool vec = (P.D & 3) == 0;
-    const bool writer = (blockIdx.x == 0 && tid == 0);
+    const bool writer = (wg == 0 && tid == 0);
     const int T = rb * Q.WT + w;
     const int r0 = 16 * T + 4 * (lane >> 4);
     const bool tile_ok = T < Q.MT;
@@ -112,6 +109,8 @@
         for (int i = 0; i < 4; ++i) GL[col * KG + kperm(16 * w + 4 * (lane >> 4) + i)] = tile_ok ? v[i] : 0.f;
         __syncthreads();
         f32x4* sl = (f32x4*)Q.slab + ((((size_t)par * Q.C + ct) * Q.R + rb) * Q.HT) * 64;
+        const size_t tile0 = ((size_t)ct * Q.R + rb) * Q.HT;
+        if constexpr (HO) { for (int ht = w; ht < Q.HT; ht += Q.WT) slab_clear(clear_slab, tile0 + ht, lane); }
         const float* gbp = GL + col * KG + 4 * (lane >> 4);
         f32x4 bg[kSMaxW];
 #pragma unroll
@@ -127,7 +126,8 @@
                     acc1 = mfma16(wD[kb][3], bg[kb][3], acc1);
                 }
             }
-            sl[(size_t)w * 64 + lane] = acc0 + acc1;
+            if constexpr (HO) slab_put(Y->tslab, tile0 + w, lane, acc0 + acc1);
+            else sl[(size_t)w * 64 + lane] = acc0 + acc1;
         }
         for (int ht = w + Q.WT; ht < Q.HT; ht += Q.WT) {
             f32x4 acc0 = {0.f, 0.f, 0.f, 0.f}, acc1 = {0.f, 0.f, 0.f, 0.f};
@@ -141,9 +141,10 @@
                     acc1 = mfma16(a[3], bg[kb][3], acc1);
                 }
             }
-            sl[(size_t)ht * 64 + lane] = acc0 + acc1;
-        }
-        return;
+            if constexpr (HO) slab_put(Y->tslab, tile0 + ht, lane, acc0 + acc1);
+            else sl[(size_t)ht * 64 + lane] = acc0 + acc1;
+        }
+        return true;
     } else {
         f32x4 wB[kSMaxHT];
 #pragma unroll
@@ -155,9 +156,11 @@
         const f32x4* sl = (const f32x4*)Q.slab + (((size_t)par * Q.C + ct) * Q.R) * Q.HT * 64;
         f32x4 f0v = {0.f, 0.f, 0.f, 0.f};
         if (kPhase == 1 && tile_ok) f0v = ld4(P.f0 + co, r0, P.D, true, vec);
+        bool dead = false;
         for (int ht = w; ht < Q.HT; ht += Q.WT) {
             f32x4 z = {0.f, 0.f, 0.f, 0.f};
-            for (int r = 0; r < Q.R; ++r) z += sl[((size_t)r * Q.HT + ht) * 64 + lane];
+            if constexpr (HO) { if (!dead) dead = !slab_poll_sum(*Y, 0, Q.C, Q.R, Q.HT, ct, ht, lane, z); }
+            else for (int r = 0; r < Q.R; ++r) z += sl[((size_t)r * Q.HT + ht) * 64 + lane];
             const int h0 = 16 * ht + 4 * (lane >> 4);
 #pragma unroll
             for (int i = 0; i < 4; ++i) {
@@ -179,7 +182,9 @@
                 if (k >= 16 * Q.HT) ZL[c * KZ + kperm(k)] = 0.f;
             }
         }
-        __syncthreads();
+        if constexpr (HO) { if (dead && lane == 0) RED[24] = 1.f; }
+        __syncthreads();
+        if constexpr (HO) { if (RED[24] != 0.f) return false; }
         f32x4 gb = {0.f, 0.f, 0.f, 0.f};
         if (tile_ok) {
             f32x4 acc0 = {0.f, 0.f, 0.f, 0.f}, acc1 = {0.f, 0.f, 0.f, 0.f};
@@ -219,7 +224,29 @@
             if constexpr (kPhase == 1) { float* o = Bq.ipart + (size_t)wg * 4; o[0] = sa; o[1] = ta; o[2] = 0.f; o[3] = 0.f; }
             else { float* o = Bq.ipart + ((size_t)P.nwg + wg) * 4; o[0] = ta; o[1] = 0.f; o[2] = 0.f; o[3] = 0.f; }
         }
+        return true;
     }
 }
-
-}
+template <int ACT2, int STEP>
+__global__ __launch_bounds__(64 * kSMaxW) void rnde_binit_stage_kernel(const BStageParams Q) {
+    extern __shared__ __attribute__((aligned(16))) float smem[];
+    const int rb = blockIdx.x / Q.C, ct = blockIdx.x - rb * Q.C;
+    binit_stage_body<ACT2, STEP, 0>(Q, smem, rb, ct, (int)blockIdx.x, nullptr, nullptr);
+}
+
+template <int ACT2, int PAIR>
+__global__ __launch_bounds__(64 * kSMaxW) void rnde_binit_stage_pair_kernel(const BStageParams Q, const PersistSync Y, float* clear_slab) {
+    extern __shared__ __attribute__((aligned(16))) float smem[];
+    const int rb = (blockIdx.x >> 3) % Q.R, ct = 8 * ((blockIdx.x >> 3) / Q.R) + (blockIdx.x & 7);
+    if (ct >= Q.C) return;
+    const int wg = rb * Q.C + ct;
+    float* RED = smem + kSCB * (16 * Q.KHb + 4) + kSCB * (16 * Q.WT + 4);
+    if (threadIdx.x == 0) {
+        Y.xcc[wg] = __builtin_amdgcn_s_getreg((3 << 11) | (0 << 6) | 20) & 15;
+        RED[24] = 0.f;
+    }
+    binit_stage_body<ACT2, 2 * PAIR, 1>(Q, smem, rb, ct, wg, &Y, clear_slab);
+    binit_stage_body<ACT2, 2 * PAIR + 1, 1>(Q, smem, rb, ct, wg, &Y, nullptr);
+}
+
+}
diff --git a/regneuralde.jl_amd/csrc/rnde_head.h b/regneuralde.jl_amd/csrc/rnde_head.h
--- a/regneuralde.jl_amd/csrc/rnde_head.h
+++ b/regneuralde.jl_amd/csrc/rnde_head.h
@@ -124,14 +124,25 @@
     }
 }
 
+__device__ __forceinline__ void momentum_update(float* __restrict__ p, const float* __restrict__ g, float* __restrict__ v, long long i, float inv_decay, float eta, float rho) {
+    const float gs = g[i] * inv_decay;
+    const float vn = rho * v[i] - eta * gs;
+    v[i] = vn;
+    p[i] = p[i] + vn;
+}
 static __global__ __launch_bounds__(256) void rnde_momentum_kernel(float* __restrict__ p, const float* __restrict__ g, float* __restrict__ v,
                                                             long long len, float inv_decay, float eta, float rho) {
     const long long i = (long long)blockIdx.x * 256 + threadIdx.x;
     if (i >= len) return;
-    const float gs = g[i] * inv_decay;
-    const float vn = rho * v[i] - eta * gs;
-    v[i] = vn;
-    p[i] = p[i] + vn;
+    momentum_update(p, g, v, i, inv_decay, eta, rho);
+}
+constexpr int kMomentumMaxGroups = 8;
+struct MomentumGroups { float* p[kMomentumMaxGroups]; const float* g[kMomentumMaxGroups]; float* v[kMomentumMaxGroups]; long long len[kMomentumMaxGroups]; float inv_decay[kMomentumMaxGroups]; };
+static __global__ __launch_bounds__(256) void rnde_momentum_groups_kernel(const MomentumGroups G, float eta, float rho) {
+    const int k = blockIdx.y;
+    const long long i = (long long)blockIdx.x * 256 + threadIdx.x;
+    if (i >= G.len[k]) return;
+    momentum_update(G.p[k], G.g[k], G.v[k], i, G.inv_decay[k], eta, rho);
 }
 
 static __global__ __launch_bounds__(256) void rnde_adam_kernel(float* __restrict__ p, const float* __restrict__ g, float* __restrict__ m, float* __restrict__ v,
diff --git a/regneuralde.jl_amd/csrc/rnde_node.h b/regneuralde.jl_amd/csrc/rnde_node.h
--- a/regneuralde.jl_amd/csrc/rnde_node.h
+++ b/regneuralde.jl_amd/csrc/rnde_node.h
@@ -68,6 +68,7 @@
     int wgrad_side_pct = 30, stage_generic = 0;
     int persist_clean = 0, persist_retry_after = 8, persist_fallbacks = 0;
     int persist2 = -1;
+    bool init_pairs_open = false;
     int persist = 0, persist_spins = kPersistMaxSpins; int tslab_Bpad = -1; size_t tslab_bytes = 0; float* tslab = nullptr; unsigned *pabort = nullptr, *pxcc = nullptr; unsigned* h_pchk = nullptr;
     int stage_solve = 1; unsigned long long* sxch = nullptr; unsigned s_epoch = 0; int one_launch_solves = 0;
     int x3 = 0; void *x3B = nullptr, *x3D = nullptr, *x3Bt = nullptr, *x3Dt = nullptr; bool x3_packed = false, x3_fwd = false;
@@ -115,6 +116,9 @@
 hipError_t stage_pack(rnde_node* h, const float* p, f32x4* dst, int which, int MTrows, int Kb, hipStream_t st);
 rnde_status stage_pack_all(rnde_node* h, const float* p_dev, hipStream_t s, const float* x_src = nullptr, long long x_floats = 0);
 hipError_t slab_prepare(rnde_node* h, int Bpad, hipStream_t s);
+float* init_region(const rnde_node* h, int k);
+hipError_t init_pairs_begin(rnde_node* h, int Bpad, hipStream_t s);
+bool init_pairs_on(const rnde_node* h, const char* off_switch);
 void persist_check_enqueue(rnde_node* h, int grid, hipStream_t s);
 bool persist_check_result(rnde_node* h, int C, int R, hipStream_t s);
 bool bsweep_failed(rnde_node* h, hipStream_t s);
diff --git a/regneuralde.jl_amd/csrc/rnde_reverse.hip b/regneuralde.jl_amd/csrc/rnde_reverse.hip
--- a/regneuralde.jl_amd/csrc/rnde_reverse.hip
+++ b/regneuralde.jl_amd/csrc/rnde_reverse.hip
@@ -347,20 +347,32 @@
         }
         HIPCHK(h, hipGetLastError());
         {
-            if (h->act2) {
-                hipLaunchKernelGGL((rnde_binit_stage_kernel<1, 0>), grid, blk, h->stage_lds, s, BQ);
-                hipLaunchKernelGGL((rnde_binit_stage_kernel<1, 1>), grid, blk, h->stage_lds, s, BQ);
+            if (init_pairs_on(h, "RNDE_BINIT_FUSE_OFF")) {
+                HIPCHK(h, init_pairs_begin(h, Q.F.Bpad, s));
+                const dim3 pgrid(8 * BQ.R * ((BQ.C + 7) / 8));
+                PersistSync Y0{init_region(h, 0), h->pabort, h->pxcc, h->persist_spins}, Y1{init_region(h, 1), h->pabort, h->pxcc, h->persist_spins};
+                if (h->act2) hipLaunchKernelGGL((rnde_binit_stage_pair_kernel<1, 0>), pgrid, blk, h->stage_lds, s, BQ, Y0, init_region(h, 1));
+                else hipLaunchKernelGGL((rnde_binit_stage_pair_kernel<0, 0>), pgrid, blk, h->stage_lds, s, BQ, Y0, init_region(h, 1));
+                if ((st = couple_sum(h, Q.ipart, 4LL * Q.F.nwg, s)) != RNDE_OK) return st;
+                if (h->act2) hipLaunchKernelGGL((rnde_binit_stage_pair_kernel<1, 1>), pgrid, blk, h->stage_lds, s, BQ, Y1, init_region(h, 0));
+                else hipLaunchKernelGGL((rnde_binit_stage_pair_kernel<0, 1>), pgrid, blk, h->stage_lds, s, BQ, Y1, init_region(h, 0));
+                h->init_pairs_open = false;
             } else {
-                hipLaunchKernelGGL((rnde_binit_stage_kernel<0, 0>), grid, blk, h->stage_lds, s, BQ);
-                hipLaunchKernelGGL((rnde_binit_stage_kernel<0, 1>), grid, blk, h->stage_lds, s, BQ);
-            }
-            if ((st = couple_sum(h, Q.ipart, 4LL * Q.F.nwg, s)) != RNDE_OK) return st;
-            if (h->act2) {
-                hipLaunchKernelGGL((rnde_binit_stage_kernel<1, 2>), grid, blk, h->stage_lds, s, BQ);
-                hipLaunchKernelGGL((rnde_binit_stage_kernel<1, 3>), grid, blk, h->stage_lds, s, BQ);
-            } else {
-                hipLaunchKernelGGL((rnde_binit_stage_kernel<0, 2>), grid, blk, h->stage_lds, s, BQ);
-                hipLaunchKernelGGL((rnde_binit_stage_kernel<0, 3>), grid, blk, h->stage_lds, s, BQ);
+                if (h->act2) {
+                    hipLaunchKernelGGL((rnde_binit_stage_kernel<1, 0>), grid, blk, h->stage_lds, s, BQ);
+                    hipLaunchKernelGGL((rnde_binit_stage_kernel<1, 1>), grid, blk, h->stage_lds, s, BQ);
+                } else {
+                    hipLaunchKernelGGL((rnde_binit_stage_kernel<0, 0>), grid, blk, h->stage_lds, s, BQ);
+                    hipLaunchKernelGGL((rnde_binit_stage_kernel<0, 1>), grid, blk, h->stage_lds, s, BQ);
+                }
+                if ((st = couple_sum(h, Q.ipart, 4LL * Q.F.nwg, s)) != RNDE_OK) return st;
+                if (h->act2) {
+                    hipLaunchKernelGGL((rnde_binit_stage_kernel<1, 2>), grid, blk, h->stage_lds, s, BQ);
+                    hipLaunchKernelGGL((rnde_binit_stage_kernel<1, 3>), grid, blk, h->stage_lds, s, BQ);
+                } else {
+                    hipLaunchKernelGGL((rnde_binit_stage_kernel<0, 2>), grid, blk, h->stage_lds, s, BQ);
+                    hipLaunchKernelGGL((rnde_binit_stage_kernel<0, 3>), grid, blk, h->stage_lds, s, BQ);
+                }
             }
             if ((st = couple_sum(h, Q.ipart + 4LL * Q.F.nwg, 4LL * Q.F.nwg, s)) != RNDE_OK) return st;
             hipLaunchKernelGGL(rnde_bfin_kernel, dim3(1), dim3(64), 0, s, Q);
@@ -820,3 +832,21 @@
                        v_dev, (long long)len, inv_decay, eta, rho);
     return hipGetLastError() == hipSuccess ? RNDE_OK : RNDE_ERR_HIP;
 }
+extern "C" rnde_status rnde_momentum_step_groups(int32_t n_groups, float* const* p_dev, const float* const* g_dev, float* const* v_dev, const int64_t* len,
+                                                 const int64_t* n, float gamma, float eta, float rho, float gscale, void* stream) {
+    if (n_groups < 0 || n_groups > rnde::kMomentumMaxGroups || (n_groups && (!p_dev || !g_dev || !v_dev || !len || !n))) return RNDE_ERR_BAD_ARG;
+    rnde::MomentumGroups G{};
+    int k = 0;
+    long long most = 0;
+    for (int i = 0; i < n_groups; ++i) {
+        if (!p_dev[i] || !g_dev[i] || !v_dev[i] || len[i] < 0 || n[i] < 1) return RNDE_ERR_BAD_ARG;
+        if (len[i] == 0) continue;
+        G.p[k] = p_dev[i]; G.g[k] = g_dev[i]; G.v[k] = v_dev[i]; G.len[k] = (long long)len[i];
+        G.inv_decay[k] = gscale / (1.0f + gamma * (float)n[i]);
+        most = std::max(most, (long long)len[i]);
+        ++k;
+    }
+    if (k == 0) return RNDE_OK;
+    hipLaunchKernelGGL(rnde::rnde_momentum_groups_kernel, dim3((unsigned)((most + 255) / 256), k), dim3(256), 0, (hipStream_t)stream, G, eta, rho);
+    return hipGetLastError() == hipSuccess ? RNDE_OK : RNDE_ERR_HIP;
+}
diff --git a/regneuralde.jl_amd/csrc/rnde_stage.h b/regneuralde.jl_amd/csrc/rnde_stage.h
--- a/regneuralde.jl_amd/csrc/rnde_stage.h
+++ b/regneuralde.jl_amd/csrc/rnde_stage.h
@@ -1,5 +1,6 @@
 #pragma once
 #include "rnde_fwd.h"
+#include "rnde_x3.h"
 
 namespace rnde {
 
@@ -59,13 +60,14 @@
 }
 
 struct PackJob { void* dst; const float* src; long long total; int kind, which, kdim, pad; };
-struct PackJobs { PackJob j[8]; };
+struct PackJobs { PackJob j[8]; X3PackDst x3; int MT, WT, R, HT; };
 static __global__ void rnde_pack_all_kernel(const float* __restrict__ p, const PackJobs J, int D, int H) {
     const PackJob job = J.j[blockIdx.y];
     for (long long i = blockIdx.x * (long long)blockDim.x + threadIdx.x; i < job.total; i += (long long)gridDim.x * blockDim.x) {
         if (job.kind == 0) ((f32x4*)job.dst)[i] = stage_pack_elem(p, job.which, D, H, job.kdim, i);
         else if (job.kind == 2) ((float*)job.dst)[i] = (job.src ? job.src : p)[i];
-        else ((f32x4*)job.dst)[i] = ((const f32x4*)(job.src ? job.src : p))[i];
+        else if (job.kind == 3) ((f32x4*)job.dst)[i] = ((const f32x4*)(job.src ? job.src : p))[i];
+        else x3_pack_elem(p, J.x3, D, H, J.MT, J.WT, J.R, J.HT, i);
     }
 }
 
@@ -92,26 +94,83 @@
     }
 }
 
+struct PersistSync {
+    float* tslab;
+    unsigned* abort_flag;
+    unsigned* xcc;
+    int max_spins;
+};
+
+constexpr int kPersistMaxSpins = 2000000;
+typedef unsigned u32x4 __attribute__((ext_vector_type(4)));
+
+constexpr unsigned kSlabEmpty = 0xFFFFFFFFu;
+__device__ __forceinline__ int slab_buf(unsigned ex) { return (int)(ex % 3u); }
+__device__ __forceinline__ void slab_put(float* tslab, size_t tile_index, int lane, const f32x4& v) {
+    u32x4 b = __builtin_bit_cast(u32x4, v);
+#pragma unroll
+    for (int i = 0; i < 4; ++i) b[i] = b[i] < 0xFFFFFFFEu ? b[i] : 0xFFFFFFFEu;
+    ((u32x4*)tslab + tile_index * 64)[lane] = b;
+}
+__device__ __forceinline__ void slab_clear(float* tslab, size_t tile_index, int lane) {
+    const float e = __builtin_bit_cast(float, kSlabEmpty);
+    ((f32x4*)tslab + tile_index * 64)[lane] = (f32x4){e, e, e, e};
+}
+__device__ __forceinline__ void slab_clears_done() { __builtin_amdgcn_s_waitcnt(0x0F70); }
+__device__ __forceinline__ bool slab_poll_sum(const PersistSync& Y, int buf, int C, int R, int HT, int ct, int ht, int lane, f32x4& zs) {
+    const float* base = Y.tslab + ((((size_t)buf * C + ct) * R) * HT) * 256;
+    __amdgpu_buffer_rsrc_t rs = __builtin_amdgcn_make_buffer_rsrc((void*)base, 0, 0x7fffffff, 0x00020000);
+    int spins = 0;
+    while (true) {
+        __asm__ volatile("" ::: "memory");
+        u32x4 e[kSMaxW];
+#pragma unroll
+        for (int r = 0; r < kSMaxW; ++r)
+            if (r < R) e[r] = __builtin_amdgcn_raw_buffer_load_b128(rs, ((r * HT + ht) * 64 + lane) * 16, 0, 16);
+        float s0 = 0.f, s1 = 0.f, s2 = 0.f, s3 = 0.f;
+#pragma unroll
+        for (int r = 0; r < kSMaxW; ++r) {
+            if (r < R) {
+                const f32x4 f = __builtin_bit_cast(f32x4, e[r]);
+                s0 += f[0]; s1 += f[1]; s2 += f[2]; s3 += f[3];
+            }
+        }
+        zs = (f32x4){s0, s1, s2, s3};
+        const bool clean = !(__builtin_isunordered(s0, s1) || __builtin_isunordered(s2, s3));
+        if (__all(clean)) return true;
+        unsigned m = 0u;
+#pragma unroll
+        for (int r = 0; r < kSMaxW; ++r)
+            if (r < R) { const unsigned a = e[r][0] > e[r][1] ? e[r][0] : e[r][1], b = e[r][2] > e[r][3] ? e[r][2] : e[r][3]; const unsigned c = a > b ? a : b; m = m > c ? m : c; }
+        const bool ok = m != kSlabEmpty;
+        if (__all(ok)) return true;
+        if (++spins > Y.max_spins || ((spins & 63) == 0 && __hip_atomic_load(Y.abort_flag, __ATOMIC_RELAXED, __HIP_MEMORY_SCOPE_AGENT))) {
+            __hip_atomic_store(Y.abort_flag, 1u, __ATOMIC_RELAXED, __HIP_MEMORY_SCOPE_AGENT);
+            zs = (f32x4){0.f, 0.f, 0.f, 0.f};
+            return false;
+        }
+    }
+}
+
 enum { SM_START = 0, SM_STAGE = 1, SM_LAST = 2, SM_I1 = 3, SM_I2 = 4, SM_I3 = 5, SM_I4 = 6, SM_FEVAL1 = 7, SM_FEVAL2 = 8 };
 
 __device__ __forceinline__ f32x4 ld4(const float* colbase, int r0, int D, bool ok, bool vec) { return ld_tile(colbase, r0, D, ok, vec); }
 __device__ __forceinline__ void st4(float* colbase, int r0, int D, bool ok, bool vec, f32x4 v) { st_tile(colbase, r0, D, ok, vec, v); }
 
-template <int ACT2, int MODE>
-__global__ __launch_bounds__(64 * kSMaxW) void rnde_stage_kernel(const StageParams Q, const int n, const int s) {
+template <int ACT2, int MODE, int HO>
+__device__ __forceinline__ bool stage_body(const StageParams& Q, const int n, const int s, float* smem, const int rb, const int ct, const int wg,
+                                           const PersistSync* Y, float* clear_slab, float& dt0_io) {
     const StepParams& P = Q.F;
-    extern __shared__ __attribute__((aligned(16))) float smem[];
     const int KH = 16 * Q.K2b + 4, KG = 16 * Q.WT + 4;
     float* HL = smem;
     float* GL = HL + kSCB * KH;
     float* RED = GL + kSCB * KG;
     const int tid = threadIdx.x, lane = tid & 63;
     const int w = __builtin_amdgcn_readfirstlane(tid >> 6);
-    const int rb = blockIdx.x / Q.C, ct = blockIdx.x - rb * Q.C;
     const int col = lane & 15, gcol = ct * kSCB + col;
     const bool colok = gcol < P.B;
     const bool vec = (P.D & 3) == 0;
-    const bool writer = (blockIdx.x == 0 && tid == 0);
+    const bool writer = (wg == 0 && tid == 0);
     const int T = rb * Q.WT + w;
     const int r0 = 16 * T + 4 * (lane >> 4);
     const bool tile_ok = T < Q.MT;
@@ -165,11 +224,12 @@
         }
         const int par0 = (MODE == SM_STAGE || MODE == SM_LAST) ? (s & 1) : 0;
         const f32x4* sl0 = (const f32x4*)Q.slab + (((size_t)par0 * Q.C + ct) * Q.R) * Q.HT * 64;
-        if (w < Q.HT) {
+        if (!HO && w < Q.HT) {
 #pragma unroll
             for (int r = 0; r < kSMaxW; ++r) if (r < Q.R) zr[r] = sl0[((size_t)r * Q.HT + w) * 64 + lane];
         }
     }
+    bool dead = false;
 
     float t = P.t0, dt = 0.f;
     int live = -1, rec = 0;
@@ -189,11 +249,11 @@
                 }
             }
         }
-        if (S.done) return;
+        if (S.done) return true;
         t = S.t; dt = (!P.forced && (P.t1 - S.t < S.dtp)) ? (P.t1 - S.t) : S.dtp; live = S.live;
     } else if constexpr (MODE == SM_STAGE || MODE == SM_LAST) {
         const StepState S = S0;
-        if (S.done) return;
+        if (S.done) return true;
         t = S.t; dt = (!P.forced && (P.t1 - S.t < S.dtp)) ? (P.t1 - S.t) : S.dtp; live = S.live;
     }
     if constexpr (MODE == SM_START || MODE == SM_STAGE || MODE == SM_LAST) rec = P.tape ? n + P.rec_shift : (live == 0 ? 1 : 0);
@@ -203,11 +263,14 @@
 
     if constexpr (kHasA) {
         if (w < Q.HT) {
-            const int par0 = (MODE == SM_STAGE || MODE == SM_LAST) ? (s & 1) : 0;
-            const f32x4* sl0 = (const f32x4*)Q.slab + (((size_t)par0 * Q.C + ct) * Q.R) * Q.HT * 64;
-#pragma unroll
-            for (int r = 0; r < kSMaxW; ++r) if (r < Q.R) zs += zr[r];
-            for (int r = kSMaxW; r < Q.R; ++r) zs += sl0[((size_t)r * Q.HT + w) * 64 + lane];
+            if constexpr (HO) dead = !slab_poll_sum(*Y, 0, Q.C, Q.R, Q.HT, ct, w, lane, zs);
+            else {
+                const int par0 = (MODE == SM_STAGE || MODE == SM_LAST) ? (s & 1) : 0;
+                const f32x4* sl0 = (const f32x4*)Q.slab + (((size_t)par0 * Q.C + ct) * Q.R) * Q.HT * 64;
+#pragma unroll
+                for (int r = 0; r < kSMaxW; ++r) if (r < Q.R) zs += zr[r];
+                for (int r = kSMaxW; r < Q.R; ++r) zs += sl0[((size_t)r * Q.HT + w) * 64 + lane];
+            }
         }
     }
     if constexpr (MODE == SM_START || MODE == SM_STAGE || MODE == SM_LAST) {
@@ -231,8 +294,9 @@
         if (d0 < 1e-5f || d1 < 1e-5f) { dt0 = 1e-6f; c0 = 1; } else dt0 = (d0 / d1) / 100.f;
         if (dtmax < dt0) { dt0 = dtmax; cl = 1; }
         if (writer) { P.initrec->d0 = d0; P.initrec->d1 = d1; P.initrec->dt0 = dt0; P.initrec->dt0_const = c0; P.initrec->dt0_clamped = cl; }
-    }
-    if constexpr (MODE == SM_I4) dt0 = P.initrec->dt0;
+        dt0_io = dt0;
+    }
+    if constexpr (MODE == SM_I4) dt0 = HO ? dt0_io : P.initrec->dt0;
 
     float ts = t;
     float* hdst = nullptr; float* kdst = nullptr;
@@ -253,7 +317,8 @@
             f32x4 z = zs;
             if (ht != w) {
                 z = (f32x4){0.f, 0.f, 0.f, 0.f};
-                for (int r = 0; r < Q.R; ++r) z += sl[((size_t)r * Q.HT + ht) * 64 + lane];
+                if constexpr (HO) { if (!dead) dead = !slab_poll_sum(*Y, 0, Q.C, Q.R, Q.HT, ct, ht, lane, z); }
+                else for (int r = 0; r < Q.R; ++r) z += sl[((size_t)r * Q.HT + ht) * 64 + lane];
             }
             const int h0 = 16 * ht + 4 * (lane >> 4);
             float pre[4];
@@ -283,7 +348,9 @@
             }
         }
         SSTAMP(2);
+        if constexpr (HO) { if (dead && lane == 0) RED[24] = 1.f; }
         __syncthreads();
+        if constexpr (HO) { if (RED[24] != 0.f) return false; }
         SSTAMP(3);
         if (tile_ok) {
             f32x4 acc0 = {0.f, 0.f, 0.f, 0.f}, acc1 = {0.f, 0.f, 0.f, 0.f};
@@ -406,6 +473,8 @@
         SSTAMP(6);
         const int par = (MODE == SM_START) ? 1 : (MODE == SM_STAGE ? ((s + 1) & 1) : 0);
         f32x4* sl = (f32x4*)Q.slab + ((((size_t)par * Q.C + ct) * Q.R + rb) * Q.HT) * 64;
+        const size_t tile0 = ((size_t)ct * Q.R + rb) * Q.HT;
+        if constexpr (HO) { for (int ht = w; ht < Q.HT; ht += Q.WT) slab_clear(clear_slab, tile0 + ht, lane); }
         const float* gbp = GL + col * KG + 4 * (lane >> 4);
         f32x4 bg[kSMaxW];
 #pragma unroll
@@ -421,7 +490,8 @@
                     acc1 = mfma16(wD[kb][3], bg[kb][3], acc1);
                 }
             }
-            sl[(size_t)w * 64 + lane] = acc0 + acc1;
+            if constexpr (HO) slab_put(Y->tslab, tile0 + w, lane, acc0 + acc1);
+            else sl[(size_t)w * 64 + lane] = acc0 + acc1;
         }
         for (int ht = w + Q.WT; ht < Q.HT; ht += Q.WT) {
             f32x4 acc0 = {0.f, 0.f, 0.f, 0.f}, acc1 = {0.f, 0.f, 0.f, 0.f};
@@ -435,7 +505,8 @@
                     acc1 = mfma16(a[3], bg[kb][3], acc1);
                 }
             }
-            sl[(size_t)ht * 64 + lane] = acc0 + acc1;
+            if constexpr (HO) slab_put(Y->tslab, tile0 + ht, lane, acc0 + acc1);
+            else sl[(size_t)ht * 64 + lane] = acc0 + acc1;
         }
         SSTAMP(7);
     }
@@ -449,12 +520,36 @@
             for (int i = 0; i < Q.WT; ++i) { sa += RED[i]; sb += RED[8 + i]; sc += RED[16 + i]; }
             if constexpr (MODE == SM_LAST) {
                 float* ep = P.errpart + (size_t)(n & 1) * 3 * P.nwg;
-                ep[blockIdx.x] = sa; ep[P.nwg + blockIdx.x] = sb; ep[2 * P.nwg + blockIdx.x] = sc;
-            }
-            else if constexpr (MODE == SM_I2) { P.initpart[blockIdx.x] = sa; P.initpart[P.nwg + blockIdx.x] = sb; }
-            else P.initpart[2 * P.nwg + blockIdx.x] = sa;
-        }
-    }
+                ep[wg] = sa; ep[P.nwg + wg] = sb; ep[2 * P.nwg + wg] = sc;
+            }
+            else if constexpr (MODE == SM_I2) { P.initpart[wg] = sa; P.initpart[P.nwg + wg] = sb; }
+            else P.initpart[2 * P.nwg + wg] = sa;
+        }
+    }
+    return true;
+}
+template <int ACT2, int MODE>
+__global__ __launch_bounds__(64 * kSMaxW) void rnde_stage_kernel(const StageParams Q, const int n, const int s) {
+    extern __shared__ __attribute__((aligned(16))) float smem[];
+    const int rb = blockIdx.x / Q.C, ct = blockIdx.x - rb * Q.C;
+    float dt0 = 0.f;
+    stage_body<ACT2, MODE, 0>(Q, n, s, smem, rb, ct, (int)blockIdx.x, nullptr, nullptr, dt0);
+}
+
+template <int ACT2, int PAIR>
+__global__ __launch_bounds__(64 * kSMaxW) void rnde_stage_init_pair_kernel(const StageParams Q, const PersistSync Y, float* clear_slab) {
+    extern __shared__ __attribute__((aligned(16))) float smem[];
+    const int rb = (blockIdx.x >> 3) % Q.R, ct = 8 * ((blockIdx.x >> 3) / Q.R) + (blockIdx.x & 7);
+    if (ct >= Q.C) return;
+    const int wg = rb * Q.C + ct;
+    float* RED = smem + kSCB * (16 * Q.K2b + 4) + kSCB * (16 * Q.WT + 4);
+    if (threadIdx.x == 0) {
+        Y.xcc[wg] = __builtin_amdgcn_s_getreg((3 << 11) | (0 << 6) | 20) & 15;
+        RED[24] = 0.f;
+    }
+    float dt0 = 0.f;
+    stage_body<ACT2, PAIR ? SM_I3 : SM_I1, 1>(Q, 0, 0, smem, rb, ct, wg, &Y, clear_slab, dt0);
+    stage_body<ACT2, PAIR ? SM_I4 : SM_I2, 1>(Q, 0, 0, smem, rb, ct, wg, &Y, nullptr, dt0);
 }
 
 static __global__ __launch_bounds__(256) void rnde_stage_finish_kernel(const StageParams Q, const int n, float* __restrict__ u_out) {
diff --git a/regneuralde.jl_amd/csrc/rnde_stage_persist.h b/regneuralde.jl_amd/csrc/rnde_stage_persist.h
--- a/regneuralde.jl_amd/csrc/rnde_stage_persist.h
+++ b/regneuralde.jl_amd/csrc/rnde_stage_persist.h
@@ -6,63 +6,6 @@
 
 namespace rnde {
 
-struct PersistSync {
-    float* tslab;
-    unsigned* abort_flag;
-    unsigned* xcc;
-    int max_spins;
-};
-
-constexpr int kPersistMaxSpins = 2000000;
-typedef unsigned u32x4 __attribute__((ext_vector_type(4)));
-
-constexpr unsigned kSlabEmpty = 0xFFFFFFFFu;
-__device__ __forceinline__ int slab_buf(unsigned ex) { return (int)(ex % 3u); }
-__device__ __forceinline__ void slab_put(float* tslab, size_t tile_index, int lane, const f32x4& v) {
-    u32x4 b = __builtin_bit_cast(u32x4, v);
-#pragma unroll
-    for (int i = 0; i < 4; ++i) b[i] = b[i] < 0xFFFFFFFEu ? b[i] : 0xFFFFFFFEu;
-    ((u32x4*)tslab + tile_index * 64)[lane] = b;
-}
-__device__ __forceinline__ void slab_clear(float* tslab, size_t tile_index, int lane) {
-    const float e = __builtin_bit_cast(float, kSlabEmpty);
-    ((f32x4*)tslab + tile_index * 64)[lane] = (f32x4){e, e, e, e};
-}
-__device__ __forceinline__ void slab_clears_done() { __builtin_amdgcn_s_waitcnt(0x0F70); }
-__device__ __forceinline__ bool slab_poll_sum(const PersistSync& Y, int buf, int C, int R, int HT, int ct, int ht, int lane, f32x4& zs) {
-    const float* base = Y.tslab + ((((size_t)buf * C + ct) * R) * HT) * 256;
-    __amdgpu_buffer_rsrc_t rs = __builtin_amdgcn_make_buffer_rsrc((void*)base, 0, 0x7fffffff, 0x00020000);
-    int spins = 0;
-    while (true) {
-        __asm__ volatile("" ::: "memory");
-        u32x4 e[kSMaxW];
-#pragma unroll
-        for (int r = 0; r < kSMaxW; ++r)
-            if (r < R) e[r] = __builtin_amdgcn_raw_buffer_load_b128(rs, ((r * HT + ht) * 64 + lane) * 16, 0, 16);
-        float s0 = 0.f, s1 = 0.f, s2 = 0.f, s3 = 0.f;
-#pragma unroll
-        for (int r = 0; r < kSMaxW; ++r) {
-            if (r < R) {
-                const f32x4 f = __builtin_bit_cast(f32x4, e[r]);
-                s0 += f[0]; s1 += f[1]; s2 += f[2]; s3 += f[3];
-            }
-        }
-        zs = (f32x4){s0, s1, s2, s3};
-        const bool clean = !(__builtin_isunordered(s0, s1) || __builtin_isunordered(s2, s3));
-        if (__all(clean)) return true;
-        unsigned m = 0u;
-#pragma unroll
-        for (int r = 0; r < kSMaxW; ++r)
-            if (r < R) { const unsigned a = e[r][0] > e[r][1] ? e[r][0] : e[r][1], b = e[r][2] > e[r][3] ? e[r][2] : e[r][3]; const unsigned c = a > b ? a : b; m = m > c ? m : c; }
-        const bool ok = m != kSlabEmpty;
-        if (__all(ok)) return true;
-        if (++spins > Y.max_spins || ((spins & 63) == 0 && __hip_atomic_load(Y.abort_flag, __ATOMIC_RELAXED, __HIP_MEMORY_SCOPE_AGENT))) {
-            __hip_atomic_store(Y.abort_flag, 1u, __ATOMIC_RELAXED, __HIP_MEMORY_SCOPE_AGENT);
-            zs = (f32x4){0.f, 0.f, 0.f, 0.f};
-            return false;
-        }
-    }
-}
 
 #ifdef RNDE_DIAG
 #define PSTAMP(i) do { if (P.dbg_out && wg == 0 && tid == 0) ((unsigned long long*)P.dbg_out)[i] = clock64(); } while (0)
diff --git a/regneuralde.jl_amd/csrc/rnde_x3.h b/regneuralde.jl_amd/csrc/rnde_x3.h
--- a/regneuralde.jl_amd/csrc/rnde_x3.h
+++ b/regneuralde.jl_amd/csrc/rnde_x3.h
@@ -81,48 +81,50 @@
 }
 
 struct X3PackDst { x3u4* d[4]; };
-static __global__ void rnde_x3_pack_kernel(const float* __restrict__ p, const X3PackDst dst, int D, int H, int MT, int WT, int R, int HT) {
+__device__ __forceinline__ void x3_pack_elem(const float* __restrict__ p, const X3PackDst& dst, int D, int H, int MT, int WT, int R, int HT, long long i) {
     const float* W1 = p;
     const float* b1 = W1 + (size_t)H * (D + 1);
     const float* W2 = b1 + H;
     const float* b2 = W2 + (size_t)D * (H + 1);
     const long long nB = (long long)MT * 4 * 64, nD = (long long)HT * R * 4 * 64, per = nB + nD;
-    const int nimg = dst.d[2] ? 2 : 1;
-    for (long long i = blockIdx.x * (long long)blockDim.x + threadIdx.x; i < nimg * per; i += (long long)gridDim.x * blockDim.x) {
-        const int rev = (int)(i / per);
-        const long long ii = i - rev * per;
-        const bool isD = ii >= nB;
-        const long long q = isD ? ii - nB : ii;
-        const int l = (int)(q & 63), s = (int)((q >> 6) & 3), tile = (int)(q >> 8);
-        float wv[8];
+    const int rev = (int)(i / per);
+    const long long ii = i - rev * per;
+    const bool isD = ii >= nB;
+    const long long q = isD ? ii - nB : ii;
+    const int l = (int)(q & 63), s = (int)((q >> 6) & 3), tile = (int)(q >> 8);
+    float wv[8];
 #pragma unroll
-        for (int j = 0; j < 8; ++j) {
-            const int k = 32 * s + 8 * (l >> 4) + j;
-            float w = 0.f;
-            if (!isD) {
-                const int m = 16 * tile + (l & 15);
-                if (m < D) {
-                    if (!rev) w = k <= H ? W2[(size_t)k * D + m] : (k == H + 1 ? b2[m] : 0.f);
-                    else if (k < H) w = W1[(size_t)m * H + k];
-                }
-            } else {
-                const int wt = tile / R, rb = tile % R;
-                const int m = 16 * wt + (l & 15), row = 16 * WT * rb + k;
-                if (k < 16 * WT && row < D) {
-                    if (!rev) { if (m < H) w = W1[(size_t)row * H + m]; }
-                    else if (m <= H) w = W2[(size_t)m * D + row];
-                }
+    for (int j = 0; j < 8; ++j) {
+        const int k = 32 * s + 8 * (l >> 4) + j;
+        float w = 0.f;
+        if (!isD) {
+            const int m = 16 * tile + (l & 15);
+            if (m < D) {
+                if (!rev) w = k <= H ? W2[(size_t)k * D + m] : (k == H + 1 ? b2[m] : 0.f);
+                else if (k < H) w = W1[(size_t)m * H + k];
             }
-            wv[j] = w;
+        } else {
+            const int wt = tile / R, rb = tile % R;
+            const int m = 16 * wt + (l & 15), row = 16 * WT * rb + k;
+            if (k < 16 * WT && row < D) {
+                if (!rev) { if (m < H) w = W1[(size_t)row * H + m]; }
+                else if (m <= H) w = W2[(size_t)m * D + row];
+            }
         }
-        unsigned hi[4], mid[4], lo[4];
+        wv[j] = w;
+    }
+    unsigned hi[4], mid[4], lo[4];
 #pragma unroll
-        for (int j = 0; j < 4; ++j) x3_split2(wv[2 * j], wv[2 * j + 1], hi[j], mid[j], lo[j]);
-        x3u4* o = dst.d[2 * rev + (isD ? 1 : 0)] + ((size_t)(tile * 4 + s) * 3) * 64 + l;
-        o[0] = (x3u4){hi[0], hi[1], hi[2], hi[3]};
-        o[64] = (x3u4){mid[0], mid[1], mid[2], mid[3]};
-        o[128] = (x3u4){lo[0], lo[1], lo[2], lo[3]};
-    }
+    for (int j = 0; j < 4; ++j) x3_split2(wv[2 * j], wv[2 * j + 1], hi[j], mid[j], lo[j]);
+    x3u4* o = dst.d[2 * rev + (isD ? 1 : 0)] + ((size_t)(tile * 4 + s) * 3) * 64 + l;
+    o[0] = (x3u4){hi[0], hi[1], hi[2], hi[3]};
+    o[64] = (x3u4){mid[0], mid[1], mid[2], mid[3]};
+    o[128] = (x3u4){lo[0], lo[1], lo[2], lo[3]};
+}
+static __global__ void rnde_x3_pack_kernel(const float* __restrict__ p, const X3PackDst dst, int D, int H, int MT, int WT, int R, int HT) {
+    const long long total = (dst.d[2] ? 2 : 1) * ((long long)(MT + HT * R) * 4 * 64);
+    for (long long i = blockIdx.x * (long long)blockDim.x + threadIdx.x; i < total; i += (long long)gridDim.x * blockDim.x)
+        x3_pack_elem(p, dst, D, H, MT, WT, R, HT, i);
 }
 
 }
```

Result: no change. 309,500 samples/s (median of 5 runs) (+0.8%).
